# Luckick/EAGCN

Measured on AMD Instinct MI355X. Metric: molecules/sec fwd+bwd, 2-layer 5-view EAGCN, Tox21 batch, higher is better.
Workload: dtype f32 (bf16x3 split, fp32 accumulate): every fp32 operand leaves its producer as three bf16 planes, six v_mfma_f32_32x32x16_bf16 piece products per 16 k rebuild the fp32 product (csrc/gemm_bx3.hip); aggregation, BatchNorm, head, first layer fp32

## Files before the change

eagcn_amd/_lib.py:

```python
import ctypes as C
import os

_HERE = os.path.dirname(os.path.abspath(__file__))
LIB_PATH = os.path.join(_HERE, 'lib', 'libeagcn_hip.so')

MAX_VIEWS = 8
MAX_SEGS = 8
META_WORDS = 16
META_NLOG = 8
META_T, META_NMAX, META_NTILES, META_BAD_ADJ, META_BAD_REL, META_NEDGE, META_OVERFLOW, META_EDGE_OVERFLOW = range(8)
META_NBLK = 9
STRUCT_CONCATE, STRUCT_WEIGHTED = 0, 1

_fp = C.c_void_p


class Batch(C.Structure):
    _fields_ = [('B', C.c_int32), ('N', C.c_int32), ('K', C.c_int32), ('ldc', C.c_int32),
                ('T', C.c_int32), ('n_max', C.c_int32), ('n_tiles', C.c_int32),
                ('channels', C.c_int32 * MAX_VIEWS),
                ('code', _fp), ('deg_bn', _fp), ('nat', _fp), ('row0', _fp), ('tile0', _fp),
                ('meta', _fp), ('row_mol', _fp), ('row_loc', _fp), ('row_m', _fp), ('row_deg', _fp),
                ('tile_mol', _fp), ('row_info', _fp), ('tile_info', _fp),
                ('rel_vec', _fp * MAX_VIEWS), ('rel_c', C.c_int32 * MAX_VIEWS),
# ... 33 lines not shown
    _fields_ = [('K', C.c_int32), ('mode', C.c_int32), ('att_c', C.c_int32 * MAX_VIEWS), ('att_w', _fp * MAX_VIEWS),
                ('ave_a', _fp), ('self_r', _fp), ('datt_w', _fp * MAX_VIEWS), ('dave_a', _fp), ('dself_r', _fp)]


class Layout(C.Structure):
    _fields_ = [('nseg', C.c_int32), ('width', C.c_int32 * MAX_SEGS), ('pad', C.c_int32 * MAX_SEGS)]


class LayerParams(C.Structure):
    _fields_ = [('K', C.c_int32), ('structure', C.c_int32), ('training', C.c_int32),
                ('width', C.c_int32 * MAX_VIEWS), ('inp', Layout),
                ('dropout', C.c_float), ('bn_eps', C.c_float), ('bn_momentum', C.c_float),
                ('seed', C.c_uint64), ('seed_dev', _fp),
                ('att_w', _fp * MAX_VIEWS), ('self_r', _fp * MAX_VIEWS), ('W', _fp * MAX_VIEWS),
                ('bias', _fp * MAX_VIEWS), ('gamma', _fp * MAX_VIEWS), ('beta', _fp * MAX_VIEWS),
                ('run_mean', _fp * MAX_VIEWS), ('run_var', _fp * MAX_VIEWS), ('ave_w', _fp)]


class LayerBufs(C.Structure):
    _fields_ = [('x', _fp), ('P', _fp), ('Y', _fp), ('rscale', _fp), ('bn', _fp), ('xout', _fp),
                ('pad_row', _fp), ('scratch', _fp), ('scratch_bytes', C.c_size_t),
                ('aux_stream', _fp), ('packed', _fp), ('packed_bytes', C.c_size_t),
                ('stats_hook', _fp), ('stats_user', _fp), ('x_planes', _fp), ('xout_planes', _fp)]


class LayerGrads(C.Structure):
    _fields_ = [('dW', _fp * MAX_VIEWS), ('dbias', _fp * MAX_VIEWS), ('dgamma', _fp * MAX_VIEWS),
                ('dbeta', _fp * MAX_VIEWS), ('datt_w', _fp * MAX_VIEWS), ('dself_r', _fp * MAX_VIEWS),
                ('dave_w', _fp)]


class HeadParams(C.Structure):
    _fields_ = [('f_in', C.c_int32), ('n_den1', C.c_int32), ('n_den2', C.c_int32), ('nclass', C.c_int32),
                ('dropout', C.c_float), ('bn_eps', C.c_float), ('bn_momentum', C.c_float),
                ('den1_w', _fp), ('den2_w', _fp), ('den3_w', _fp),
                ('gbn_w', _fp), ('gbn_b', _fp), ('gbn_rm', _fp), ('gbn_rv', _fp),
                ('bn1_w', _fp), ('bn1_b', _fp), ('bn1_rm', _fp), ('bn1_rv', _fp),
                ('bn2_w', _fp), ('bn2_b', _fp), ('bn2_rm', _fp), ('bn2_rv', _fp)]


class HeadGrads(C.Structure):
    _fields_ = [(n, _fp) for n in ('d_den1_w', 'd_den2_w', 'd_den3_w', 'd_gbn_w', 'd_gbn_b', 'd_bn1_w', 'd_bn1_b',
                                   'd_bn2_w', 'd_bn2_b')]


class Model(C.Structure):
    _fields_ = [('n_layers', C.c_int32), ('molfp_mode', C.c_int32), ('training', C.c_int32),
                ('head_seed', C.c_uint64), ('head_seed_dev', _fp), ('input_packed', C.c_int32), ('aux_stream', _fp),
                ('layer', LayerParams * 4), ('head', HeadParams), ('stats_hook', _fp), ('stats_user', _fp),
                ('stats_world', C.c_int32), ('fuse_readout', C.c_int32), ('fwd_signal', _fp), ('wait_flag', _fp), ('start_signal', _fp)]


class StepLoss(C.Structure):
    _fields_ = [('kind', C.c_int32), ('labels', _fp), ('class_weight', _fp), ('loss', _fp), ('scale', _fp), ('dout', _fp)]


ALLREDUCE_FN = C.CFUNCTYPE(C.c_int, C.c_void_p, C.c_int, C.c_void_p, C.c_void_p)


SIGNATURES = {
    'eagcn_abi_version': (C.c_int, []),
    'eagcn_struct_size': (C.c_size_t, [C.c_int]),
    'eagcn_last_error': (C.c_char_p, []),
    'eagcn_pad16': (C.c_int, [C.c_int]),
    'eagcn_layer_out_ld': (C.c_int, [C.POINTER(LayerParams)]),
    'eagcn_layer_fp': (C.c_int, [C.POINTER(LayerParams)]),
    'eagcn_layer_packed_bytes': (C.c_size_t, [C.POINTER(Batch), C.POINTER(LayerParams)]),
    'eagcn_layer_fwd_scratch_bytes': (C.c_size_t, [C.POINTER(Batch), C.POINTER(LayerParams)]),
    'eagcn_layer_bwd_scratch_bytes': (C.c_size_t, [C.POINTER(Batch), C.POINTER(LayerParams)]),
    'eagcn_index_build': (C.c_int, [_fp, C.POINTER(_fp), C.POINTER(Batch), _fp, _fp]),
    'eagcn_index_from_bonds': (C.c_int, [_fp, _fp, _fp, _fp, C.c_int64, C.POINTER(Batch), _fp, _fp]),
    'eagcn_index_rows': (C.c_int, [C.POINTER(Batch), _fp]),
    'eagcn_set_gemm_mode': (C.c_int, [C.c_int]),
    'eagcn_stream_wait_counter': (C.c_int, [_fp, C.c_uint32, _fp]),
    'eagcn_stream_signal_flag': (C.c_int, [_fp, _fp]),
    'eagcn_stream_wait_flag': (C.c_int, [_fp, C.c_double, _fp]),
    'eagcn_stream_wait_timeouts': (C.c_int, []),
    'eagcn_stream_wait_reset': (None, []),
    'eagcn_adam_step': (C.c_int, [_fp, _fp, _fp, _fp, C.c_int64, _fp, _fp, _fp, _fp]),
    'eagcn_agg_wants_bond_lists': (C.c_int, [C.c_int, C.c_int]),
    'eagcn_agg_wants_bond_lists_for': (C.c_int, [C.c_int, C.c_int, C.c_int]),
    'eagcn_bx3_used_splits': (C.c_int, [C.c_int, C.c_int, C.c_int, C.c_int]),
    'eagcn_set_bx3_wide': (C.c_int, [C.c_int]),
    'eagcn_bx3_pair_used_splits': (C.c_int, [C.c_int] * 7),
    'eagcn_bx3_plane_elems': (C.c_size_t, [C.c_int, C.c_int]),
    'eagcn_bx3_split': (C.c_int, [_fp, C.c_int, C.c_int, _fp, C.c_size_t, C.c_int, C.c_int, _fp]),
    'eagcn_gemm_bx3': (C.c_int, [C.c_int, C.c_int, C.c_int, C.c_int, _fp, C.c_size_t, C.c_int, C.c_int, _fp, C.c_size_t, C.c_int, C.c_int,
                                 _fp, C.c_int, C.c_int, C.c_size_t, C.c_int, _fp]),
    'eagcn_gemm_bx3_pair': (C.c_int, [C.c_int, C.c_int, C.c_int, _fp, C.c_size_t, C.c_int, C.c_int, _fp, C.c_size_t, C.c_int, C.c_int, _fp, C.c_int,
                                      C.c_int, C.c_int, C.c_int, _fp, C.c_size_t, C.c_int, C.c_int, _fp, C.c_size_t, C.c_int, C.c_int, _fp, C.c_int,
                                      C.c_int, C.c_size_t, C.c_int, _fp]),
    'eagcn_pack_rows': (C.c_int, [C.POINTER(Batch), _fp, C.c_int, C.POINTER(Layout), _fp, _fp]),
    'eagcn_unpack_rows': (C.c_int, [C.POINTER(Batch), _fp, C.POINTER(Layout), _fp, _fp, C.c_int, _fp]),
    'eagcn_pad_rows': (C.c_int, [_fp, _fp, C.c_int, C.c_int, C.c_int, _fp, _fp]),
    'eagcn_gat_scratch_bytes': (C.c_size_t, [C.POINTER(Batch), C.c_int]),
    'eagcn_gat_forward': (C.c_int, [C.POINTER(Batch), C.POINTER(GatParams), _fp, _fp, _fp, _fp, _fp]),
    'eagcn_gat_backward': (C.c_int, [C.POINTER(Batch), C.POINTER(GatParams), _fp, _fp, _fp, _fp, _fp, _fp, _fp, _fp, _fp,
                                     C.c_size_t, _fp]),
    'eagcn_pool_scratch_bytes': (C.c_size_t, []),
    'eagcn_pool_attention_forward': (C.c_int, [C.POINTER(Batch), C.POINTER(PoolAtt), _fp, C.c_int, _fp, _fp, _fp]),
    'eagcn_pool_attention_backward': (C.c_int, [C.POINTER(Batch), C.POINTER(PoolAtt), _fp, C.c_int, _fp, _fp, _fp, C.c_size_t,
                                                _fp]),
    'eagcn_pool_mix_forward': (C.c_int, [C.POINTER(Batch), C.POINTER(Layout), _fp, C.c_int, _fp, _fp, _fp, _fp, C.c_int, _fp]),
    'eagcn_pool_mix_backward': (C.c_int, [C.POINTER(Batch), C.POINTER(Layout), _fp, C.c_int, _fp, _fp, _fp, _fp, C.c_int, _fp,
                                          _fp, _fp, _fp]),
    'eagcn_pool_reduce_forward': (C.c_int, [C.POINTER(Batch), _fp, C.c_int, C.c_int, C.c_int, _fp, _fp, _fp, _fp]),
    'eagcn_pool_reduce_backward': (C.c_int, [C.POINTER(Batch), _fp, C.c_int, C.c_int, C.c_int, _fp, _fp, _fp, _fp, _fp]),
    'eagcn_layer_forward': (C.c_int, [C.POINTER(Batch), C.POINTER(LayerParams), C.POINTER(LayerBufs), _fp]),
    'eagcn_layer_backward': (C.c_int, [C.POINTER(Batch), C.POINTER(LayerParams), C.POINTER(LayerBufs),
                                       _fp, _fp, _fp, C.POINTER(LayerGrads), _fp]),
    'eagcn_attention_dense': (C.c_int, [C.POINTER(Batch), C.POINTER(LayerParams), _fp, _fp]),
    'eagcn_readout_forward': (C.c_int, [C.POINTER(Batch), _fp, C.POINTER(Layout), _fp, _fp, C.c_int, _fp,
                                        C.c_int, _fp]),
    'eagcn_readout_backward': (C.c_int, [C.POINTER(Batch), _fp, C.POINTER(Layout), _fp, C.c_int, C.c_int,
                                         _fp, _fp, _fp]),
    'eagcn_gemm_f32': (C.c_int, [C.c_int, C.c_int, C.c_int, C.c_int, C.c_int, _fp, C.c_int, _fp, C.c_int,
                                 _fp, C.c_int, _fp]),
    'eagcn_gemm_f32_dev': (C.c_int, [C.c_int, C.c_int, C.c_int, C.c_int, C.c_int, _fp, C.c_int, _fp, C.c_int,
                                     _fp, C.c_int, _fp, C.c_int, _fp]),
    'eagcn_gemm_sk_workspace_bytes': (C.c_size_t, []),
    'eagcn_gemm_f32_sk': (C.c_int, [C.c_int, C.c_int, C.c_int, C.c_int, C.c_int, _fp, C.c_int, _fp, C.c_int,
                                    _fp, C.c_int, _fp, C.c_size_t, _fp]),
    'eagcn_gemm_pair_sk': (C.c_int, [C.c_int, C.c_int, C.c_int, _fp, C.c_int, _fp, C.c_int, _fp, C.c_int,
                                     C.c_int, C.c_int, C.c_int, _fp, C.c_int, _fp, C.c_int, _fp, C.c_int,
                                     _fp, C.c_size_t, _fp]),
    'eagcn_gemm_pair_sk_slabs': (C.c_int, [C.c_int, C.c_int, C.c_int, _fp, C.c_int, _fp, C.c_int, _fp, C.c_int,
                                           C.c_int, C.c_int, C.c_int, _fp, C.c_int, _fp, C.c_int, _fp, C.c_int,
                                           C.c_size_t, _fp, C.c_size_t, _fp]),
    'eagcn_gemm_sk_plan': (C.c_int, [C.c_int] * 7 + [C.POINTER(C.c_int), C.POINTER(C.c_int)]),
    'eagcn_gemm_sk_timeouts': (C.c_int, []),
    'eagcn_gemm_sk_failed': (C.c_int, []),
    'eagcn_gemm_sk_reset_failed': (None, []),
    'eagcn_gemm_sk_inject_failure': (None, []),
    'eagcn_model_saved_bytes': (C.c_size_t, [C.POINTER(Batch), C.POINTER(Model)]),
    'eagcn_model_scratch_bytes': (C.c_size_t, [C.POINTER(Batch), C.POINTER(Model)]),
    'eagcn_model_atom_rep': (C.c_int, [C.POINTER(Batch), C.POINTER(Model), C.POINTER(C.c_size_t),
                                       C.POINTER(C.c_size_t), C.POINTER(C.c_int)]),
    'eagcn_model_atom_rep_materialize': (C.c_int, [C.POINTER(Batch), C.POINTER(Model), _fp, C.c_size_t, _fp]),
    'eagcn_model_pack_input': (C.c_int, [C.POINTER(Batch), C.POINTER(Model), _fp, _fp, C.c_size_t, _fp]),
    'eagcn_model_forward': (C.c_int, [C.POINTER(Batch), C.POINTER(Model), _fp, _fp, _fp, C.c_size_t, _fp,
                                      C.c_size_t, _fp, _fp, _fp]),
    'eagcn_model_backward': (C.c_int, [C.POINTER(Batch), C.POINTER(Model), _fp, _fp, C.c_size_t, _fp, C.c_size_t,
                                       _fp, _fp, C.POINTER(LayerGrads), C.POINTER(HeadGrads), _fp]),
    'eagcn_model_backward_range': (C.c_int, [C.POINTER(Batch), C.POINTER(Model), _fp, _fp, C.c_size_t, _fp, C.c_size_t,
                                             _fp, _fp, C.POINTER(LayerGrads), C.POINTER(HeadGrads), C.c_int, C.c_int, C.c_int, _fp]),
    'eagcn_model_input_scratch_bytes': (C.c_size_t, [C.POINTER(Batch), C.POINTER(Model)]),
    'eagcn_model_backward_input': (C.c_int, [C.POINTER(Batch), C.POINTER(Model), _fp, _fp, C.c_size_t, _fp, C.c_size_t,
                                             _fp, _fp, C.POINTER(LayerGrads), C.POINTER(HeadGrads), _fp, _fp]),
    'eagcn_attr_alpha': (C.c_float, [C.c_int, C.c_int]),
    'eagcn_attr_weight': (C.c_float, [C.c_int]),
    'eagcn_attr_acc_elems': (C.c_size_t, [C.POINTER(Batch), C.POINTER(Model)]),
    'eagcn_attr_pack_input': (C.c_int, [C.POINTER(Batch), C.POINTER(Model), _fp, _fp, C.c_float, _fp, C.c_size_t, _fp]),
    'eagcn_attr_step': (C.c_int, [C.POINTER(Batch), C.POINTER(Model), _fp, _fp, C.c_size_t, _fp, C.c_size_t, _fp, _fp, C.c_float,
                                  C.c_int, _fp, _fp]),
    'eagcn_attr_finalize': (C.c_int, [C.POINTER(Batch), C.POINTER(Model), _fp, _fp, _fp, _fp, _fp, _fp]),
    'eagcn_model_forward_step': (C.c_int, [C.POINTER(Batch), C.POINTER(Model), _fp, _fp, _fp, C.c_size_t, _fp, C.c_size_t, _fp, _fp,
                                           C.POINTER(StepLoss), _fp, C.POINTER(HeadGrads), _fp]),
    'eagcn_head_saved_bytes': (C.c_size_t, [C.POINTER(HeadParams), C.c_int]),
    'eagcn_head_scratch_bytes': (C.c_size_t, [C.POINTER(HeadParams), C.c_int]),
    'eagcn_head_forward': (C.c_int, [C.POINTER(HeadParams), C.c_int, C.c_int, C.c_uint64, _fp, _fp, _fp, C.c_size_t, _fp, C.c_size_t,
                                     _fp, _fp, _fp]),
    'eagcn_head_backward': (C.c_int, [C.POINTER(HeadParams), C.c_int, C.c_int, C.c_uint64, _fp, _fp, _fp, C.c_size_t, _fp, C.c_size_t,
                                      _fp, _fp, C.POINTER(HeadGrads), _fp, _fp]),
    'eagcn_bce_loss': (C.c_int, [_fp, _fp, _fp, C.c_int, C.c_int, _fp, _fp, _fp]),
    'eagcn_mse_loss': (C.c_int, [_fp, _fp, C.c_int, _fp, _fp, _fp]),
    'eagcn_eval_append': (C.c_int, [_fp, _fp, C.c_int, C.c_int, C.c_int, _fp, _fp, _fp, C.c_int64, _fp]),
# ... 65 lines not shown
```

eagcn_amd/csrc/head.hip:

```cpp
#include <stdlib.h>

#include <algorithm>

#include "common.h"
#include "kernels.h"

namespace eagcn {

__global__ void wait_counter_kernel(const uint32_t* __restrict__ word, uint32_t value, int* __restrict__ err,
                                    unsigned long long budget_ticks) {
    if (threadIdx.x == 0) {
        const unsigned long long t0 = wall_clock64();
        while ((int32_t)(__hip_atomic_load(word, __ATOMIC_ACQUIRE, __HIP_MEMORY_SCOPE_AGENT) - value) < 0) {
            __builtin_amdgcn_s_sleep(64);
            if (wall_clock64() - t0 > budget_ticks) {
                if (err) __hip_atomic_store(err, 1, __ATOMIC_RELAXED, __HIP_MEMORY_SCOPE_SYSTEM);
                break;
            }
        }
    }
}



// ... 36 lines not shown
    return EAGCN_OK;
}

struct Carver2 {
    char* base;
    size_t off = 0;
    explicit Carver2(void* p) : base((char*)p) {}
    template <typename T>
    T* take(size_t n) {
        T* p = base ? (T*)(base + off) : nullptr;
        off = align256(off + std::max<size_t>(n, 1) * sizeof(T));
        return p;
    }
};

struct LayerSaved { float *P, *Y, *rscale, *bn, *xout, *pad_row; void* packed; size_t packed_bytes; int fp, ldo, ld_in;
                    uint16_t* xout_planes; };
struct ModelSaved {
    float* x0;
    LayerSaved L[4];
    float *g, *h1, *h2, *bn_g, *bn_1, *bn_2;
    uint16_t* pad_cnt;
    float* padc;
    uint32_t* pad_tab;
    size_t xout_last_off, pad_last_off;
};
static bool pad_sampled(const eagcn_model* m) {
    const eagcn_layer_params* last = &m->layer[m->n_layers - 1];
    return last->structure == EAGCN_STRUCT_WEIGHTED && m->training && last->dropout > 0.0f;
}

static size_t carve_saved(void* base, const eagcn_batch* b, const eagcn_model* m, ModelSaved* out) {
    Carver2 c(base);
    ModelSaved s;
    const size_t T = (size_t)b->T;
    s.x0 = c.take<float>(T * layout_ld(&m->layer[0].in));
    for (int l = 0; l < m->n_layers; ++l) {
        const eagcn_layer_params* p = &m->layer[l];
        LayerSaved& L = s.L[l];
        L.fp = eagcn_layer_fp(p);
        L.ldo = eagcn_layer_out_ld(p);
        L.ld_in = layout_ld(&p->in);
        L.P = c.take<float>(T * L.fp);
        L.Y = c.take<float>(T * L.fp);
        L.rscale = c.take<float>((size_t)p->K * T);
        L.bn = c.take<float>((size_t)4 * L.fp);
        if (l == m->n_layers - 1) s.xout_last_off = c.off;
        L.xout = c.take<float>(T * L.ldo);
        if (l == m->n_layers - 1) s.pad_last_off = c.off;
        L.pad_row = c.take<float>(L.ldo);
        L.packed_bytes = eagcn_layer_packed_bytes(b, p);
        L.packed = c.take<char>(L.packed_bytes);
        const int np = (l + 1 < m->n_layers && L.ldo >= 128 && (L.ldo & 15) == 0) ? gemm_planes() : 0;
        L.xout_planes = np ? c.take<uint16_t>((size_t)np * bx_plane_elems(T, L.ldo)) : nullptr;
    }
    const eagcn_head_params* h = &m->head;
    const size_t B = (size_t)b->B;
    s.g = c.take<float>(B * h->f_in);
    s.h1 = c.take<float>(B * h->n_den1);
    s.h2 = c.take<float>(B * h->n_den2);
    s.bn_g = c.take<float>((size_t)4 * h->f_in);
    s.bn_1 = c.take<float>((size_t)4 * h->n_den1);
    s.bn_2 = c.take<float>((size_t)4 * h->n_den2);
    {
        const eagcn_layer_params* last = &m->layer[m->n_layers - 1];
        const size_t ldo = (size_t)eagcn_layer_out_ld(last);
        const bool need = last->structure == EAGCN_STRUCT_WEIGHTED;
        s.pad_cnt = c.take<uint16_t>(need ? B * last->K * ldo : 1);
        s.padc = c.take<float>(need ? B * ldo : 1);
        const size_t nt = (size_t)(b->N + 1) * (b->N + 1);
        s.pad_tab = c.take<uint32_t>(need ? nt : 1);
    }
    if (out) *out = s;
    return c.off;
}

struct ModelScratch {
    float *da2, *da1, *dgn, *dg, *dxa, *dxb, *dpad;
    float* hdw; int hdw_ks;
    double* hst; int n_hst;
    double* hws;
    double* hsb;
    void* layer; size_t layer_bytes;
};
static size_t carve_scratch(void* base, const eagcn_batch* b, const eagcn_model* m, ModelScratch* out) {
    Carver2 c(base);
    ModelScratch s;
    const eagcn_head_params* h = &m->head;
    const size_t B = (size_t)b->B, T = (size_t)b->T;
    s.n_hst = 2 * (h->f_in + h->n_den1 + h->n_den2) + 6;
    s.hst = c.take<double>((size_t)(HEAD_COPIES + 1) * s.n_hst + HEAD_WS);
    s.hsb = s.hst + (size_t)HEAD_COPIES * s.n_hst;
    s.hws = s.hsb + s.n_hst;
    s.da2 = c.take<float>(B * h->n_den2);
    s.da1 = c.take<float>(B * h->n_den1);
    s.dgn = c.take<float>(B * h->f_in);
    s.dg = c.take<float>(B * h->f_in);
    s.hdw_ks = head_dw_chunks(b->B);
    s.hdw = c.take<float>(s.hdw_ks > 1 ? (size_t)s.hdw_ks * ((size_t)h->f_in * h->n_den1 + (size_t)h->n_den1 * h->n_den2 +
                                                             (size_t)h->n_den2 * h->nclass) : 1);
    int ldmax = 0;
    size_t lbytes = 0;
    for (int l = 0; l < m->n_layers; ++l) {
        ldmax = std::max(ldmax, eagcn_layer_out_ld(&m->layer[l]));
        lbytes = std::max(lbytes, eagcn_layer_fwd_scratch_bytes(b, &m->layer[l]));
        lbytes = std::max(lbytes, eagcn_layer_bwd_scratch_bytes(b, &m->layer[l]));
    }
    s.dxa = c.take<float>(T * ldmax);
    s.dxb = c.take<float>(T * ldmax);
    s.dpad = c.take<float>((size_t)EAGCN_MAX_VIEWS * ldmax);
    s.layer_bytes = lbytes;
    s.layer = c.take<char>(lbytes);
    if (out) *out = s;
    return c.off;
}

static int check_model(const eagcn_batch* b, const eagcn_model* m, const char* who) {
    EAGCN_CHECK_ARG(b && m, "%s: null argument", who);
    EAGCN_CHECK_ARG(m->n_layers >= 1 && m->n_layers <= 4, "%s: n_layers=%d", who, m->n_layers);
    const eagcn_head_params* h = &m->head;
    EAGCN_CHECK_ARG(h->f_in >= 1 && h->n_den1 >= 1 && h->n_den2 >= 1 && h->nclass >= 1, "%s: bad head sizes", who);
    EAGCN_CHECK_ARG(h->den1_w && h->den2_w && h->den3_w && h->gbn_w && h->gbn_b && h->gbn_rm && h->gbn_rv &&
                        h->bn1_w && h->bn1_b && h->bn1_rm && h->bn1_rv && h->bn2_w && h->bn2_b && h->bn2_rm &&
                        h->bn2_rv, "%s: null head parameter", who);
    const eagcn_layer_params* last = &m->layer[m->n_layers - 1];
    const int f_last = last->structure == EAGCN_STRUCT_CONCATE ? [&] { int s = 0; for (int k = 0; k < last->K; ++k) s += last->width[k]; return s; }()
                                                                 : last->width[0];
    EAGCN_CHECK_ARG(f_last == h->f_in, "%s: head expects %d features, last layer yields %d", who, h->f_in, f_last);
    EAGCN_CHECK_ARG(!m->training || b->B > 1, "%s: BatchNorm in training mode needs more than one molecule", who);
    return EAGCN_OK;
}

static eagcn_layout out_layout(const eagcn_layer_params* p) {
    eagcn_layout l;
    memset(&l, 0, sizeof(l));
    if (p->structure == EAGCN_STRUCT_CONCATE) {
        l.nseg = p->K;
        for (int k = 0; k < p->K; ++k) { l.width[k] = p->width[k]; l.pad[k] = pad16(p->width[k]); }
    } else {
        l.nseg = 1;
        l.width[0] = p->width[0];
        l.pad[0] = pad16(p->width[0]);
    }
    return l;
}

static bool fused_readout(const eagcn_model* m) {
    static const bool env = [] { const char* v = getenv("EAGCN_NO_FUSED_READOUT"); return !(v && v[0] == '1'); }();
    return env && m->fuse_readout && m->layer[m->n_layers - 1].structure == EAGCN_STRUCT_CONCATE;
}

static bool hidden_planes_only(const eagcn_batch* b, const eagcn_model* m, const ModelSaved& sv, int l) {
    return l + 1 < m->n_layers && sv.L[l].xout_planes && layer_reads_planes_only(b, &m->layer[l + 1], m->aux_stream != nullptr);
}

static void fill_drop(float p, int training, int* do_drop, uint32_t* thr, float* inv_keep) {
    *do_drop = (training && p > 0.0f) ? 1 : 0;
    *thr = (uint32_t)std::min(4294967295.0, (double)p * 4294967296.0);
    *inv_keep = 1.0f / (1.0f - p);
}

}

using namespace eagcn;

#define RC(call) do { int rc_ = (call); if (rc_) return rc_; } while (0)

extern "C" size_t eagcn_model_saved_bytes(const eagcn_batch* b, const eagcn_model* m) {
    return carve_saved(nullptr, b, m, nullptr);
}
extern "C" size_t eagcn_model_scratch_bytes(const eagcn_batch* b, const eagcn_model* m) {
    return carve_scratch(nullptr, b, m, nullptr);
}
extern "C" int eagcn_model_atom_rep(const eagcn_batch* b, const eagcn_model* m, size_t* xout_offset,
                                    size_t* pad_row_offset, int* ld) {
    EAGCN_CHECK_ARG(b && m && xout_offset && pad_row_offset && ld, "eagcn_model_atom_rep: null argument");
    ModelSaved s;
    carve_saved(nullptr, b, m, &s);
    *xout_offset = s.xout_last_off;
    *pad_row_offset = s.pad_last_off;
    *ld = eagcn_layer_out_ld(&m->layer[m->n_layers - 1]);
    return EAGCN_OK;
}

extern "C" int eagcn_model_atom_rep_materialize(const eagcn_batch* b, const eagcn_model* m, void* saved, size_t saved_bytes,
                                                 void* stream) {
    EAGCN_CHECK_ARG(b && m && saved, "eagcn_model_atom_rep_materialize: null argument");
    if (!fused_readout(m)) return EAGCN_OK;
    ModelSaved sv;
// ... 10 lines not shown
                                      size_t saved_bytes, void* stream) {
    EAGCN_CHECK_ARG(b && m && afm && saved, "eagcn_model_pack_input: null argument");
    ModelSaved sv;
    EAGCN_CHECK_ARG(carve_saved(saved, b, m, &sv) <= saved_bytes, "eagcn_model_pack_input: saved block too small");
    return eagcn_pack_rows(b, afm, layout_width(&m->layer[0].in), &m->layer[0].in, sv.x0, stream);
}

struct HeadPlan {
    HeadFwd f1, f2, f3;
    HeadBwd b3, b2, b1;
    HeadGbn bg;
    double *st_g, *st_1, *st_2, *sb_g, *sb_1, *sb_2;
    bool sync;
};
static HeadPlan head_plan(const eagcn_batch* b, const eagcn_model* m, const ModelSaved& sv, const ModelScratch& sc, float* out,
                          float* graph_rep, const float* dout, const float* dgraph_rep, const eagcn_head_grads* hg) {
    HeadPlan P;
    const eagcn_head_params* h = &m->head;
    const int B = b->B, F = h->f_in, n1 = h->n_den1, n2 = h->n_den2, nc = h->nclass;
    P.st_g = sc.hst; P.st_1 = sc.hst + 2 * F + 2; P.st_2 = sc.hst + 2 * (F + n1) + 4;
    P.sb_g = sc.hsb; P.sb_1 = sc.hsb + 2 * F + 2; P.sb_2 = sc.hsb + 2 * (F + n1) + 4;
    P.sync = m->stats_hook && m->training;
    const int copies = P.sync ? 1 : HEAD_COPIES;
    HeadDrop nodrop{0, 0u, 1.0f, 0, nullptr}, drop1 = nodrop;
    {
        int on; uint32_t thr; float inv_keep;
        fill_drop(h->dropout, m->training, &on, &thr, &inv_keep);
        drop1 = HeadDrop{on, thr, inv_keep, m->head_seed, m->head_seed_dev};
    }
    P.f1 = HeadFwd{B, F, n1, sv.g, P.st_g, h->gbn_w, h->gbn_b, h->gbn_rm, h->gbn_rv, sv.bn_g, h->den1_w, sv.h1, nullptr, P.st_1,
                   m->training, 0, h->bn_eps, h->bn_momentum, nodrop};
    P.f2 = HeadFwd{B, n1, n2, sv.h1, P.st_1, h->bn1_w, h->bn1_b, h->bn1_rm, h->bn1_rv, sv.bn_1, h->den2_w, sv.h2, graph_rep, P.st_2,
                   m->training, 1, h->bn_eps, h->bn_momentum, drop1};
    P.f3 = HeadFwd{B, n2, nc, sv.h2, P.st_2, h->bn2_w, h->bn2_b, h->bn2_rm, h->bn2_rv, sv.bn_2, h->den3_w, out, nullptr, nullptr,
                   m->training, 1, h->bn_eps, h->bn_momentum, nodrop};
    if (P.sync) { P.f1.cnt_in = P.st_g + 2 * F; P.f2.cnt_in = P.st_1 + 2 * n1; P.f3.cnt_in = P.st_2 + 2 * n2; }
    P.f3.nw = 8;
    P.f1.signal = m->fwd_signal;
    P.f1.st_copies = P.f2.st_copies = P.f3.st_copies = copies;
    P.f1.st_stride = P.f2.st_stride = P.f3.st_stride = sc.n_hst;
    if (!hg) return P;
    const double *cn_g = sc.hst + 2 * F, *cn_1 = sc.hst + 2 * F + 2 + 2 * n1, *cn_2 = sc.hst + 2 * (F + n1) + 4 + 2 * n2;
    const float gscale = P.sync && m->stats_world > 1 ? 1.0f / (float)m->stats_world : 1.0f;
    P.b3 = HeadBwd{B, n2, nc, sv.h2, sv.bn_2, 1, nodrop, h->den3_w, dout, nullptr, nullptr, nullptr, nullptr, nullptr, nullptr,
                   sc.da2, P.sb_2, hg->d_den3_w, m->training};
    P.b2 = HeadBwd{B, n1, n2, sv.h1, sv.bn_1, 1, drop1, h->den2_w, sc.da2, sv.h2, sv.bn_2, P.sb_2, dgraph_rep, hg->d_bn2_w, hg->d_bn2_b,
                   sc.da1, P.sb_1, hg->d_den2_w, m->training};
    P.b1 = HeadBwd{B, F, n1, sv.g, sv.bn_g, 0, nodrop, h->den1_w, sc.da1, sv.h1, sv.bn_1, P.sb_1, nullptr, hg->d_bn1_w, hg->d_bn1_b,
                   sc.dgn, P.sb_g, hg->d_den1_w, m->training};
    if (P.sync) { P.b2.cnt_y = cn_2; P.b2.gscale = gscale; P.b1.cnt_y = cn_1; P.b1.gscale = gscale; }
    P.b3.nw = 8;
    const int ks = sc.hdw_ks;
    float* part3 = sc.hdw;
    float* part2 = part3 + (size_t)ks * n2 * nc;
    float* part1 = part2 + (size_t)ks * n1 * n2;
    if (ks > 1) {
        P.b3.ks = ks; P.b3.dW_part = part3;
        P.b2.ks = ks; P.b2.dW_part = part2;
        P.b1.ks = ks; P.b1.dW_part = part1;
    }
    P.bg = HeadGbn{B, F, sc.dgn, sv.g, sv.bn_g, P.sb_g, sc.dg, hg->d_gbn_w, hg->d_gbn_b, m->training};
    if (P.sync) { P.bg.cnt = cn_g; P.bg.gscale = gscale; }
    if (ks > 1) {
        P.bg.sum[0] = HeadDwSum{hg->d_den3_w, part3, n2 * nc, ks};
        P.bg.sum[1] = HeadDwSum{hg->d_den2_w, part2, n1 * n2, ks};
        P.bg.sum[2] = HeadDwSum{hg->d_den1_w, part1, F * n1, ks};
        P.bg.nsum = 3;
    }
    return P;
}

static int model_forward_trunk(const eagcn_batch* b, const eagcn_model* m, const float* afm, const int64_t* size, void* saved,
                               size_t saved_bytes, void* scratch, size_t scratch_bytes, ModelSaved& sv, ModelScratch& sc,
                               void* stream, const char* who) {
    hipStream_t s = (hipStream_t)stream;
    RC(check_model(b, m, who));
    EAGCN_CHECK_GEMM3(who);
    EAGCN_CHECK_ARG((afm || m->input_packed) && saved && scratch, "%s: null buffer", who);
    EAGCN_CHECK_ARG(m->molfp_mode == 0 || size, "%s: 'ave' read-out needs size", who);
    EAGCN_CHECK_ARG(carve_saved(saved, b, m, &sv) <= saved_bytes, "%s: saved block too small", who);
    EAGCN_CHECK_ARG(carve_scratch(scratch, b, m, &sc) <= scratch_bytes, "%s: scratch too small", who);
    const eagcn_head_params* h = &m->head;
    HandOff ho{m->start_signal, m->wait_flag, wait_err_word(), 200000000ull};
    if (!m->input_packed && (m->wait_flag || m->start_signal)) {
        handoff_kernel<<<1, 64, 0, s>>>(ho);
        EAGCN_LAUNCH_CHECK();
        ho.start = nullptr; ho.flag = nullptr;
    }
    ZeroJob zj;
    RC(gemm3_zero_job(sc.layer, sc.layer_bytes, sc.hst, (HEAD_COPIES + 1) * sc.n_hst + HEAD_WS, &zj));
    if (!m->input_packed)
        RC(eagcn_pack_rows(b, afm, layout_width(&m->layer[0].in), &m->layer[0].in, sv.x0, stream));
    const float* x = sv.x0;
    {
        const eagcn_layer_params* ps[4];
        void* pk[4];
        size_t pkb[4];
        for (int l = 0; l < m->n_layers; ++l) { ps[l] = &m->layer[l]; pk[l] = sv.L[l].packed; pkb[l] = sv.L[l].packed_bytes; }
        RC(pack_params_all(b, ps, pk, pkb, m->n_layers, stream, &zj, &ho));
    }
    for (int l = 0; l < m->n_layers; ++l) {
        LayerSaved& L = sv.L[l];
        eagcn_layer_bufs w;
        memset(&w, 0, sizeof(w));
        w.x = x; w.P = L.P; w.Y = L.Y; w.rscale = L.rscale; w.bn = L.bn; w.xout = L.xout; w.pad_row = L.pad_row;
        w.scratch = sc.layer; w.scratch_bytes = sc.layer_bytes; w.packed = L.packed; w.packed_bytes = L.packed_bytes;
        w.stats_hook = m->stats_hook; w.stats_user = m->stats_user;
        w.x_planes = l > 0 ? sv.L[l - 1].xout_planes : nullptr; w.xout_planes = L.xout_planes;
        const bool po = hidden_planes_only(b, m, sv, l);
        RC(layer_forward_impl(b, &m->layer[l], &w, stream, true, l == m->n_layers - 1 && fused_readout(m), po));
        x = po ? nullptr : L.xout;
    }
    const eagcn_layer_params* last = &m->layer[m->n_layers - 1];
    const LayerSaved& LL = sv.L[m->n_layers - 1];
    const eagcn_layout lay = out_layout(last);
    const int B = b->B, F = h->f_in, n1 = h->n_den1, n2 = h->n_den2;
    double *st_g = sc.hst, *st_1 = sc.hst + 2 * F + 2, *st_2 = sc.hst + 2 * (F + n1) + 4;
    const int copies = (m->stats_hook && m->training) ? 1 : HEAD_COPIES;
    if (fused_readout(m)) {
        ReadoutBn rb;
        rb.Y = LL.Y; rb.ldy = LL.fp; rb.bn = LL.bn; rb.fp = LL.fp;
        fill_drop(last->dropout, last->training, &rb.do_drop, &rb.thr, &rb.inv_keep);
        rb.seed = last->seed; rb.seed_dev = last->seed_dev;
        rb.size = size; rb.mode = m->molfp_mode; rb.g = sv.g; rb.F = F; rb.st = st_g;
        rb.cnt0 = st_g + 2 * F; rb.cnt1 = st_1 + 2 * n1; rb.cnt2 = st_2 + 2 * n2;
        rb.st_copies = copies; rb.st_stride = sc.n_hst;
        RC(readout_bn_forward(b, &lay, rb, stream));
    } else if (pad_sampled(m))
        RC(readout_forward_sampled(b, LL.xout, &lay, last, LL.bn + (size_t)LL.fp , size,
                                   m->molfp_mode, sv.g, F, sv.pad_cnt, sv.padc, sv.pad_tab, stream));
    else
        RC(eagcn_readout_forward(b, LL.xout, &lay, last->structure == EAGCN_STRUCT_WEIGHTED ? LL.pad_row : nullptr,
                                 size, m->molfp_mode, sv.g, F, stream));
    if (!fused_readout(m)) RC(head_colstats(sv.g, B, F, st_g, s, st_g + 2 * F, st_1 + 2 * n1, st_2 + 2 * n2));
    return EAGCN_OK;
}

static int stats_hook_call(const eagcn_model* m, bool sync, double* buf, int n, void* stream) {
    if (!sync) return EAGCN_OK;
    if (m->stats_hook(buf, n, stream, m->stats_user)) {
        set_error("eagcn_model: the sync-BatchNorm all-reduce hook failed");
        return EAGCN_ERR_HIP;
    }
    return EAGCN_OK;
}

static int head_forward_launches(const eagcn_model* m, const HeadPlan& P, void* stream) {
    hipStream_t s = (hipStream_t)stream;
    const eagcn_head_params* h = &m->head;
    RC(stats_hook_call(m, P.sync, P.st_g, 2 * h->f_in + 1, stream));
    RC(head_fwd(P.f1, s));
    RC(stats_hook_call(m, P.sync, P.st_1, 2 * h->n_den1 + 1, stream));
    RC(head_fwd(P.f2, s));
    RC(stats_hook_call(m, P.sync, P.st_2, 2 * h->n_den2 + 1, stream));
    RC(head_fwd(P.f3, s));
    return EAGCN_OK;
}
static int head_backward_launches(const eagcn_model* m, const HeadPlan& P, void* stream) {
    hipStream_t s = (hipStream_t)stream;
    const eagcn_head_params* h = &m->head;
    RC(head_bwd(P.b3, s));
    RC(stats_hook_call(m, P.sync, P.sb_2, 2 * h->n_den2, stream));
    RC(head_bwd(P.b2, s));
    RC(stats_hook_call(m, P.sync, P.sb_1, 2 * h->n_den1, stream));
    RC(head_bwd(P.b1, s));
    RC(stats_hook_call(m, P.sync, P.sb_g, 2 * h->f_in, stream));
    RC(head_gbn_bwd(P.bg, s));
    return EAGCN_OK;
}
static int readout_pad_backward(const eagcn_batch* b, const eagcn_model* m, const int64_t* size, const ModelSaved& sv,
                                const ModelScratch& sc, void* stream) {
    const eagcn_layer_params* last = &m->layer[m->n_layers - 1];
    const eagcn_layout lay = out_layout(last);
    const int F = m->head.f_in;
    if (pad_sampled(m)) return readout_backward_pad_views(b, sc.dg, &lay, size, m->molfp_mode, F, last->K, sv.pad_cnt, last->dropout, sc.dpad, stream);
    if (last->structure == EAGCN_STRUCT_WEIGHTED) return readout_backward_pad(b, sc.dg, &lay, size, m->molfp_mode, F, sc.dpad, stream);
    return EAGCN_OK;
}

extern "C" int eagcn_model_forward(const eagcn_batch* b, const eagcn_model* m, const float* afm,
                                   const int64_t* size, void* saved, size_t saved_bytes, void* scratch,
                                   size_t scratch_bytes, float* out, float* graph_rep, void* stream) {
    EAGCN_CHECK_ARG(out && graph_rep, "eagcn_model_forward: null buffer");
    ModelSaved sv;
    ModelScratch sc;
    RC(model_forward_trunk(b, m, afm, size, saved, saved_bytes, scratch, scratch_bytes, sv, sc, stream, "eagcn_model_forward"));
    const HeadPlan P = head_plan(b, m, sv, sc, out, graph_rep, nullptr, nullptr, nullptr);
    return head_forward_launches(m, P, stream);
}

namespace eagcn {
static int check_head(const eagcn_head_params* h, int B, int training, const char* who) {
    EAGCN_CHECK_ARG(h, "%s: null argument", who);
// ... 113 lines not shown
                                        const eagcn_head_grads* hg, void* stream) {
    hipStream_t s = (hipStream_t)stream;
    EAGCN_CHECK_ARG(out && graph_rep && loss && hg, "eagcn_model_forward_step: null argument");
    EAGCN_CHECK_ARG(m && m->training, "eagcn_model_forward_step: a training-mode model is required");
    EAGCN_CHECK_ARG((loss->kind == 0 || loss->kind == 1) && loss->labels && loss->loss && loss->dout && (loss->kind == 1 || loss->class_weight),
                    "eagcn_model_forward_step: bad loss descriptor");
    EAGCN_CHECK_ARG(hg->d_den1_w && hg->d_den2_w && hg->d_den3_w && hg->d_gbn_w && hg->d_gbn_b && hg->d_bn1_w &&
                        hg->d_bn1_b && hg->d_bn2_w && hg->d_bn2_b, "eagcn_model_forward_step: null head gradient");
    ModelSaved sv;
    ModelScratch sc;
    RC(model_forward_trunk(b, m, afm, size, saved, saved_bytes, scratch, scratch_bytes, sv, sc, stream, "eagcn_model_forward_step"));
    const HeadPlan P = head_plan(b, m, sv, sc, out, graph_rep, loss->dout, dgraph_rep, hg);
    const eagcn_head_params* h = &m->head;
    if (!P.sync && head_mid_ok(h->n_den2, h->nclass)) {
        HeadPlan Q = P;
        unsigned* words = reinterpret_cast<unsigned*>(sc.hws);
        if (loss->kind == 0) { Q.f2.lab = loss->labels; Q.f2.nlab = b->B * h->nclass; Q.f2.lab_cnt = words + 1; }
        RC(head_fwd(Q.f1, s));
        RC(head_fwd(Q.f2, s));
        HeadMid M;
        M.f3 = Q.f3; M.b3 = Q.b3;
        M.L = HeadLoss{loss->kind, loss->labels, loss->class_weight, loss->loss, loss->scale, loss->dout};
        M.ws = sc.hws;
        RC(head_mid(M, s));
        RC(head_bwd_pair(Q.b2, Q.b3, HeadLossFin{loss->loss, sc.hws, loss->scale, loss->kind, b->B * h->nclass}, s));
        RC(head_bwd(Q.b1, s));
        RC(head_gbn_bwd(Q.bg, s));
    } else {
        RC(head_forward_launches(m, P, stream));
        if (loss->kind == 0) RC(eagcn_bce_loss(out, loss->labels, loss->class_weight, b->B, h->nclass, loss->loss, loss->dout, stream));
        else RC(eagcn_mse_loss(out, loss->labels, b->B * h->nclass, loss->loss, loss->dout, stream));
        if (loss->scale) {
            const int n = b->B * h->nclass;
            scale_loss_kernel<<<cdiv(n, 256), 256, 0, s>>>(loss->loss, loss->dout, n, loss->scale);
            EAGCN_LAUNCH_CHECK();
        }
        RC(head_backward_launches(m, P, stream));
    }
    return readout_pad_backward(b, m, size, sv, sc, stream);
}

extern "C" int eagcn_model_backward(const eagcn_batch* b, const eagcn_model* m, const int64_t* size, void* saved,
                                    size_t saved_bytes, void* scratch, size_t scratch_bytes, const float* dout,
                                    const float* dgraph_rep, const eagcn_layer_grads* lg,
                                    const eagcn_head_grads* hg, void* stream) {
    EAGCN_CHECK_ARG(m, "eagcn_model_backward: null model");
    return eagcn_model_backward_range(b, m, size, saved, saved_bytes, scratch, scratch_bytes, dout, dgraph_rep, lg, hg, 1,
                                      m->n_layers - 1, 0, stream);
}

static int model_backward_impl(const eagcn_batch* b, const eagcn_model* m, const int64_t* size, void* saved, size_t saved_bytes,
                               void* scratch, size_t scratch_bytes, const float* dout, const float* dgraph_rep,
                               const eagcn_layer_grads* lg, const eagcn_head_grads* hg, int with_head, int layer_hi, int layer_lo,
                               float* dx0, bool input_only, void* stream) {
    hipStream_t s = (hipStream_t)stream;
    EAGCN_CHECK_ARG(saved && scratch && dout && (lg || input_only) && hg, "eagcn_model_backward: null buffer");
    EAGCN_CHECK_ARG(hg->d_den1_w && hg->d_den2_w && hg->d_den3_w && hg->d_gbn_w && hg->d_gbn_b && hg->d_bn1_w &&
                        hg->d_bn1_b && hg->d_bn2_w && hg->d_bn2_b, "eagcn_model_backward: null head gradient");
    EAGCN_CHECK_ARG(layer_hi < m->n_layers && layer_lo >= 0 && layer_lo <= layer_hi + 1,
                    "eagcn_model_backward_range: layers %d..%d of %d", layer_hi, layer_lo, m->n_layers);
    EAGCN_CHECK_ARG(!with_head || layer_hi == m->n_layers - 1 || layer_hi < layer_lo,
                    "eagcn_model_backward_range: the head's backward is followed by the top layer");
    ModelSaved sv;
    ModelScratch sc;
    EAGCN_CHECK_ARG(carve_saved(saved, b, m, &sv) <= saved_bytes, "eagcn_model_backward: saved block too small");
    EAGCN_CHECK_ARG(carve_scratch(scratch, b, m, &sc) <= scratch_bytes, "eagcn_model_backward: scratch too small");
    const int F = m->head.f_in;
    const ZeroJob zb{nullptr, 0, sc.hsb, sc.n_hst};
    hipStream_t side = m->aux_stream ? (hipStream_t)m->aux_stream : s;
    const bool forked = side != s;
    const eagcn_layer_params* last = &m->layer[m->n_layers - 1];
    const eagcn_layout lay = out_layout(last);
    const bool weighted = last->structure == EAGCN_STRUCT_WEIGHTED;
    const bool sampled = pad_sampled(m);
    if (with_head) {
        const HeadPlan P = head_plan(b, m, sv, sc, nullptr, nullptr, dout, dgraph_rep, hg);
        RC(head_backward_launches(m, P, stream));
        if (!(input_only && !m->training)) RC(readout_pad_backward(b, m, size, sv, sc, stream));
    }
    ReadoutGrad rgd;
    memset(&rgd, 0, sizeof(rgd));
    rgd.dg = sc.dg; rgd.F = F; rgd.size = size; rgd.mode = m->molfp_mode; rgd.map = make_colmap(&lay);
    const int top_l = m->n_layers - 1;
    EdgeDrain pend_in, pend_out;
    pend_in.eacc = nullptr;
    pend_out.eacc = nullptr;
    for (int l = layer_hi; l >= layer_lo; --l) {
        const int t = top_l - l;
        float* cur = (t & 1) ? sc.dxb : sc.dxa;
        float* other = (t & 1) ? sc.dxa : sc.dxb;
        LayerSaved& L = sv.L[l];
        eagcn_layer_bufs w;
        memset(&w, 0, sizeof(w));
        w.x = l == 0 ? sv.x0 : (hidden_planes_only(b, m, sv, l - 1) ? nullptr : sv.L[l - 1].xout);
        w.P = L.P; w.Y = L.Y; w.rscale = L.rscale; w.bn = L.bn; w.xout = L.xout; w.pad_row = L.pad_row;
        w.scratch = sc.layer; w.scratch_bytes = sc.layer_bytes; w.packed = L.packed; w.packed_bytes = L.packed_bytes;
        w.aux_stream = m->aux_stream;
        w.stats_hook = m->stats_hook; w.stats_user = m->stats_user;
        w.x_planes = l > 0 ? sv.L[l - 1].xout_planes : nullptr;
        const bool top = l == top_l;
        const float* dpad = (weighted && top) ? sc.dpad : nullptr;
        RC(layer_backward_impl(b, &m->layer[l], &w, top ? nullptr : cur, top ? &rgd : nullptr, dpad,
                               l > 0 ? other : dx0, input_only ? nullptr : &lg[l], stream, top && sampled, top ? &zb : nullptr,
                               pend_in.eacc ? &pend_in : nullptr, (l > layer_lo && !input_only) ? &pend_out : nullptr, input_only));
        pend_in = pend_out;
        if (l == layer_lo) pend_in.eacc = nullptr;
    }
    if (forked) RC(stream_after(s, side));
    return EAGCN_OK;
}

extern "C" int eagcn_model_backward_range(const eagcn_batch* b, const eagcn_model* m, const int64_t* size, void* saved,
                                          size_t saved_bytes, void* scratch, size_t scratch_bytes, const float* dout,
                                          const float* dgraph_rep, const eagcn_layer_grads* lg,
                                          const eagcn_head_grads* hg, int with_head, int layer_hi, int layer_lo, void* stream) {
    RC(check_model(b, m, "eagcn_model_backward"));
    EAGCN_CHECK_GEMM3("eagcn_model_backward");
    return model_backward_impl(b, m, size, saved, saved_bytes, scratch, scratch_bytes, dout, dgraph_rep, lg, hg, with_head, layer_hi,
                               layer_lo, nullptr, false, stream);
}

struct InputScratch { float* dx0; eagcn_head_grads hg; };
static size_t carve_input_scratch(void* base, const eagcn_batch* b, const eagcn_model* m, InputScratch* out) {
    Carver2 c(base);
    c.off = carve_scratch(nullptr, b, m, nullptr);
    InputScratch t;
    const eagcn_head_params* h = &m->head;
    const size_t F = h->f_in, n1 = h->n_den1, n2 = h->n_den2, nc = h->nclass;
    t.dx0 = c.take<float>((size_t)std::max(b->T, 1) * layout_ld(&m->layer[0].in));
    t.hg.d_den1_w = c.take<float>(F * n1);
    t.hg.d_den2_w = c.take<float>(n1 * n2);
    t.hg.d_den3_w = c.take<float>(n2 * nc);
    t.hg.d_gbn_w = c.take<float>(F);
    t.hg.d_gbn_b = c.take<float>(F);
    t.hg.d_bn1_w = c.take<float>(n1);
    t.hg.d_bn1_b = c.take<float>(n1);
    t.hg.d_bn2_w = c.take<float>(n2);
    t.hg.d_bn2_b = c.take<float>(n2);
    if (out) *out = t;
    return c.off;
}

static int check_engine_model(const eagcn_batch* b, const eagcn_model* m, const char* who) {
    RC(check_model(b, m, who));
    EAGCN_CHECK_ARG(m->molfp_mode == 0 || m->molfp_mode == 1, "%s: read-out mode %d has no engine path", who, m->molfp_mode);
    for (int l = 0; l < m->n_layers; ++l)
        EAGCN_CHECK_ARG(m->layer[l].structure == EAGCN_STRUCT_CONCATE || m->layer[l].structure == EAGCN_STRUCT_WEIGHTED,
                        "%s: layer %d has structure %d, which the engine does not run", who, l, m->layer[l].structure);
    return EAGCN_OK;
}

int eagcn::model_backward_input_packed(const eagcn_batch* b, const eagcn_model* m, const int64_t* size, void* saved, size_t saved_bytes,
                                       void* scratch, size_t scratch_bytes, const float* dout, const float* dgraph_rep,
                                       const eagcn_layer_grads* lg, const eagcn_head_grads* hg, float** dx0, void* stream,
                                       const char* who) {
    EAGCN_CHECK_ARG(b && m, "%s: null argument", who);
    EAGCN_CHECK_ARG((lg == nullptr) == (hg == nullptr), "%s: lg and hg are both given (full backward) or both NULL (input-only)", who);
    RC(check_engine_model(b, m, who));
    EAGCN_CHECK_GEMM3(who);
    EAGCN_CHECK_ARG(saved && scratch && dout, "%s: null buffer", who);
    InputScratch is;
    EAGCN_CHECK_ARG(carve_input_scratch(scratch, b, m, &is) <= scratch_bytes, "%s: scratch too small (eagcn_model_input_scratch_bytes)", who);
    *dx0 = is.dx0;
    const bool input_only = lg == nullptr;
    return model_backward_impl(b, m, size, saved, saved_bytes, scratch, scratch_bytes, dout, dgraph_rep, lg, input_only ? &is.hg : hg, 1,
                               m->n_layers - 1, 0, is.dx0, input_only, stream);
}

int eagcn::model_input_slot(const eagcn_batch* b, const eagcn_model* m, void* saved, size_t saved_bytes, float** x0, const char* who) {
    ModelSaved sv;
    EAGCN_CHECK_ARG(carve_saved(saved, b, m, &sv) <= saved_bytes, "%s: saved block too small", who);
    *x0 = sv.x0;
    return EAGCN_OK;
}

extern "C" size_t eagcn_model_input_scratch_bytes(const eagcn_batch* b, const eagcn_model* m) {
    return (b && m) ? carve_input_scratch(nullptr, b, m, nullptr) : 0;
}

extern "C" int eagcn_model_backward_input(const eagcn_batch* b, const eagcn_model* m, const int64_t* size, void* saved,
                                          size_t saved_bytes, void* scratch, size_t scratch_bytes, const float* dout,
                                          const float* dgraph_rep, const eagcn_layer_grads* lg, const eagcn_head_grads* hg,
                                          float* dafm, void* stream) {
    EAGCN_CHECK_ARG(dafm, "eagcn_model_backward_input: null dafm");
    float* dx0 = nullptr;
    RC(model_backward_input_packed(b, m, size, saved, saved_bytes, scratch, scratch_bytes, dout, dgraph_rep, lg, hg, &dx0, stream,
                                   "eagcn_model_backward_input"));
    return launch_attr_dense(b, &m->layer[0].in, dx0, nullptr, nullptr, dafm, nullptr, (hipStream_t)stream);
}
// ... 25 lines not shown
```

eagcn_amd/csrc/kernels.h:

```cpp
#pragma once
#include "bx3.h"
#include "common.h"

namespace eagcn {

struct AggArgs {
    eagcn_batch bt;
    ViewCols vc;
    const float* src; int lds;
    float* dst; int ldd;
    const float* sig;
    const float* rsig;
    float* rscale;
    double* stats;
    int nchunk;
    int cpw = 1;
    int xcd = 0;
    bool w_rowm = false;
    BxOut planes = {nullptr, 0, 0, 0};
    const float* bn_tab = nullptr; const float* bn_cc = nullptr; int bn_fp = 0;
    const float* w_aw = nullptr;
    int w_drop = 0; uint32_t w_thr = 0; float w_inv_keep = 1.0f; uint64_t w_seed = 0; const uint64_t* w_seed_dev = nullptr;
};
int agg_grid_x(const eagcn_batch* b);
// ... 92 lines not shown
}
size_t gemm3_workspace_bytes();
bool gemm3_xk_enabled();
int gemm3_grid();
int gemm3_clear_flags(void* workspace, size_t bytes, hipStream_t s, double* zero = nullptr, int nzero = 0);
int gemm3_failed();
#define EAGCN_CHECK_GEMM3(who)                                                                                         \
    do {                                                                                                               \
        if (::eagcn::gemm3_failed()) {                                                                                 \
            ::eagcn::set_error("%s: a stream-K hand-off of an earlier GEMM launch timed out (a contributor wave was not " \
                               "co-resident with its owner): that launch's results are NaN-poisoned; call "           \
                               "eagcn_gemm_sk_reset_failed() after fixing the cause (EAGCN_GEMM3_WGS, concurrent work)", who); \
            return EAGCN_ERR_HIP;                                                                                      \
        }                                                                                                              \
    } while (0)
int gemm_mode();
inline int gemm_planes() { const int m = gemm_mode(); return m == 3 ? 3 : m == 4 ? 1 : 0; }
struct ZeroJob { unsigned* u; int nu; double* d; int nd; };
struct HandOff { uint32_t* start; uint32_t* flag; int* err; unsigned long long budget; };
__device__ __forceinline__ void handoff_body(const HandOff& h) {
    if (h.start) __hip_atomic_fetch_add(h.start, 1u, __ATOMIC_RELEASE, __HIP_MEMORY_SCOPE_AGENT);
    if (h.flag) {
        const unsigned long long t0 = wall_clock64();
        while (__hip_atomic_load(h.flag, __ATOMIC_ACQUIRE, __HIP_MEMORY_SCOPE_AGENT) == 0u) {
            __builtin_amdgcn_s_sleep(8);
            if (wall_clock64() - t0 > h.budget) {
                if (h.err) __hip_atomic_store(h.err, 1, __ATOMIC_RELAXED, __HIP_MEMORY_SCOPE_SYSTEM);
                break;
            }
        }
        __hip_atomic_store(h.flag, 0u, __ATOMIC_RELAXED, __HIP_MEMORY_SCOPE_AGENT);
    }
}
int gemm3_zero_job(void* workspace, size_t bytes, double* zero, int nzero, ZeroJob* out);
int zero_fill(void* p, size_t bytes, hipStream_t s);
bool gemm3_ok(const GemmDesc& g);
int launch_gemm3(const GemmDesc& g, const DwScatter* sc, void* workspace, size_t bytes, hipStream_t s);
int launch_gemm3_pair(const GemmDesc& dx, const GemmDesc& dw, const DwScatter* sc, void* workspace, size_t bytes, hipStream_t s,
                      size_t xk_slab = 0);

constexpr int HEAD_COPIES = 8;
struct HeadDrop { int on; uint32_t thr; float inv_keep; uint64_t seed; const uint64_t* seed_dev; };
struct HeadFwd {
    int B, K, N;
    const float* x; const double* st_in; const float *gamma, *beta; float *run_mean, *run_var; float* bn;
    const float* W; float* y; float* y2; double* st_out;
    int training, relu; float eps, momentum; HeadDrop drop;
    const double* cnt_in = nullptr;
    int st_copies = 1, st_stride = 0;
    const float* lab = nullptr; int nlab = 0; unsigned* lab_cnt = nullptr;
    int nw = 0;
    uint32_t* signal = nullptr;
};
struct HeadBwd {
    int B, K, N;
    const float* x; const float* bnp; int relu_p; HeadDrop drop; const float* W;
    const float* dy; const float* y; const float* bny; const double* sb_y; const float* extra;
    float *dgamma_y, *dbeta_y; float* dyp; double* sb_p; float* dW; int training;
    const double* cnt_y = nullptr;
    float gscale = 1.0f;
    int ks = 1; float* dW_part = nullptr;
    int nw = 0;
};
inline int head_dw_chunks(int B) { return B > 256 ? (B + 255) / 256 < 16 ? (B + 255) / 256 : 16 : 1; }
struct HeadDwSum { float* dst; const float* part; int n, ks; };
struct HeadGbn { int B, F; const float *dgn, *g, *bn; const double* sb; float *dg, *dgamma, *dbeta; int training;
                 const double* cnt = nullptr; float gscale = 1.0f;
                 HeadDwSum sum[3] = {}; int nsum = 0; };
struct HeadLoss { int kind;
                  const float* labels; const float* weight; float* loss; const float* scale; float* dout; };
struct HeadMid { HeadFwd f3; HeadBwd b3; HeadLoss L;
                 double* ws; };
constexpr int HEAD_WS = 4;
struct HeadLossFin { float* loss; const double* ws; const float* scale; int kind, n; };
bool head_mid_ok(int n_den2, int nclass);
int head_mid(const HeadMid& a, hipStream_t s);
int head_bwd_pair(const HeadBwd& a, const HeadBwd& e, const HeadLossFin& lf, hipStream_t s);
int head_colstats(const float* g, int B, int F, double* st, hipStream_t s, double* cnt0 = nullptr, double* cnt1 = nullptr,
                  double* cnt2 = nullptr);
int head_fwd(const HeadFwd& a, hipStream_t s);
int head_bwd(const HeadBwd& a, hipStream_t s);
int head_gbn_bwd(const HeadGbn& a, hipStream_t s);

struct EdgeDrain {
    double* eacc; int K;
    float* datt_w[EAGCN_MAX_VIEWS]; float* dself_r[EAGCN_MAX_VIEWS]; int channels[EAGCN_MAX_VIEWS];
    const float* rsig;
};
int layer_backward_impl(const eagcn_batch* b, const eagcn_layer_params* p, const eagcn_layer_bufs* w,
                        const float* dxout, const ReadoutGrad* rg, const float* dpad_row, float* dx,
                        const eagcn_layer_grads* g, void* stream, bool dpad_views = false,
                        const ZeroJob* zero_after = nullptr, const EdgeDrain* drain_in = nullptr, EdgeDrain* drain_out = nullptr,
                        bool input_only = false);
int model_backward_input_packed(const eagcn_batch* b, const eagcn_model* m, const int64_t* size, void* saved, size_t saved_bytes,
                                void* scratch, size_t scratch_bytes, const float* dout, const float* dgraph_rep,
                                const eagcn_layer_grads* lg, const eagcn_head_grads* hg, float** dx0, void* stream, const char* who);
int launch_attr_dense(const eagcn_batch* b, const eagcn_layout* in, const float* acc, const float* x, const float* base, float* attr,
                      float* score, hipStream_t s);
int model_input_slot(const eagcn_batch* b, const eagcn_model* m, void* saved, size_t saved_bytes, float** x0, const char* who);
int layer_forward_impl(const eagcn_batch* b, const eagcn_layer_params* p, const eagcn_layer_bufs* w, void* stream,
                       bool prepacked, bool skip_apply = false, bool planes_only = false);
bool layer_reads_planes_only(const eagcn_batch* b, const eagcn_layer_params* p, bool aux_stream);
int layer_apply_impl(const eagcn_batch* b, const eagcn_layer_params* p, const eagcn_layer_bufs* w, void* stream);
int pack_params_all(const eagcn_batch* b, const eagcn_layer_params* const* ps, void* const* packed,
                    const size_t* packed_bytes, int n, void* stream, const ZeroJob* zj = nullptr, const HandOff* ho = nullptr);
struct ReadoutBn {
    const float* Y; int ldy;
    const float* bn; int fp;
    int do_drop; uint32_t thr; float inv_keep; uint64_t seed; const uint64_t* seed_dev;
    const int64_t* size; int mode;
    float* g; int F;
    double* st;
    int st_copies = 1, st_stride = 0;
    bool pair = false;
    double *cnt0, *cnt1, *cnt2;
};
int readout_bn_forward(const eagcn_batch* b, const eagcn_layout* lay, const ReadoutBn& a, void* stream);
int readout_forward_sampled(const eagcn_batch* b, const float* x, const eagcn_layout* lay, const eagcn_layer_params* p,
                            const float* bn_sh, const int64_t* size, int mode, float* g, int F, uint16_t* cnt, float* padc,
                            uint32_t* tab, void* stream);
int readout_backward_pad_views(const eagcn_batch* b, const float* dg, const eagcn_layout* lay, const int64_t* size, int mode,
                               int F, int K, const uint16_t* cnt, float dropout, float* dpad, void* stream);
int readout_backward_pad(const eagcn_batch* b, const float* dg, const eagcn_layout* lay, const int64_t* size,
                         int mode, int F, float* dpad_row, void* stream);

}
```

eagcn_amd/csrc/layer.hip:

```cpp
#include <algorithm>

#include <stdlib.h>

#include "common.h"
#include "kernels.h"

namespace eagcn {

struct ParamPtrs {
    const float* att_w[EAGCN_MAX_VIEWS];
    const float* self_r[EAGCN_MAX_VIEWS];
    const float* W[EAGCN_MAX_VIEWS];
    const float* bias[EAGCN_MAX_VIEWS];
    const float* gamma[EAGCN_MAX_VIEWS];
    const float* beta[EAGCN_MAX_VIEWS];
    float* run_mean[EAGCN_MAX_VIEWS];
    float* run_var[EAGCN_MAX_VIEWS];
    const float* ave_w;
    int channels[EAGCN_MAX_VIEWS];
    const float* rel_vec[EAGCN_MAX_VIEWS];
    int rel_c[EAGCN_MAX_VIEWS];
};
__device__ __forceinline__ float att_logit(const ParamPtrs& pp, int k, int c) {
    if (!pp.rel_vec[k]) return pp.att_w[k][c - 1];
    const float* v = pp.rel_vec[k] + (size_t)(c - 1) * pp.rel_c[k];
    float s = 0.0f;
    for (int ch = 0; ch < pp.rel_c[k]; ++ch) s = fmaf(pp.att_w[k][ch], v[ch], s);
    return s;
}
struct GradPtrs {
    float* dW[EAGCN_MAX_VIEWS];
    float* dbias[EAGCN_MAX_VIEWS];
    float* dgamma[EAGCN_MAX_VIEWS];
    float* dbeta[EAGCN_MAX_VIEWS];
    float* datt_w[EAGCN_MAX_VIEWS];
    float* dself_r[EAGCN_MAX_VIEWS];
    float* dave_w;
};

enum { CP_GAMMA = 0, CP_BETA, CP_BIAS, CP_RMEAN, CP_RVAR, CP_AVEW, CP_ROWS = 8 };

__device__ __forceinline__ int col_view(const ViewCols& vc, int cp) {
    int k = 0;
#pragma unroll
    for (int v = 1; v < EAGCN_MAX_VIEWS; ++v) k += (v < vc.K && cp >= vc.off[v]) ? 1 : 0;
    return k;
}
__device__ __forceinline__ int packed_to_exact(const ColMapD& m, int cp) {
    int eo = 0, po = 0;
    for (int s = 0; s < m.nseg; ++s) {
        if (cp < po + m.p[s]) return (cp - po < m.w[s]) ? eo + (cp - po) : -1;
        eo += m.w[s];
        po += m.p[s];
    }
    return -1;
}

__device__ __forceinline__ void pack_params_body(const ParamPtrs& pp, const ViewCols& vc, const ColMapD& in, int ld_in,
                                                 int fp, float* __restrict__ Wcat, float* __restrict__ WcatT,
                                                 float* __restrict__ colp, float* __restrict__ sig, float* __restrict__ rsig,
                                                 const BxOut wp = BxOut{nullptr, 0, 0, 0}, const BxOut wtp = BxOut{nullptr, 0, 0, 0}) {
    __shared__ float tile[32][33];
    const int tx = threadIdx.x & 31, ty = threadIdx.x >> 5;
    const int ntx = (fp + 31) >> 5, nty = (ld_in + 31) >> 5;
    for (int t = blockIdx.x; t < ntx * nty; t += gridDim.x) {
        const int ip0 = (t / ntx) << 5, cp0 = (t % ntx) << 5;
        {
            const int cp = cp0 + tx;
            const int k = cp < fp ? col_view(vc, cp) : 0;
            const int f = cp - vc.off[k];
#pragma unroll
            for (int j = 0; j < 4; ++j) {
                const int ip = ip0 + ty + 8 * j;
                float v = 0.0f;
                if (ip < ld_in && cp < fp) {
                    const int fi = packed_to_exact(in, ip);
                    if (fi >= 0 && f < vc.width[k]) v = pp.W[k][(size_t)fi * vc.width[k] + f];
                    Wcat[(size_t)ip * fp + cp] = v;
                }
                tile[ty + 8 * j][tx] = v;
            }
        }
        __syncthreads();
#pragma unroll
        for (int j = 0; j < 4; ++j) {
            const int cp = cp0 + ty + 8 * j, ip = ip0 + tx;
            if (cp < fp && ip < ld_in) WcatT[(size_t)cp * ld_in + ip] = tile[tx][ty + 8 * j];
        }
        if (wp.p) {
            const int r = threadIdx.x >> 3, c4 = (threadIdx.x & 7) << 2;
            if (ip0 + r < ld_in && cp0 + c4 < fp)
                bx_store4(wp, ip0 + r, cp0 + c4, make_float4(tile[r][c4], tile[r][c4 + 1], tile[r][c4 + 2], tile[r][c4 + 3]));
            if (cp0 + r < fp && ip0 + c4 < ld_in)
                bx_store4(wtp, cp0 + r, ip0 + c4, make_float4(tile[c4][r], tile[c4 + 1][r], tile[c4 + 2][r], tile[c4 + 3][r]));
        }
        __syncthreads();
    }
    for (int cp = blockIdx.x * blockDim.x + threadIdx.x; cp < fp; cp += gridDim.x * blockDim.x) {
        const int k = col_view(vc, cp), f = cp - vc.off[k];
        const bool ok = f < vc.width[k];
        colp[CP_GAMMA * fp + cp] = ok ? pp.gamma[k][f] : 0.0f;
        colp[CP_BETA * fp + cp] = ok ? pp.beta[k][f] : 0.0f;
        colp[CP_BIAS * fp + cp] = ok ? pp.bias[k][f] : 0.0f;
        colp[CP_RMEAN * fp + cp] = ok ? pp.run_mean[k][f] : 0.0f;
        colp[CP_RVAR * fp + cp] = ok ? pp.run_var[k][f] : 1.0f;
        colp[CP_AVEW * fp + cp] = pp.ave_w ? pp.ave_w[k] : 1.0f;
    }
    for (int e = blockIdx.x * blockDim.x + threadIdx.x; e < vc.K * 256; e += gridDim.x * blockDim.x) {
        const int k = e >> 8, c = e & 255;
        sig[e] = (c >= 1 && c <= pp.channels[k]) ? sigmoidf_(att_logit(pp, k, c)) : 0.0f;
    }
    if (blockIdx.x == 0 && threadIdx.x < vc.K) rsig[threadIdx.x] = sigmoidf_(pp.self_r[threadIdx.x][0]);
}
__global__ __launch_bounds__(256) void pack_params_kernel(ParamPtrs pp, ViewCols vc, ColMapD in, int ld_in, int fp,
                                                           float* __restrict__ Wcat, float* __restrict__ WcatT,
                                                           float* __restrict__ colp, float* __restrict__ sig,
                                                           float* __restrict__ rsig, BxOut wp, BxOut wtp) {
    pack_params_body(pp, vc, in, ld_in, fp, Wcat, WcatT, colp, sig, rsig, wp, wtp);
}
struct PackJob {
    ParamPtrs pp; ViewCols vc; ColMapD in; int ld_in, fp;
    float *Wcat, *WcatT, *colp, *sig, *rsig;
    BxOut wp, wtp;
};
struct PackJobs { PackJob j0, j1, j2, j3; };
__global__ __launch_bounds__(256) void pack_params_multi_kernel(PackJobs jobs, ZeroJob zj, HandOff ho) {
    if (blockIdx.y == 0) {
        for (int i = blockIdx.x * blockDim.x + threadIdx.x; i < max(zj.nu, zj.nd); i += gridDim.x * blockDim.x) {
            if (i < zj.nu) zj.u[i] = 0u;
            if (i < zj.nd) zj.d[i] = 0.0;
        }
    }
    if (blockIdx.y == 0) pack_params_body(jobs.j0.pp, jobs.j0.vc, jobs.j0.in, jobs.j0.ld_in, jobs.j0.fp, jobs.j0.Wcat, jobs.j0.WcatT, jobs.j0.colp, jobs.j0.sig, jobs.j0.rsig, jobs.j0.wp, jobs.j0.wtp);
    else if (blockIdx.y == 1) pack_params_body(jobs.j1.pp, jobs.j1.vc, jobs.j1.in, jobs.j1.ld_in, jobs.j1.fp, jobs.j1.Wcat, jobs.j1.WcatT, jobs.j1.colp, jobs.j1.sig, jobs.j1.rsig, jobs.j1.wp, jobs.j1.wtp);
    else if (blockIdx.y == 2) pack_params_body(jobs.j2.pp, jobs.j2.vc, jobs.j2.in, jobs.j2.ld_in, jobs.j2.fp, jobs.j2.Wcat, jobs.j2.WcatT, jobs.j2.colp, jobs.j2.sig, jobs.j2.rsig, jobs.j2.wp, jobs.j2.wtp);
    else pack_params_body(jobs.j3.pp, jobs.j3.vc, jobs.j3.in, jobs.j3.ld_in, jobs.j3.fp, jobs.j3.Wcat, jobs.j3.WcatT, jobs.j3.colp, jobs.j3.sig, jobs.j3.rsig, jobs.j3.wp, jobs.j3.wtp);
    if (blockIdx.x == 0 && blockIdx.y == 0 && threadIdx.x == 0) handoff_body(ho);
}

template <int L>
__device__ __forceinline__ void slab_sum(const double* __restrict__ slab, int nslab, int fp, int cp, int sl,
                                           double& s1, double& s2) {
    s1 = 0.0;
    s2 = 0.0;
    for (int s0 = sl; s0 < nslab; s0 += L * 8) {
        double2 v[8];
#pragma unroll
        for (int u = 0; u < 8; ++u) {
            const int s = s0 + L * u;
            v[u] = s < nslab ? *reinterpret_cast<const double2*>(slab + ((size_t)s * fp + cp) * 2) : make_double2(0.0, 0.0);
        }
#pragma unroll
        for (int u = 0; u < 8; ++u) { s1 += v[u].x; s2 += v[u].y; }
    }
#pragma unroll
    for (int o = L / 2; o > 0; o >>= 1) {
        s1 += __shfl_xor(s1, o);
        s2 += __shfl_xor(s2, o);
    }
}

constexpr int BWD_ROWS = 7;
template <int L>
__global__ __launch_bounds__(256) void bn_stats_sum_kernel(const double* __restrict__ slab, int nslab, int fp, double M,
                                                            double* __restrict__ out, const int32_t* __restrict__ meta,
                                                            int mode, int tiles_per_wg, int nvirt, int batch_B) {
    if (meta[EAGCN_META_NLOG] > 0) M = (double)batch_B * (double)meta[EAGCN_META_NLOG];
    if (mode == 1 && tiles_per_wg > 0) nslab = min(nslab, (meta[EAGCN_META_NTILES] + tiles_per_wg - 1) / tiles_per_wg);
    if (mode == 1 && tiles_per_wg < 0) nslab = min(nslab, meta[EAGCN_META_NBLK]);
    if (mode == 2) nslab = max(1, min(nslab, (meta[EAGCN_META_T] + nvirt + BWD_ROWS - 1) / BWD_ROWS));
    const int cpr = blockIdx.x * (256 / L) + threadIdx.x / L, sl = threadIdx.x % L;
    const int cp = min(cpr, fp - 1);
    double s1, s2;
    slab_sum<L>(slab, nslab, fp, cp, sl, s1, s2);
    if (cpr < fp && sl == 0) { out[2 * cp] = s1; out[2 * cp + 1] = s2; }
    if (blockIdx.x == 0 && threadIdx.x == 0) out[2 * fp] = M;
}

template <int L>
__global__ __launch_bounds__(256) void bn_finalize_kernel(const double* __restrict__ slab, int nslab, int fp,
                                                           double M, int training, float eps, float momentum,
                                                           const float* __restrict__ colp, ParamPtrs pp,
                                                           ViewCols vc, float* __restrict__ bn,
                                                           const int32_t* __restrict__ meta, int tiles_per_wg, int batch_B,
                                                           const double* __restrict__ M_dev) {
    if (meta[EAGCN_META_NLOG] > 0) M = (double)batch_B * (double)meta[EAGCN_META_NLOG];
    if (M_dev) M = *M_dev;
    if (tiles_per_wg > 0) nslab = min(nslab, (meta[EAGCN_META_NTILES] + tiles_per_wg - 1) / tiles_per_wg);
    if (tiles_per_wg < 0) nslab = min(nslab, meta[EAGCN_META_NBLK]);
    const int cpr = blockIdx.x * (256 / L) + threadIdx.x / L, sl = threadIdx.x % L;
    const int cp = min(cpr, fp - 1);
    double s1 = 0.0, s2 = 0.0;
    if (training) slab_sum<L>(slab, nslab, fp, cp, sl, s1, s2);
    if (cpr >= fp || sl != 0) return;
    const int k = col_view(vc, cp), f = cp - vc.off[k];
    const float gamma = colp[CP_GAMMA * fp + cp], beta = colp[CP_BETA * fp + cp];
    const float bias = colp[CP_BIAS * fp + cp];
    float mu, inv;
    if (training) {
        const double mean = s1 / M;
        double var = s2 / M - mean * mean;
        var = var > 0.0 ? var : 0.0;
        mu = (float)mean;
        inv = (float)(1.0 / sqrt(var + (double)eps));
        if (f < vc.width[k]) {
            const double unbiased = var * (M / (M - 1.0));
            pp.run_mean[k][f] = (float)((1.0 - momentum) * (double)colp[CP_RMEAN * fp + cp] + momentum * (mean + (double)bias));
            pp.run_var[k][f] = (float)((1.0 - momentum) * (double)colp[CP_RVAR * fp + cp] + momentum * unbiased);
        }
    } else {
        mu = colp[CP_RMEAN * fp + cp] - bias;
        inv = 1.0f / sqrtf(colp[CP_RVAR * fp + cp] + eps);
    }
    const float sc = gamma * inv;
    bn[BN_SC * fp + cp] = sc;
    bn[BN_SH * fp + cp] = beta - mu * sc;
    bn[BN_MU * fp + cp] = mu;
    bn[BN_INV * fp + cp] = inv;
}

struct ApplyArgs {
    eagcn_batch bt;
    ViewCols vc;
    int structure, fp;
    const float* Y; int ldy;
    const float* bn;
    const float* colp;
    float* out; int ldo;
    float* pad_row;
    int do_drop; uint32_t thr; float inv_keep; uint64_t seed; const uint64_t* seed_dev;
    BxOut planes;
    int tile_map;
};

__global__ __launch_bounds__(256) void bn_apply_kernel(ApplyArgs a) {
    const int fp = a.fp;
    const uint64_t seed = a.seed_dev ? *a.seed_dev : a.seed;
    if (blockIdx.x == 0) {
        for (int c = threadIdx.x; c < a.ldo; c += blockDim.x) {
            float v = 0.0f;
            if (a.structure == EAGCN_STRUCT_WEIGHTED)
                for (int k = 0; k < a.vc.K; ++k) {
                    const int cp = a.vc.off[k] + c;
                    v += a.colp[CP_AVEW * fp + cp] * fmaxf(a.bn[BN_SH * fp + cp], 0.0f);
                }
            a.pad_row[c] = v;
        }
    }
    const int T = dev_rows(a.bt);
    if (a.structure == EAGCN_STRUCT_CONCATE) {
        const uint32_t g4 = a.tile_map ? ((uint32_t)(fp + 31) >> 5) : fp / 4;
        const uint32_t total = a.tile_map ? (((uint32_t)T + 7) >> 3) * g4 * 64u : (uint32_t)T * g4;
        for (uint32_t e = blockIdx.x * blockDim.x + threadIdx.x; e < total; e += gridDim.x * blockDim.x) {
            int r, c;
            if (a.tile_map) {
                const uint32_t it = e >> 6, rg = it / g4;
                r = (int)(rg * 8u + ((e >> 3) & 7u)); c = (int)((it - rg * g4) * 32u + (e & 7u) * 4u);
                if (r >= T || c >= fp) continue;
            } else {
                r = (int)(e / g4); c = (int)(e - (uint32_t)r * g4) * 4;
            }
            const float4 y = *reinterpret_cast<const float4*>(a.Y + (size_t)r * a.ldy + c);
            const float4 sc = *reinterpret_cast<const float4*>(a.bn + BN_SC * fp + c);
            const float4 sh = *reinterpret_cast<const float4*>(a.bn + BN_SH * fp + c);
            const float m = a.bt.row_m[r];
            float4 o;
            o.x = fmaxf(y.x * sc.x + sh.x, 0.0f) * m;
            o.y = fmaxf(y.y * sc.y + sh.y, 0.0f) * m;
            o.z = fmaxf(y.z * sc.z + sh.z, 0.0f) * m;
            o.w = fmaxf(y.w * sc.w + sh.w, 0.0f) * m;
            if (a.do_drop) {
                float ds[4];
                drop_scale4(seed, (uint64_t)r * fp + c, a.thr, a.inv_keep, ds);
                o.x *= ds[0]; o.y *= ds[1]; o.z *= ds[2]; o.w *= ds[3];
            }
            if (a.out) *reinterpret_cast<float4*>(a.out + (size_t)r * a.ldo + c) = o;
            if (a.planes.p) bx_store4(a.planes, r, c, o);
        }
    } else {
        const uint32_t g4 = a.tile_map ? ((uint32_t)(a.ldo + 31) >> 5) : a.ldo / 4;
        const uint32_t total = a.tile_map ? (((uint32_t)T + 7) >> 3) * g4 * 64u : (uint32_t)T * g4;
        for (uint32_t e = blockIdx.x * blockDim.x + threadIdx.x; e < total; e += gridDim.x * blockDim.x) {
            int r, f;
            if (a.tile_map) {
                const uint32_t it = e >> 6, rg = it / g4;
                r = (int)(rg * 8u + ((e >> 3) & 7u)); f = (int)((it - rg * g4) * 32u + (e & 7u) * 4u);
                if (r >= T || f >= a.ldo) continue;
            } else {
                r = (int)(e / g4); f = (int)(e - (uint32_t)r * g4) * 4;
            }
            float4 y[EAGCN_MAX_VIEWS];
#pragma unroll
            for (int k = 0; k < EAGCN_MAX_VIEWS; ++k)
                if (k < a.vc.K) y[k] = *reinterpret_cast<const float4*>(a.Y + (size_t)r * a.ldy + a.vc.off[k] + f);
            float4 acc = {0.0f, 0.0f, 0.0f, 0.0f};
#pragma unroll
            for (int k = 0; k < EAGCN_MAX_VIEWS; ++k)
                if (k < a.vc.K) {
                    const int cp = a.vc.off[k] + f;
                    const float4 sc = *reinterpret_cast<const float4*>(a.bn + BN_SC * fp + cp);
                    const float4 sh = *reinterpret_cast<const float4*>(a.bn + BN_SH * fp + cp);
                    const float4 w = *reinterpret_cast<const float4*>(a.colp + CP_AVEW * fp + cp);
                    float4 p;
                    p.x = fmaxf(y[k].x * sc.x + sh.x, 0.0f);
                    p.y = fmaxf(y[k].y * sc.y + sh.y, 0.0f);
                    p.z = fmaxf(y[k].z * sc.z + sh.z, 0.0f);
                    p.w = fmaxf(y[k].w * sc.w + sh.w, 0.0f);
                    if (a.do_drop) {
                        float ds[4];
                        drop_scale4(seed, (uint64_t)r * fp + cp, a.thr, a.inv_keep, ds);
                        p.x *= ds[0]; p.y *= ds[1]; p.z *= ds[2]; p.w *= ds[3];
                    }
                    acc.x += w.x * p.x; acc.y += w.y * p.y; acc.z += w.z * p.z; acc.w += w.w * p.w;
                }
            if (a.out) *reinterpret_cast<float4*>(a.out + (size_t)r * a.ldo + f) = acc;
            if (a.planes.p) bx_store4(a.planes, r, f, acc);
        }
    }
}

struct BwdArgs {
    const int32_t* meta; int Tcap;
    const int32_t* row_mol;
    const float* row_m;
    ViewCols vc;
    int structure, fp, nvirt;
    const float* dxout; int ldo;
    ReadoutGrad rg;
    const float* dpad;
    int dpad_views;
    const float* Y; int ldy;
    const float* bn;
    const float* colp;
    float* dH;
    double* slab;
    double* slab_da;
    int do_drop; uint32_t thr; float inv_keep; uint64_t seed; const uint64_t* seed_dev;
    double* zero; int nzero;
    EdgeDrain drain;
    const float* cc;
    int store_dh;
};

template <bool WEIGHTED, bool DG, bool DROP, bool APPLY>
__global__ __launch_bounds__(256) void bn_bwd_reduce_kernel(BwdArgs a) {
    __shared__ double da_s[EAGCN_MAX_VIEWS];
    const uint64_t seed = DROP ? (a.seed_dev ? *a.seed_dev : a.seed) : 0ull;
    const int fp = a.fp, T = min(a.meta[EAGCN_META_T], a.Tcap);
    const int rows = T + (APPLY ? 0 : a.nvirt);
    const int nwg = max(1, min((int)gridDim.x, (rows + BWD_ROWS - 1) / BWD_ROWS));
    if (!APPLY && a.drain.eacc && blockIdx.x == 0 && blockIdx.y == 0) {
        const int K = a.drain.K;
        for (int e = threadIdx.x; e < K * EDGE_SLAB; e += blockDim.x) {
            const int k = e / EDGE_SLAB, c = e - k * EDGE_SLAB;
            if (c > 256) continue;
            double v[EDGE_COPIES];
#pragma unroll
            for (int z = 0; z < EDGE_COPIES; ++z) v[z] = a.drain.eacc[((size_t)z * K + k) * EDGE_SLAB + c];
            double t = 0.0;
#pragma unroll
            for (int z = 0; z < EDGE_COPIES; ++z) { t += v[z]; a.drain.eacc[((size_t)z * K + k) * EDGE_SLAB + c] = 0.0; }
            float* dw = nullptr;
            float* dr = nullptr;
            int ch = 0;
#pragma unroll
            for (int q = 0; q < EAGCN_MAX_VIEWS; ++q)
                if (q == k) { dw = a.drain.datt_w[q]; dr = a.drain.dself_r[q]; ch = a.drain.channels[q]; }
            if (c == 256) {
                const double r = (double)a.drain.rsig[k];
                dr[0] = (float)(t * r * (1.0 - r));
            } else if (c >= 1 && c <= ch) {
                dw[c - 1] = (float)t;
            }
        }
    }
    if ((int)blockIdx.x >= nwg || (APPLY && T == 0)) return;
    if constexpr (!APPLY) {
        if (threadIdx.x < EAGCN_MAX_VIEWS) da_s[threadIdx.x] = 0.0;
        __syncthreads();
    }
    constexpr bool weighted = WEIGHTED;
    double da[EAGCN_MAX_VIEWS];
#pragma unroll
    for (int k = 0; k < EAGCN_MAX_VIEWS; ++k) da[k] = 0.0;
    const int c_lo = blockIdx.y * (int)blockDim.x * 4;
    for (int cp = c_lo + threadIdx.x * 4; cp < min(fp, c_lo + (int)blockDim.x * 4); cp += blockDim.x * 4) {
        const int k = col_view(a.vc, cp), f = cp - a.vc.off[k];
        const float4 sc = *reinterpret_cast<const float4*>(a.bn + BN_SC * fp + cp);
        const float4 sh = *reinterpret_cast<const float4*>(a.bn + BN_SH * fp + cp);
        const float4 mu = *reinterpret_cast<const float4*>(a.bn + BN_MU * fp + cp);
        const float4 iv = *reinterpret_cast<const float4*>(a.bn + BN_INV * fp + cp);
        const float4 aw = *reinterpret_cast<const float4*>(a.colp + CP_AVEW * fp + cp);
        float4 c1 = make_float4(0.f, 0.f, 0.f, 0.f), c2 = c1;
        if constexpr (APPLY) {
            c1 = *reinterpret_cast<const float4*>(a.cc + cp);
            c2 = *reinterpret_cast<const float4*>(a.cc + fp + cp);
        }
        const int cu = weighted ? f : cp;
        auto exact = [&](int c) {
            int eo = 0, po = 0, res = -1;
            bool done = false;
#pragma unroll
            for (int sg = 0; sg < EAGCN_MAX_SEGS; ++sg) {
                if (sg < a.rg.map.nseg && !done) {
                    if (c < po + a.rg.map.p[sg]) { res = (c - po < a.rg.map.w[sg]) ? eo + (c - po) : -1; done = true; }
                    eo += a.rg.map.w[sg];
                    po += a.rg.map.p[sg];
                }
            }
            return res;
        };
        int ce0 = -1, ce1 = -1, ce2 = -1, ce3 = -1;
        bool ce4 = false;
        if constexpr (DG) {
            ce0 = exact(cu); ce1 = exact(cu + 1); ce2 = exact(cu + 2); ce3 = exact(cu + 3);
            ce4 = ce0 >= 0 && ce3 == ce0 + 3 && (ce0 & 3) == 0 && (a.rg.F & 3) == 0 &&
                  (reinterpret_cast<uintptr_t>(a.rg.dg) & 15) == 0;
        }
        double s1[4] = {0.0, 0.0, 0.0, 0.0}, s2[4] = {0.0, 0.0, 0.0, 0.0}, dak = 0.0;
        for (int rb = blockIdx.x; rb < rows; rb += BWD_ROWS * nwg) {
            float4 yv[BWD_ROWS], upv[BWD_ROWS];
#pragma unroll
            for (int u = 0; u < BWD_ROWS; ++u) {
                const int r = rb + u * nwg;
                yv[u] = make_float4(0.f, 0.f, 0.f, 0.f);
                upv[u] = make_float4(0.f, 0.f, 0.f, 0.f);
                if (r < T) {
                    yv[u] = *reinterpret_cast<const float4*>(a.Y + (size_t)r * a.ldy + cp);
                    if constexpr (DG) {
                        const int mol = a.row_mol[r];
                        const float* g = a.rg.dg + (size_t)mol * a.rg.F;
                        float4 v;
                        if (ce4) {
                            v = *reinterpret_cast<const float4*>(g + ce0);
                        } else {
                            v.x = ce0 >= 0 ? g[ce0] : 0.0f;
                            v.y = ce1 >= 0 ? g[ce1] : 0.0f;
                            v.z = ce2 >= 0 ? g[ce2] : 0.0f;
                            v.w = ce3 >= 0 ? g[ce3] : 0.0f;
                        }
                        if (a.rg.mode == 1) {
                            const float is = 1.0f / (float)a.rg.size[mol];
                            v.x *= is; v.y *= is; v.z *= is; v.w *= is;
                        }
                        upv[u] = v;
                    } else {
                        upv[u] = *reinterpret_cast<const float4*>(a.dxout + (size_t)r * a.ldo + cu);
                    }
                    if (!weighted) {
                        const float m = a.row_m[r];
                        upv[u].x *= m; upv[u].y *= m; upv[u].z *= m; upv[u].w *= m;
                    }
                } else if (r < rows) {
                    upv[u] = *reinterpret_cast<const float4*>(a.dpad + (size_t)(a.dpad_views ? k : (r - T)) * a.ldo + cu);
                }
            }
#pragma unroll
            for (int u = 0; u < BWD_ROWS; ++u) {
                const int r = rb + u * nwg;
                if (r >= rows) continue;
                const float yy[4] = {yv[u].x, yv[u].y, yv[u].z, yv[u].w};
                const float uu[4] = {upv[u].x, upv[u].y, upv[u].z, upv[u].w};
                const float scv[4] = {sc.x, sc.y, sc.z, sc.w}, shv[4] = {sh.x, sh.y, sh.z, sh.w};
                const float muv[4] = {mu.x, mu.y, mu.z, mu.w}, ivv[4] = {iv.x, iv.y, iv.z, iv.w};
                const float awv[4] = {aw.x, aw.y, aw.z, aw.w};
                const float c1v[4] = {c1.x, c1.y, c1.z, c1.w}, c2v[4] = {c2.x, c2.y, c2.z, c2.w};
                float dh[4], dsv[4] = {1.0f, 1.0f, 1.0f, 1.0f};
                if (DROP && r < T) drop_scale4(seed, (uint64_t)r * fp + cp, a.thr, a.inv_keep, dsv);
#pragma unroll
                for (int j = 0; j < 4; ++j) {
                    float up = uu[j];
                    const float ds = dsv[j];
                    const float h = yy[j] * scv[j] + shv[j];
                    if (weighted) { if constexpr (!APPLY) dak += (double)(up * ds * fmaxf(h, 0.0f)); up *= awv[j]; }
                    dh[j] = h > 0.0f ? up * ds : 0.0f;
                    const float xh = (yy[j] - muv[j]) * ivv[j];
                    if constexpr (APPLY) {
                        dh[j] = scv[j] * (dh[j] - c1v[j] - xh * c2v[j]);
                    } else {
                        s1[j] += (double)dh[j];
                        s2[j] += (double)(dh[j] * xh);
                    }
                }
                if ((APPLY || a.store_dh) && r < T)
                    *reinterpret_cast<float4*>(a.dH + (size_t)r * fp + cp) = make_float4(dh[0], dh[1], dh[2], dh[3]);
            }
        }
        if constexpr (!APPLY) {
            double* sl = a.slab + ((size_t)blockIdx.x * fp + cp) * 2;
            *reinterpret_cast<double4*>(sl) = make_double4(s1[0], s2[0], s1[1], s2[1]);
            *reinterpret_cast<double4*>(sl + 4) = make_double4(s1[2], s2[2], s1[3], s2[3]);
            if (weighted) {
#pragma unroll
                for (int v = 0; v < EAGCN_MAX_VIEWS; ++v) da[v] += (v == k) ? dak : 0.0;
            }
        }
    }
    if (weighted && !APPLY) {
#pragma unroll
        for (int v = 0; v < EAGCN_MAX_VIEWS; ++v) {
            const double t = wave_sum(da[v]);
            if ((threadIdx.x & 63) == 0 && t != 0.0) atomicAdd(&da_s[v], t);
        }
        __syncthreads();
        if (threadIdx.x < EAGCN_MAX_VIEWS)
            a.slab_da[((size_t)blockIdx.y * gridDim.x + blockIdx.x) * EAGCN_MAX_VIEWS + threadIdx.x] = da_s[threadIdx.x];
    }
}

template <int L>
__global__ __launch_bounds__(256) void bn_bwd_finalize_kernel(const double* __restrict__ slab,
                                                               const double* __restrict__ slab_da, int nslab,
                                                               int fp, double M, int training,
                                                               const float* __restrict__ bn, ViewCols vc,
                                                               GradPtrs gp, float* __restrict__ cc, const int32_t* __restrict__ meta, int nvirt,
                                                               int batch_B, int da_chunks, int da_stride,
                                                               const double* __restrict__ gsum, double* __restrict__ zero, int nzero) {
    if (blockIdx.x == 0 && zero)
        for (int i = threadIdx.x; i < nzero; i += blockDim.x) zero[i] = 0.0;
    if (meta[EAGCN_META_NLOG] > 0) M = (double)batch_B * (double)meta[EAGCN_META_NLOG];
    nslab = max(1, min(nslab, (meta[EAGCN_META_T] + nvirt + BWD_ROWS - 1) / BWD_ROWS));
    const int cpr = blockIdx.x * (256 / L) + threadIdx.x / L, sl = threadIdx.x % L;
    const int cp = min(cpr, fp - 1);
    if (blockIdx.x == 0 && gp.dave_w) {
        const int v = threadIdx.x >> 5, l = threadIdx.x & 31;
        double t = 0.0;
        if (v < vc.K)
            for (int y = 0; y < da_chunks; ++y)
                for (int s = l; s < nslab; s += 32) t += slab_da[((size_t)y * da_stride + s) * EAGCN_MAX_VIEWS + v];
#pragma unroll
        for (int o = 16; o > 0; o >>= 1) t += __shfl_xor(t, o);
        if (v < vc.K && l == 0) gp.dave_w[v] = (float)t;
    }
    double s1, s2;
    slab_sum<L>(slab, nslab, fp, cp, sl, s1, s2);
    if (cpr >= fp || sl != 0) return;
    {
        double g1 = s1, g2 = s2;
        if (gsum) { g1 = gsum[2 * cp]; g2 = gsum[2 * cp + 1]; M = gsum[2 * fp]; }
        cc[cp] = training ? (float)(g1 / M) : 0.0f;
        cc[fp + cp] = training ? (float)(g2 / M) : 0.0f;
    }
    const int k = col_view(vc, cp), f = cp - vc.off[k];
    if (f < vc.width[k]) {
        gp.dgamma[k][f] = (float)s2;
        gp.dbeta[k][f] = (float)s1;
        gp.dbias[k][f] = training ? 0.0f : (float)((double)bn[BN_SC * fp + cp] * s1);
    }
}

__global__ __launch_bounds__(256) void bn_bwd_apply_kernel(eagcn_batch bt, int fp, const float* __restrict__ Y, int ldy,
                                                            const float* __restrict__ bn,
                                                            const float* __restrict__ cc, float* __restrict__ dH) {
    const uint32_t g4 = fp / 4;
    const uint32_t total = (uint32_t)dev_rows(bt) * g4;
    for (uint32_t e = blockIdx.x * blockDim.x + threadIdx.x; e < total; e += gridDim.x * blockDim.x) {
        const int r = (int)(e / g4), c = (int)(e - (uint32_t)r * g4) * 4;
        const float4 y = *reinterpret_cast<const float4*>(Y + (size_t)r * ldy + c);
        float4 d = *reinterpret_cast<float4*>(dH + (size_t)r * fp + c);
        const float4 sc = *reinterpret_cast<const float4*>(bn + BN_SC * fp + c);
        const float4 mu = *reinterpret_cast<const float4*>(bn + BN_MU * fp + c);
        const float4 iv = *reinterpret_cast<const float4*>(bn + BN_INV * fp + c);
        const float4 c1 = *reinterpret_cast<const float4*>(cc + c);
        const float4 c2 = *reinterpret_cast<const float4*>(cc + fp + c);
        d.x = sc.x * (d.x - c1.x - (y.x - mu.x) * iv.x * c2.x);
        d.y = sc.y * (d.y - c1.y - (y.y - mu.y) * iv.y * c2.y);
        d.z = sc.z * (d.z - c1.z - (y.z - mu.z) * iv.z * c2.z);
        d.w = sc.w * (d.w - c1.w - (y.w - mu.w) * iv.w * c2.w);
        *reinterpret_cast<float4*>(dH + (size_t)r * fp + c) = d;
    }
}

__global__ __launch_bounds__(256) void unpack_grads_kernel(GradPtrs gp, ParamPtrs pp, ViewCols vc, ColMapD in,
                                                            int ld_in, int fp, const float* __restrict__ dWcat,
                                                            int nsplit, size_t slab, double* __restrict__ datt,
                                                            int nedge, const float* __restrict__ rsig, int wblocks,
                                                            const int32_t* __restrict__ meta, int xk_G, int edge_drain, int bx_per, int bx_wide) {
    nedge = nedge < 0 ? -nedge : min(nedge, (meta[EAGCN_META_T] + 15) / 16);
    const int bxm = bx_wide ? BX3W_BM : BX3_BM, bxn = bx_wide ? BX3W_BN : BX3_BN;
    nsplit = nsplit < 0 ? bx3_used_splits_wave(-nsplit, meta[EAGCN_META_T], ((ld_in + bxm - 1) / bxm) * ((fp + bxn - 1) / bxn),
                                          bx_per > 0 ? ((meta[EAGCN_META_T] + bxm - 1) / bxm) * ((ld_in + bxn - 1) / bxn) : 0, max(1, (fp + 31) >> 5), bx_per)
                        : max(1, min(nsplit, meta[EAGCN_META_T] >> 7));
    if ((int)blockIdx.x < wblocks) {
        const int tid = blockIdx.x * blockDim.x + threadIdx.x;
        if (xk_G > 0) {
            const int e = tid;
            if (e >= ld_in * fp) return;
            const int ip = e / fp, cp = e % fp;
            const int k = col_view(vc, cp), f = cp - vc.off[k];
            const int fi = packed_to_exact(in, ip);
            if (fi < 0 || f >= vc.width[k]) return;
            const int T = meta[EAGCN_META_T];
            G3Plan pl;
            g3_plan((T + 63) / 64, (ld_in + 63) / 64, max(1, (fp + 15) / 16), ((ld_in + 63) / 64) * ((fp + 63) / 64),
                    max(1, (T + 15) / 16), xk_G, pl);
            float v[G3_XSEG];
#pragma unroll
            for (int x = 0; x < G3_XSEG; ++x) v[x] = pl.c[x + 1] > pl.c[x] ? dWcat[(size_t)x * slab + e] : 0.0f;
            float t = 0.0f;
#pragma unroll
            for (int x = 0; x < G3_XSEG; ++x) t += v[x];
            gp.dW[k][(size_t)fi * vc.width[k] + f] = T > 0 ? t : 0.0f;
            return;
        }
        const int sub = tid & 3;
        const int e = (tid >> 2) * 4;
        if (e >= ld_in * fp) return;
        const int ip = e / fp, cp = e % fp;
        const int k = col_view(vc, cp), f = cp - vc.off[k];
        const int fi = packed_to_exact(in, ip);
        if (fi < 0 || f >= vc.width[k]) return;
        float4 s0 = make_float4(0.f, 0.f, 0.f, 0.f), s1 = s0;
        int z = sub;
#pragma unroll 4
        for (; z + 4 < nsplit; z += 8) {
            const float4 a0 = *reinterpret_cast<const float4*>(dWcat + (size_t)z * slab + e);
            const float4 a1 = *reinterpret_cast<const float4*>(dWcat + (size_t)(z + 4) * slab + e);
            s0.x += a0.x; s0.y += a0.y; s0.z += a0.z; s0.w += a0.w;
            s1.x += a1.x; s1.y += a1.y; s1.z += a1.z; s1.w += a1.w;
        }
        if (z < nsplit) {
            const float4 a0 = *reinterpret_cast<const float4*>(dWcat + (size_t)z * slab + e);
            s0.x += a0.x; s0.y += a0.y; s0.z += a0.z; s0.w += a0.w;
        }
        float t[4] = {s0.x + s1.x, s0.y + s1.y, s0.z + s1.z, s0.w + s1.w};
#pragma unroll
        for (int j = 0; j < 4; ++j) { t[j] += __shfl_xor(t[j], 1); t[j] += __shfl_xor(t[j], 2); }
        const float tv = sub == 0 ? t[0] : sub == 1 ? t[1] : sub == 2 ? t[2] : t[3];
        if (f + sub < vc.width[k]) gp.dW[k][(size_t)fi * vc.width[k] + f + sub] = tv;
        return;
    }
    const int er = ((int)blockIdx.x - wblocks) * 16 + (threadIdx.x >> 4), sl = threadIdx.x & 15;
    const int tot = vc.K * EDGE_SLAB;
    const int e = min(er, tot - 1);
    const int k = e / EDGE_SLAB, c = e % EDGE_SLAB;
    const bool general = pp.rel_vec[k] != nullptr && c != 256;
    double t = 0.0;
    if (!general) {
        for (int z0 = sl; z0 < nedge; z0 += 16 * 8) {
            double v[8];
#pragma unroll
            for (int u = 0; u < 8; ++u) {
                const int z = z0 + 16 * u;
                v[u] = z < nedge ? datt[(size_t)z * tot + e] : 0.0;
            }
#pragma unroll
            for (int u = 0; u < 8; ++u) t += v[u];
            if (edge_drain && er < tot) {
#pragma unroll
                for (int u = 0; u < 8; ++u) {
                    const int z = z0 + 16 * u;
                    if (z < nedge) datt[(size_t)z * tot + e] = 0.0;
                }
            }
        }
    } else if (c >= 1 && c <= pp.rel_c[k]) {
        const float* vec = pp.rel_vec[k];
        const int C = pp.rel_c[k], D = pp.channels[k];
        for (int z = sl; z < nedge; z += 16)
            for (int code = 1; code <= D; ++code)
                t += datt[(size_t)z * tot + k * EDGE_SLAB + code] * (double)vec[(size_t)(code - 1) * C + (c - 1)];
    }
#pragma unroll
    for (int o = 8; o > 0; o >>= 1) t += __shfl_xor(t, o);
    if (er >= tot || sl != 0) return;
    if (c == 256) {
        const double r = (double)rsig[k];
        gp.dself_r[k][0] = (float)(t * r * (1.0 - r));
    } else if (c >= 1 && c <= (pp.rel_vec[k] ? pp.rel_c[k] : pp.channels[k])) {
        gp.datt_w[k][c - 1] = (float)t;
    }
}

__global__ __launch_bounds__(256) void attention_dense_kernel(eagcn_batch bt, ParamPtrs pp, float* __restrict__ out) {
    const size_t total = (size_t)bt.K * bt.B * bt.N * bt.N;
    for (size_t e = (size_t)blockIdx.x * blockDim.x + threadIdx.x; e < total;
         e += (size_t)gridDim.x * blockDim.x) {
        const int j = (int)(e % bt.N);
        const size_t kbi = e / bt.N;
        const int k = (int)(kbi / ((size_t)bt.B * bt.N));
        const size_t bi = kbi - (size_t)k * bt.B * bt.N;
        const uint32_t c = bt.deg_bn[bi] > 0 ? bt.code[kbi * bt.ldc + j] : 0u;
        out[e] = (c >= 1 && (int)c <= pp.channels[k]) ? sigmoidf_(att_logit(pp, k, (int)c)) : 0.0f;
    }
}

struct Carver {
    char* base;
    size_t off = 0;
    explicit Carver(void* p) : base((char*)p) {}
    template <typename T>
    T* take(size_t n) {
        T* p = base ? (T*)(base + off) : nullptr;
        off = align256(off + n * sizeof(T));
        return p;
    }
};

struct LayerDims {
    ViewCols vc;
    int fp, ld_in, fin, ldo, gx, gxb, nsplit;
    int gslab;
    size_t wslab;
    size_t wpslab, wtpslab;
    int np;
    int bx_splits;
};
static LayerDims layer_dims(const eagcn_batch* b, const eagcn_layer_params* p) {
    LayerDims d;
    d.vc = view_cols(p);
    d.fp = d.vc.off[p->K];
    d.ld_in = layout_ld(&p->in);
    d.fin = layout_width(&p->in);
    d.ldo = p->structure == EAGCN_STRUCT_CONCATE ? d.fp : pad16(p->width[0]);
    d.gx = agg_grid_x(b);
    d.gslab = std::max(d.gx, lagg_use(b, 0, false, &d.vc) ? lagg_slabs(b) : 0);
    {
        const long by_rows = cdiv(b->T + 1, BWD_ROWS);
        const long by_bytes = std::max<long>(64, (32L << 20) / ((long)d.fp * 16));
        d.gxb = (int)std::max<long>(1, std::min<long>(std::min<long>(by_rows, 2048), by_bytes));
    }
    const int tiles = cdiv(d.ld_in, 64) * cdiv(d.fp, 64);
    d.nsplit = std::max(1, std::min(std::max(1, 1024 / tiles), cdiv(std::max(b->T, 1), 128)));
    d.wslab = (size_t)d.ld_in * d.fp;
    d.wpslab = bx_plane_elems(d.ld_in, d.fp);
    d.wtpslab = bx_plane_elems(d.fp, d.ld_in);
    d.np = (d.ld_in >= 128 && (d.ld_in & 15) == 0 && (d.fp & 15) == 0) ? gemm_planes() : 0;
    d.bx_splits = std::max(1, std::min(std::min(1023, std::max(64, cdiv(std::max(b->T, 1), 4096))), std::max(cdiv(std::max(b->T, 1), 4096), cdiv(std::max(b->T, 1), 256))));
    return d;
}

static bool gemm3_layer(int ld_in) {
    static const bool on = [] { const char* v = getenv("EAGCN_NO_GEMM3"); return !(v && v[0] == '1'); }();
    return on && ld_in >= 128 && gemm_mode() != 2;
}

struct Packed { float *Wcat, *WcatT, *colp, *sig, *rsig; uint16_t *Wp, *WTp; };
struct FwdScratch { void* gws; double* eacc; float *Wcat, *WcatT, *colp, *sig, *rsig; uint16_t *Wp, *WTp; double* stats; double* gsum;
                    uint16_t* xp; };
static size_t carve_packed(void* base, const LayerDims& d, Packed* s) {
    Carver c(base);
    Packed t;
    t.Wcat = c.take<float>(d.wslab);
    t.WcatT = c.take<float>(d.wslab);
    t.colp = c.take<float>((size_t)CP_ROWS * d.fp);
    t.sig = c.take<float>(EAGCN_MAX_VIEWS * 256);
    t.rsig = c.take<float>(EAGCN_MAX_VIEWS);
    t.Wp = c.take<uint16_t>(d.np ? (size_t)d.np * d.wpslab : 1);
    t.WTp = c.take<uint16_t>(d.np ? (size_t)d.np * d.wtpslab : 1);
    if (s) *s = t;
    return c.off;
}
struct BwdScratch {
    void* gws;
    double* eacc;
    float *Wcat, *WcatT, *colp, *sig, *rsig, *dY, *dP, *cc, *dWcat;
    uint16_t *Wp, *WTp;
    double *slab, *slab_da, *datt, *gsum;
    uint16_t *dPp, *xp;
};
static size_t carve_fwd(void* base, const eagcn_batch* b, const LayerDims& d, FwdScratch* s) {
    Carver c(base);
    FwdScratch t;
    t.gws = c.take<char>(gemm3_workspace_bytes());
    t.eacc = (double*)c.take<char>(edge_acc_bytes());
    t.Wcat = c.take<float>(d.wslab);
    t.WcatT = c.take<float>(d.wslab);
    t.colp = c.take<float>((size_t)CP_ROWS * d.fp);
    t.sig = c.take<float>(EAGCN_MAX_VIEWS * 256);
    t.rsig = c.take<float>(EAGCN_MAX_VIEWS);
    t.Wp = c.take<uint16_t>(d.np ? (size_t)d.np * d.wpslab : 1);
    t.WTp = c.take<uint16_t>(d.np ? (size_t)d.np * d.wtpslab : 1);
    t.stats = c.take<double>((size_t)d.gslab * d.fp * 2);
    t.gsum = c.take<double>((size_t)2 * d.fp + 8);
    t.xp = c.take<uint16_t>(d.np ? (size_t)d.np * bx_plane_elems(b->T, d.ld_in) : 1);
    if (s) *s = t;
    return c.off;
}
static size_t carve_bwd(void* base, const eagcn_batch* b, const LayerDims& d, BwdScratch* s) {
    Carver c(base);
    BwdScratch t;
    t.gws = c.take<char>(gemm3_workspace_bytes());
    t.eacc = (double*)c.take<char>(edge_acc_bytes());
    t.Wcat = c.take<float>(d.wslab);
    t.WcatT = c.take<float>(d.wslab);
    t.colp = c.take<float>((size_t)CP_ROWS * d.fp);
    t.sig = c.take<float>(EAGCN_MAX_VIEWS * 256);
    t.rsig = c.take<float>(EAGCN_MAX_VIEWS);
    t.Wp = c.take<uint16_t>(d.np ? (size_t)d.np * d.wpslab : 1);
    t.WTp = c.take<uint16_t>(d.np ? (size_t)d.np * d.wtpslab : 1);
    t.dY = c.take<float>((size_t)std::max(b->T, 1) * d.fp);
    t.dP = c.take<float>((size_t)std::max(b->T, 1) * d.fp);
    t.cc = c.take<float>((size_t)2 * d.fp);
    t.dWcat = c.take<float>(d.wslab * std::max(std::max(d.nsplit, G3_XSEG), d.np ? d.bx_splits : 1));
    t.slab = c.take<double>((size_t)d.gxb * d.fp * 2);
    t.slab_da = c.take<double>((size_t)d.gxb * cdiv(d.fp, 1024) * EAGCN_MAX_VIEWS);
    t.datt = c.take<double>((size_t)edge_grid_x(b) * EAGCN_MAX_VIEWS * EDGE_SLAB);
    t.gsum = c.take<double>((size_t)2 * d.fp + 8);
    t.dPp = c.take<uint16_t>(d.np ? (size_t)d.np * bx_plane_elems(b->T, d.fp) : 1);
    t.xp = c.take<uint16_t>(d.np ? (size_t)d.np * bx_plane_elems(b->T, d.ld_in) : 1);
    if (s) *s = t;
    return c.off;
}

static int check_layer(const eagcn_batch* b, const eagcn_layer_params* p, const char* who) {
    EAGCN_CHECK_ARG(b && p, "%s: null argument", who);
    EAGCN_CHECK_ARG(p->K >= 1 && p->K <= EAGCN_MAX_VIEWS && p->K == b->K,
                    "%s: layer has %d views, batch index has %d", who, p->K, b->K);
    EAGCN_CHECK_ARG(p->structure == EAGCN_STRUCT_CONCATE || p->structure == EAGCN_STRUCT_WEIGHTED,
                    "%s: unknown structure %d", who, p->structure);
    EAGCN_CHECK_ARG(p->in.nseg >= 1 && p->in.nseg <= EAGCN_MAX_SEGS, "%s: bad input layout", who);
    for (int s = 0; s < p->in.nseg; ++s)
        EAGCN_CHECK_ARG(p->in.width[s] >= 1 && p->in.pad[s] >= p->in.width[s] && (p->in.pad[s] % 4) == 0,
                        "%s: input segment %d: width %d pad %d (pad must be a multiple of 4 >= width)", who, s,
                        p->in.width[s], p->in.pad[s]);
    for (int k = 0; k < p->K; ++k) {
        EAGCN_CHECK_ARG(p->width[k] >= 1, "%s: view %d has width %d", who, k, p->width[k]);
        EAGCN_CHECK_ARG(p->att_w[k] && p->self_r[k] && p->W[k] && p->bias[k] && p->gamma[k] && p->beta[k] &&
                            p->run_mean[k] && p->run_var[k], "%s: view %d has a null parameter", who, k);
        if (p->structure == EAGCN_STRUCT_WEIGHTED)
            EAGCN_CHECK_ARG(p->width[k] == p->width[0], "%s: Weighted_sum needs equal view widths", who);
    }
    if (p->structure == EAGCN_STRUCT_WEIGHTED) EAGCN_CHECK_ARG(p->ave_w, "%s: Weighted_sum needs ave_w", who);
    EAGCN_CHECK_ARG(p->dropout >= 0.0f && p->dropout < 1.0f, "%s: dropout %f out of [0,1)", who, p->dropout);
    EAGCN_CHECK_ARG((uint64_t)std::max(b->T, 0) * (uint64_t)view_cols(p).off[p->K] / 4 < (1ull << 32),
                    "%s: %d rows x %d packed columns exceed the 32-bit element index of the BatchNorm passes", who, b->T,
                    view_cols(p).off[p->K]);
    return EAGCN_OK;
}

static ParamPtrs param_ptrs(const eagcn_batch* b, const eagcn_layer_params* p) {
    ParamPtrs pp;
    memset(&pp, 0, sizeof(pp));
    for (int k = 0; k < p->K; ++k) {
        pp.att_w[k] = p->att_w[k]; pp.self_r[k] = p->self_r[k]; pp.W[k] = p->W[k]; pp.bias[k] = p->bias[k];
        pp.gamma[k] = p->gamma[k]; pp.beta[k] = p->beta[k]; pp.run_mean[k] = p->run_mean[k];
        pp.run_var[k] = p->run_var[k]; pp.channels[k] = b->channels[k];
        pp.rel_vec[k] = b->rel_vec[k]; pp.rel_c[k] = b->rel_c[k];
    }
    pp.ave_w = p->structure == EAGCN_STRUCT_WEIGHTED ? p->ave_w : nullptr;
    return pp;
}

static inline int ew_grid(size_t n) { return (int)std::max<size_t>(1, std::min<size_t>((n + 255) / 256, 2048)); }

}

static int apply_launch_(const eagcn_batch* b, const eagcn_layer_params* p, const eagcn_layer_bufs* w, const eagcn::LayerDims& d,
                         const float* colp, hipStream_t s, bool planes_only = false);
#define apply_launch apply_launch_

using namespace eagcn;

extern "C" int eagcn_pad16(int w) { return pad16(w); }
extern "C" int eagcn_layer_fp(const eagcn_layer_params* p) { return view_cols(p).off[p->K]; }
extern "C" int eagcn_layer_out_ld(const eagcn_layer_params* p) {
    return p->structure == EAGCN_STRUCT_CONCATE ? eagcn_layer_fp(p) : pad16(p->width[0]);
}
extern "C" size_t eagcn_layer_packed_bytes(const eagcn_batch* b, const eagcn_layer_params* p) {
    LayerDims d = layer_dims(b, p);
    return carve_packed(nullptr, d, nullptr);
}
extern "C" size_t eagcn_layer_fwd_scratch_bytes(const eagcn_batch* b, const eagcn_layer_params* p) {
    LayerDims d = layer_dims(b, p);
    return carve_fwd(nullptr, b, d, nullptr);
}
extern "C" size_t eagcn_layer_bwd_scratch_bytes(const eagcn_batch* b, const eagcn_layer_params* p) {
    LayerDims d = layer_dims(b, p);
    return carve_bwd(nullptr, b, d, nullptr);
}

extern "C" int eagcn_layer_forward(const eagcn_batch* b, const eagcn_layer_params* p, const eagcn_layer_bufs* w,
                                   void* stream) {
    EAGCN_CHECK_GEMM3("eagcn_layer_forward");
    if (w && w->scratch && w->scratch_bytes >= gemm3_workspace_bytes()) {
        int rc = gemm3_clear_flags(w->scratch, w->scratch_bytes, (hipStream_t)stream);
        if (rc) return rc;
    }
    return layer_forward_impl(b, p, w, stream, false);
}

int eagcn::pack_params_all(const eagcn_batch* b, const eagcn_layer_params* const* ps, void* const* packed,
                           const size_t* packed_bytes, int n, void* stream, const ZeroJob* zj, const HandOff* ho) {
    hipStream_t s = (hipStream_t)stream;
    EAGCN_CHECK_ARG(n >= 1 && n <= 4, "pack_params_all: 1..4 layers");
    PackJob jobs[4];
    size_t wmax = 0;
    for (int l = 0; l < 4; ++l) {
        const int ll = l < n ? l : n - 1;
        int rc = check_layer(b, ps[ll], "eagcn_model_forward");
        if (rc) return rc;
        const LayerDims d = layer_dims(b, ps[ll]);
        Packed pk;
        const size_t pneed = carve_packed(packed[ll], d, &pk);
        if (pneed > packed_bytes[ll]) {
            set_error("pack_params_all: packed buffer of layer %d too small (%zu < %zu)", ll, packed_bytes[ll], pneed);
            return EAGCN_ERR_SCRATCH;
        }
        jobs[l].pp = param_ptrs(b, ps[ll]); jobs[l].vc = d.vc; jobs[l].in = make_colmap(&ps[ll]->in);
        jobs[l].ld_in = d.ld_in; jobs[l].fp = d.fp;
        jobs[l].Wcat = pk.Wcat; jobs[l].WcatT = pk.WcatT; jobs[l].colp = pk.colp; jobs[l].sig = pk.sig; jobs[l].rsig = pk.rsig;
        jobs[l].wp = BxOut{d.np ? pk.Wp : nullptr, d.wpslab, d.np, d.ld_in};
        jobs[l].wtp = BxOut{d.np ? pk.WTp : nullptr, d.wtpslab, d.np, d.fp};
        if (l < n) wmax = std::max(wmax, d.wslab);
    }
    PackJobs pj{jobs[0], jobs[1], jobs[2], jobs[3]};
    ProfScope ps_(PROF_PACK, s);
    const ZeroJob none{nullptr, 0, nullptr, 0};
    const HandOff noho{nullptr, nullptr, nullptr, 0};
    pack_params_multi_kernel<<<dim3(ew_grid(wmax), n), 256, 0, s>>>(pj, zj ? *zj : none, ho ? *ho : noho);
    EAGCN_LAUNCH_CHECK();
    return EAGCN_OK;
}

int eagcn::layer_forward_impl(const eagcn_batch* b, const eagcn_layer_params* p, const eagcn_layer_bufs* w,
                              void* stream, bool prepacked, bool skip_apply, bool planes_only) {
    hipStream_t s = (hipStream_t)stream;
    int rc = check_layer(b, p, "eagcn_layer_forward");
    if (rc) return rc;
    EAGCN_CHECK_ARG(w && w->bn && w->xout && w->pad_row && w->scratch, "eagcn_layer_forward: null buffer");
    EAGCN_CHECK_ARG(b->T == 0 || ((w->x || w->x_planes) && w->P && w->Y && w->rscale), "eagcn_layer_forward: null activation buffer");
    EAGCN_CHECK_ARG(!planes_only || (w->xout_planes && gemm_planes()), "eagcn_layer_forward: planes-only output without plane images");
    const LayerDims d = layer_dims(b, p);
    FwdScratch sc;
    const size_t need = carve_fwd(w->scratch, b, d, &sc);
    if (need > w->scratch_bytes) {
        set_error("eagcn_layer_forward: scratch too small (%zu < %zu)", w->scratch_bytes, need);
        return EAGCN_ERR_SCRATCH;
    }
    const ParamPtrs pp = param_ptrs(b, p);
    const ColMapD in = make_colmap(&p->in);
    if (w->packed) {
        Packed pk;
        const size_t pneed = carve_packed(w->packed, d, &pk);
        if (pneed > w->packed_bytes) {
            set_error("eagcn_layer_forward: packed buffer too small (%zu < %zu)", w->packed_bytes, pneed);
            return EAGCN_ERR_SCRATCH;
        }
        sc.Wcat = pk.Wcat; sc.WcatT = pk.WcatT; sc.colp = pk.colp; sc.sig = pk.sig; sc.rsig = pk.rsig;
        sc.Wp = pk.Wp; sc.WTp = pk.WTp;
    }
    EAGCN_CHECK_ARG(!prepacked || w->packed, "eagcn_layer_forward: prepacked parameters need the packed block");
    if (!prepacked) {
        ProfScope ps(PROF_PACK, s);
        pack_params_kernel<<<ew_grid(d.wslab), 256, 0, s>>>(pp, d.vc, in, d.ld_in, d.fp, sc.Wcat, sc.WcatT, sc.colp, sc.sig, sc.rsig,
                                                            BxOut{d.np ? sc.Wp : nullptr, d.wpslab, d.np, d.ld_in},
                                                            BxOut{d.np ? sc.WTp : nullptr, d.wtpslab, d.np, d.fp});
    }
    EAGCN_LAUNCH_CHECK();
    double fsum = 0.0;
    for (int k = 0; k < p->K; ++k) fsum += p->width[k];
    const double gemm_work = 2.0 * (double)b->T * (double)d.fin * fsum;
    int nslab = 0, tiles_per_wg = agg_ksplit(b) ? 1 : 4;
    if (b->T > 0) {
        GemmDesc g3{0, 1, b->T, d.fp, d.ld_in, w->x, d.ld_in, sc.WcatT, d.ld_in, w->P, d.fp, 1, 0, gemm_work};
        g3.M_dev = b->meta + EAGCN_META_T;
        BxProb bp;
        memset(&bp, 0, sizeof(bp));
        if (d.np) {
            const size_t xstride = bx_plane_elems(b->T, d.ld_in);
            const uint16_t* xp = w->x_planes;
            if (!xp) {
                EAGCN_CHECK_ARG(w->x, "eagcn_layer_forward: neither an fp32 input nor its plane images");
                rc = launch_bx3_split(w->x, b->T, b->meta + EAGCN_META_T, d.ld_in, sc.xp, xstride, b->T, d.np, s);
                if (rc) return rc;
                xp = sc.xp;
            }
            bp.A = BxPlanes{xp, xstride, d.ld_in, b->T}; bp.B = BxPlanes{sc.WTp, d.wtpslab, d.ld_in, d.fp}; bp.C = w->P; bp.ldc = d.fp;
            bp.M = b->T; bp.N = d.fp; bp.K = d.ld_in; bp.M_dev = b->meta + EAGCN_META_T; bp.tn = 0; bp.splits = 1;
        }
        if (d.np && bx3_ok(bp)) {
            rc = launch_bx3(bp, nullptr, d.np, s, gemm_work, PROF_GEMM, bx3_pick_wide(bp, nullptr, b->t_hint));
        } else if (!w->x) {
            set_error("eagcn_layer_forward: the input exists as plane images only and the plane product does not apply");
            return EAGCN_ERR_ARG;
        } else if (gemm3_layer(d.ld_in) && gemm3_ok(g3)) {
            rc = launch_gemm3(g3, nullptr, sc.gws, gemm3_workspace_bytes(), s);
        } else {
            GemmDesc g{0, 0, b->T, d.fp, d.ld_in, w->x, d.ld_in, sc.Wcat, d.fp, w->P, d.fp, 1, 0, gemm_work};
            g.M_dev = b->meta + EAGCN_META_T;
            rc = launch_gemm(g, s);
        }
        if (rc) return rc;
        {
            AggArgs a;
            a.bt = *b; a.vc = d.vc; a.src = w->P; a.lds = d.fp; a.dst = w->Y; a.ldd = d.fp;
            a.sig = sc.sig; a.rsig = sc.rsig; a.rscale = w->rscale; a.stats = sc.stats; a.nchunk = 1;
            if (lagg_use(b, 0, false, &d.vc)) {
                rc = launch_lagg_fwd(a, s);
                nslab = lagg_slabs(b);
                tiles_per_wg = -1;
            } else {
                rc = launch_agg(a, false, s);
                nslab = d.gx;
            }
            if (rc) return rc;
        }
    }
    const double M = (double)b->B * (double)b->N;
    {
    ProfScope psbn(PROF_BN, s);
    if (w->stats_hook && p->training) {
        if (nslab > 64) bn_stats_sum_kernel<64><<<cdiv(d.fp, 4), 256, 0, s>>>(sc.stats, nslab, d.fp, M, sc.gsum, b->meta, 1, tiles_per_wg, 0, b->B);
        else bn_stats_sum_kernel<16><<<cdiv(d.fp, 16), 256, 0, s>>>(sc.stats, nslab, d.fp, M, sc.gsum, b->meta, 1, tiles_per_wg, 0, b->B);
        EAGCN_LAUNCH_CHECK();
        if (w->stats_hook(sc.gsum, 2 * d.fp + 1, stream, w->stats_user)) {
            set_error("eagcn_layer_forward: the sync-BatchNorm all-reduce hook failed");
            return EAGCN_ERR_HIP;
        }
        bn_finalize_kernel<16><<<cdiv(d.fp, 16), 256, 0, s>>>(sc.gsum, 1, d.fp, M, p->training, p->bn_eps, p->bn_momentum, sc.colp,
                                                                pp, d.vc, w->bn, b->meta, 0, b->B, sc.gsum + 2 * d.fp);
    } else if (nslab > 64)
        bn_finalize_kernel<64><<<cdiv(d.fp, 4), 256, 0, s>>>(sc.stats, nslab, d.fp, M, p->training, p->bn_eps,
                                                               p->bn_momentum, sc.colp, pp, d.vc, w->bn, b->meta, tiles_per_wg, b->B, nullptr);
    else
        bn_finalize_kernel<16><<<cdiv(d.fp, 16), 256, 0, s>>>(sc.stats, nslab, d.fp, M, p->training, p->bn_eps,
                                                                p->bn_momentum, sc.colp, pp, d.vc, w->bn, b->meta, tiles_per_wg, b->B, nullptr);
    EAGCN_LAUNCH_CHECK();
    }
    if (skip_apply) return EAGCN_OK;
    return apply_launch(b, p, w, d, sc.colp, s, planes_only);
}

bool eagcn::layer_reads_planes_only(const eagcn_batch* b, const eagcn_layer_params* p, bool aux_stream) {
    static const bool on = [] { const char* v = getenv("EAGCN_PLANES_ONLY"); return !(v && v[0] == '0'); }();
    if (!on || aux_stream || !b || !p || b->T <= 0) return false;
    const LayerDims d = layer_dims(b, p);
    if (!d.np) return false;
    const uint16_t* pl = reinterpret_cast<const uint16_t*>(static_cast<uintptr_t>(4096));
    float* fo = reinterpret_cast<float*>(static_cast<uintptr_t>(4096));
    const size_t xstride = bx_plane_elems(b->T, d.ld_in), pstride = bx_plane_elems(b->T, d.fp);
    BxProb bp, bx, bw;
    memset(&bp, 0, sizeof(bp)); memset(&bx, 0, sizeof(bx)); memset(&bw, 0, sizeof(bw));
    bp.A = BxPlanes{pl, xstride, d.ld_in, b->T}; bp.B = BxPlanes{pl, d.wtpslab, d.ld_in, d.fp}; bp.C = fo; bp.ldc = d.fp;
    bp.M = b->T; bp.N = d.fp; bp.K = d.ld_in; bp.M_dev = b->meta + EAGCN_META_T; bp.tn = 0; bp.splits = 1;
    bx.A = BxPlanes{pl, pstride, d.fp, b->T}; bx.B = BxPlanes{pl, d.wpslab, d.fp, d.ld_in}; bx.C = fo; bx.ldc = d.ld_in;
    bx.M = b->T; bx.N = d.ld_in; bx.K = d.fp; bx.M_dev = b->meta + EAGCN_META_T; bx.tn = 0; bx.splits = 1;
    bw.A = BxPlanes{pl, xstride, d.ld_in, b->T}; bw.B = BxPlanes{pl, pstride, d.fp, b->T};
    bw.C = fo; bw.ldc = d.fp; bw.M = d.ld_in; bw.N = d.fp; bw.K = b->T; bw.K_dev = b->meta + EAGCN_META_T; bw.tn = 1;
    bw.splits = d.bx_splits; bw.slab = d.wslab;
    return bx3_ok(bp) && bx3_ok(bw) && bx3_ok(bx);
}

int eagcn::layer_apply_impl(const eagcn_batch* b, const eagcn_layer_params* p, const eagcn_layer_bufs* w, void* stream) {
    EAGCN_CHECK_ARG(b && p && w && w->bn && w->xout && w->pad_row && w->packed, "layer_apply: null buffer");
    const LayerDims d = layer_dims(b, p);
    Packed pk;
    EAGCN_CHECK_ARG(carve_packed(w->packed, d, &pk) <= w->packed_bytes, "layer_apply: packed buffer too small");
    return apply_launch(b, p, w, d, pk.colp, (hipStream_t)stream);
}

static int apply_launch_(const eagcn_batch* b, const eagcn_layer_params* p, const eagcn_layer_bufs* w, const LayerDims& d,
                         const float* colp, hipStream_t s, bool planes_only) {
    ProfScope psbn(PROF_BN, s);
    ApplyArgs aa;
    aa.bt = *b; aa.vc = d.vc; aa.structure = p->structure; aa.fp = d.fp; aa.Y = w->Y; aa.ldy = d.fp;
    aa.bn = w->bn; aa.colp = colp; aa.out = w->xout; aa.ldo = d.ldo; aa.pad_row = w->pad_row;
    aa.do_drop = (p->training && p->dropout > 0.0f) ? 1 : 0;
    aa.thr = (uint32_t)std::min(4294967295.0, (double)p->dropout * 4294967296.0);
    aa.inv_keep = 1.0f / (1.0f - p->dropout);
    aa.seed = p->seed;
    aa.seed_dev = p->seed_dev;
    aa.planes = BxOut{gemm_planes() ? w->xout_planes : nullptr, bx_plane_elems(b->T, d.ldo), gemm_planes(), b->T};
    if (planes_only && aa.planes.p) aa.out = nullptr;
    static const int map_env = [] { const char* v = getenv("EAGCN_BN_APPLY_MAP"); return v ? atoi(v) : -1; }();
    aa.tile_map = map_env >= 0 ? map_env : (aa.planes.p ? 1 : 0);
    const size_t nthr = aa.tile_map ? (size_t)cdiv(std::max(b->T, 1), 8) * cdiv(d.ldo, 32) * 64 : (size_t)std::max(b->T, 1) * d.ldo / 4;
    bn_apply_kernel<<<ew_grid(nthr), 256, 0, s>>>(aa);
    EAGCN_LAUNCH_CHECK();
    return EAGCN_OK;
}

static bool lagg_fuses_bn() {
    static const bool on = [] { const char* v = getenv("EAGCN_LAGG_FUSE_BN"); return !(v && v[0] == '0'); }();
    return on;
}
static bool bn_bwd_two_pass(bool weighted) {
    static const int force = [] { const char* v = getenv("EAGCN_BWD_STORE_DH"); return v ? (v[0] == '1' ? 1 : 0) : -1; }();
    return force < 0 ? weighted : force == 0;
}
static void launch_bn_bwd_pass(bool apply, bool wt, bool dg, bool dr, dim3 grid, const BwdArgs& ba, hipStream_t s) {
#define EAGCN_BWD(W, G, D) do { if (apply) bn_bwd_reduce_kernel<W, G, D, true><<<grid, 256, 0, s>>>(ba); \
                                else bn_bwd_reduce_kernel<W, G, D, false><<<grid, 256, 0, s>>>(ba); } while (0)
    if (wt) { if (dg) { if (dr) EAGCN_BWD(true, true, true); else EAGCN_BWD(true, true, false); }
              else    { if (dr) EAGCN_BWD(true, false, true); else EAGCN_BWD(true, false, false); } }
    else    { if (dg) { if (dr) EAGCN_BWD(false, true, true); else EAGCN_BWD(false, true, false); }
              else    { if (dr) EAGCN_BWD(false, false, true); else EAGCN_BWD(false, false, false); } }
#undef EAGCN_BWD
}

extern "C" int eagcn_layer_backward(const eagcn_batch* b, const eagcn_layer_params* p, const eagcn_layer_bufs* w,
                                    const float* dxout, const float* dpad_row, float* dx,
                                    const eagcn_layer_grads* g, void* stream) {
    EAGCN_CHECK_GEMM3("eagcn_layer_backward");
    if (w && w->scratch && w->scratch_bytes >= gemm3_workspace_bytes()) {
        int rc = gemm3_clear_flags(w->scratch, w->scratch_bytes, (hipStream_t)stream);
        if (rc) return rc;
    }
    return layer_backward_impl(b, p, w, dxout, nullptr, dpad_row, dx, g, stream);
}

int eagcn::layer_backward_impl(const eagcn_batch* b, const eagcn_layer_params* p, const eagcn_layer_bufs* w,
                               const float* dxout, const ReadoutGrad* rg, const float* dpad_row, float* dx,
                               const eagcn_layer_grads* g, void* stream, bool dpad_views, const ZeroJob* zero_after,
                               const EdgeDrain* drain_in, EdgeDrain* drain_out, bool input_only) {
    if (drain_out) drain_out->eacc = nullptr;
    hipStream_t s = (hipStream_t)stream;
    int rc = check_layer(b, p, "eagcn_layer_backward");
    if (rc) return rc;
    EAGCN_CHECK_ARG(w && (g || input_only) && w->bn && w->scratch, "eagcn_layer_backward: null buffer");
    EAGCN_CHECK_ARG(!input_only || (dx && !drain_in), "eagcn_layer_backward: the input-only form needs dx and takes no edge reduction");
    EAGCN_CHECK_ARG(b->T == 0 || ((dxout || rg) && (input_only || w->x || w->x_planes) && w->P && w->Y && w->rscale),
                    "eagcn_layer_backward: null activation buffer");
    if (!input_only)
        for (int k = 0; k < p->K; ++k)
            EAGCN_CHECK_ARG(g->dW[k] && g->dbias[k] && g->dgamma[k] && g->dbeta[k] && g->datt_w[k] && g->dself_r[k],
                            "eagcn_layer_backward: view %d has a null gradient buffer", k);
    const LayerDims d = layer_dims(b, p);
    BwdScratch sc;
    const size_t need = carve_bwd(w->scratch, b, d, &sc);
    if (need > w->scratch_bytes) {
        set_error("eagcn_layer_backward: scratch too small (%zu < %zu)", w->scratch_bytes, need);
        return EAGCN_ERR_SCRATCH;
    }
    const ParamPtrs pp = param_ptrs(b, p);
    GradPtrs gp;
    memset(&gp, 0, sizeof(gp));
    if (input_only) {
        EAGCN_CHECK_ARG(d.wslab >= (size_t)3 * d.fp + EAGCN_MAX_VIEWS, "eagcn_layer_backward: no room for the discarded BatchNorm gradients");
        for (int k = 0; k < p->K; ++k) {
            gp.dgamma[k] = sc.dWcat + d.vc.off[k];
            gp.dbeta[k] = sc.dWcat + d.fp + d.vc.off[k];
            gp.dbias[k] = sc.dWcat + 2 * d.fp + d.vc.off[k];
        }
        gp.dave_w = p->structure == EAGCN_STRUCT_WEIGHTED ? sc.dWcat + 3 * d.fp : nullptr;
    } else {
        for (int k = 0; k < p->K; ++k) {
            gp.dW[k] = g->dW[k]; gp.dbias[k] = g->dbias[k]; gp.dgamma[k] = g->dgamma[k]; gp.dbeta[k] = g->dbeta[k];
            gp.datt_w[k] = g->datt_w[k]; gp.dself_r[k] = g->dself_r[k];
        }
        gp.dave_w = p->structure == EAGCN_STRUCT_WEIGHTED ? g->dave_w : nullptr;
    }
    const ColMapD in = make_colmap(&p->in);
    if (w->packed) {
        Packed pk;
        const size_t pneed = carve_packed(w->packed, d, &pk);
        if (pneed > w->packed_bytes) {
            set_error("eagcn_layer_backward: packed buffer too small (%zu < %zu)", w->packed_bytes, pneed);
            return EAGCN_ERR_SCRATCH;
        }
        sc.Wcat = pk.Wcat; sc.WcatT = pk.WcatT; sc.colp = pk.colp; sc.sig = pk.sig; sc.rsig = pk.rsig;
        sc.Wp = pk.Wp; sc.WTp = pk.WTp;
    } else {
        ProfScope ps(PROF_PACK, s);
        pack_params_kernel<<<ew_grid(d.wslab), 256, 0, s>>>(pp, d.vc, in, d.ld_in, d.fp, sc.Wcat, sc.WcatT, sc.colp, sc.sig, sc.rsig,
                                                            BxOut{d.np ? sc.Wp : nullptr, d.wpslab, d.np, d.ld_in},
                                                            BxOut{d.np ? sc.WTp : nullptr, d.wtpslab, d.np, d.fp});
    }
    EAGCN_LAUNCH_CHECK();
    double fsum = 0.0;
    for (int k = 0; k < p->K; ++k) fsum += p->width[k];
    const double gemm_work = 2.0 * (double)b->T * (double)d.fin * fsum;

    BwdArgs ba;
    ba.meta = b->meta; ba.Tcap = b->T; ba.row_mol = b->row_mol; ba.row_m = b->row_m;
    ba.vc = d.vc; ba.structure = p->structure; ba.fp = d.fp;
    ba.nvirt = (dpad_row && p->structure == EAGCN_STRUCT_WEIGHTED) ? 1 : 0;
    ba.dxout = dxout; ba.ldo = d.ldo; ba.dpad = dpad_row; ba.dpad_views = dpad_views ? 1 : 0;
    if (rg) ba.rg = *rg; else memset(&ba.rg, 0, sizeof(ba.rg)); ba.Y = w->Y; ba.ldy = d.fp; ba.bn = w->bn;
    ba.colp = sc.colp; ba.dH = sc.dY; ba.slab = sc.slab; ba.slab_da = sc.slab_da;
    ba.do_drop = (p->training && p->dropout > 0.0f) ? 1 : 0;
    ba.thr = (uint32_t)std::min(4294967295.0, (double)p->dropout * 4294967296.0);
    ba.inv_keep = 1.0f / (1.0f - p->dropout);
    ba.seed = p->seed;
    ba.seed_dev = p->seed_dev;
    ba.zero = zero_after ? zero_after->d : nullptr;
    ba.nzero = zero_after ? zero_after->nd : 0;
    if (drain_in && drain_in->eacc) ba.drain = *drain_in; else memset(&ba.drain, 0, sizeof(ba.drain));
    const int rows = b->T + ba.nvirt;
    const int gxb = std::max(1, std::min(rows, d.gxb));
    bool fused_bn_apply = false, fused_w_apply = false, w_rows = false, fused_c_apply = false;
    bool lagg_bwd = false;
    {
        static const bool edge_atomic0 = [] { const char* v = getenv("EAGCN_EDGE_SLABS"); return !(v && v[0] == '1'); }();
        bool general0 = false;
        for (int k = 0; k < p->K; ++k) general0 = general0 || pp.rel_vec[k] != nullptr;
        const bool wt0 = p->structure == EAGCN_STRUCT_WEIGHTED;
        const bool absorbs = lagg_fuses_bn() && (!bn_bwd_two_pass(wt0) || (wt0 && lagg_wfuse()));
        lagg_bwd = b->T > 0 && edge_atomic0 && !general0 && lagg_use(b, 1, absorbs);
        if (input_only) lagg_bwd = b->T > 0 && lagg_use(b, 1, true);
    }
    const double M = (double)b->B * (double)b->N;
    const bool eval_in = input_only && !p->training;
    if (eval_in) {
        const bool wt = p->structure == EAGCN_STRUCT_WEIGHTED, dg = ba.rg.dg != nullptr;
        if (b->T > 0 && lagg_bwd) {
            if (dg) {
                rc = launch_readout_bwd_rows(b, ba.rg, d.ldo, sc.dY, s);
                if (rc) return rc;
                w_rows = true;
            }
            if (wt) fused_w_apply = true; else fused_c_apply = true;
        } else if (b->T > 0) {
            rc = zero_fill(sc.cc, (size_t)2 * d.fp * sizeof(float), s);
            if (rc) return rc;
            ba.cc = sc.cc;
            launch_bn_bwd_pass(true, wt, dg, false, dim3(std::max(1, std::min(b->T, d.gxb)), cdiv(d.fp, 1024)), ba, s);
            EAGCN_LAUNCH_CHECK();
        }
        if (zero_after && zero_after->nd) { rc = zero_fill(zero_after->d, (size_t)zero_after->nd * sizeof(double), s); if (rc) return rc; }
    } else {
        ProfScope ps(PROF_BN, s);
        const int ny = cdiv(d.fp, 1024);
        {
            const bool wt = p->structure == EAGCN_STRUCT_WEIGHTED, dr = ba.do_drop != 0;
            bool dg = ba.rg.dg != nullptr;
            const dim3 grid(gxb, ny);
            ba.cc = sc.cc;
            ba.store_dh = bn_bwd_two_pass(wt) ? 0 : 1;
            static const bool rows_first = [] { const char* v = getenv("EAGCN_W_ROWS_FIRST"); return !(v && v[0] == '0'); }();
            if (wt && dg && b->T > 0 && bn_bwd_two_pass(wt) && lagg_bwd && lagg_fuses_bn() && lagg_wfuse() && rows_first) {
                rc = launch_readout_bwd_rows(b, ba.rg, d.ldo, sc.dY, s);
                if (rc) return rc;
                w_rows = true;
                ba.dxout = sc.dY;
                dg = false;
            }
            launch_bn_bwd_pass(false, wt, dg, dr, grid, ba, s);
        }
        EAGCN_LAUNCH_CHECK();
        const double* gsum = nullptr;
        if (w->stats_hook && p->training) {
            if (gxb > 64) bn_stats_sum_kernel<64><<<cdiv(d.fp, 4), 256, 0, s>>>(sc.slab, gxb, d.fp, M, sc.gsum, b->meta, 2, 0, ba.nvirt, b->B);
            else bn_stats_sum_kernel<16><<<cdiv(d.fp, 16), 256, 0, s>>>(sc.slab, gxb, d.fp, M, sc.gsum, b->meta, 2, 0, ba.nvirt, b->B);
            EAGCN_LAUNCH_CHECK();
            if (w->stats_hook(sc.gsum, 2 * d.fp + 1, stream, w->stats_user)) {
                set_error("eagcn_layer_backward: the sync-BatchNorm all-reduce hook failed");
                return EAGCN_ERR_HIP;
            }
            gsum = sc.gsum;
        }
        if (gxb > 64)
            bn_bwd_finalize_kernel<64><<<cdiv(d.fp, 4), 256, 0, s>>>(sc.slab, sc.slab_da, gxb, d.fp, M, p->training, w->bn,
                                                                       d.vc, gp, sc.cc, b->meta, ba.nvirt, b->B, ny, gxb, gsum, ba.zero, ba.nzero);
        else
            bn_bwd_finalize_kernel<16><<<cdiv(d.fp, 16), 256, 0, s>>>(sc.slab, sc.slab_da, gxb, d.fp, M, p->training, w->bn,
                                                                        d.vc, gp, sc.cc, b->meta, ba.nvirt, b->B, ny, gxb, gsum, ba.zero, ba.nzero);
        EAGCN_LAUNCH_CHECK();
        if (b->T > 0) {
            const bool wt = p->structure == EAGCN_STRUCT_WEIGHTED, dg = ba.rg.dg != nullptr, dr = ba.do_drop != 0;
            if (bn_bwd_two_pass(wt) && wt && lagg_bwd && lagg_fuses_bn() && lagg_wfuse()) {
                fused_w_apply = true;
                if (dg && !w_rows) {
                    rc = launch_readout_bwd_rows(b, ba.rg, d.ldo, sc.dY, s);
                    if (rc) return rc;
                }
            } else if (bn_bwd_two_pass(wt)) launch_bn_bwd_pass(true, wt, dg, dr, dim3(std::max(1, std::min(b->T, d.gxb)), ny), ba, s);
            else if (lagg_bwd && lagg_fuses_bn()) fused_bn_apply = true;
            else bn_bwd_apply_kernel<<<ew_grid((size_t)b->T * d.fp / 4), 256, 0, s>>>(*b, d.fp, w->Y, d.fp, w->bn, sc.cc, sc.dY);
            EAGCN_LAUNCH_CHECK();
        }
    }
    int nsplit = 0, nedge = 0, xk_G = 0;
    bool bx_slabs = false;
    int bx_per = 0;
    int bx_wide = 0;
    hipStream_t side = w->aux_stream ? (hipStream_t)w->aux_stream : s;
    const bool forked = side != s;
    if (b->T > 0) {
        AggArgs a;
        a.bt = *b; a.vc = d.vc; a.src = sc.dY; a.lds = d.fp; a.dst = sc.dP; a.ldd = d.fp;
        a.sig = sc.sig; a.rsig = sc.rsig; a.rscale = w->rscale; a.stats = nullptr; a.nchunk = 1;
        const size_t xstride = bx_plane_elems(b->T, d.ld_in), pstride = bx_plane_elems(b->T, d.fp);
        BxProb bx, bw;
        memset(&bx, 0, sizeof(bx));
        memset(&bw, 0, sizeof(bw));
        bool use_bx = false;
        if (d.np && !w->aux_stream) {
            bx.A = BxPlanes{sc.dPp, pstride, d.fp, b->T}; bx.B = BxPlanes{sc.Wp, d.wpslab, d.fp, d.ld_in}; bx.C = dx; bx.ldc = d.ld_in;
            bx.M = b->T; bx.N = d.ld_in; bx.K = d.fp; bx.M_dev = b->meta + EAGCN_META_T; bx.tn = 0; bx.splits = 1;
            bw.A = BxPlanes{w->x_planes ? w->x_planes : sc.xp, xstride, d.ld_in, b->T}; bw.B = BxPlanes{sc.dPp, pstride, d.fp, b->T};
            bw.C = sc.dWcat; bw.ldc = d.fp; bw.M = d.ld_in; bw.N = d.fp; bw.K = b->T; bw.K_dev = b->meta + EAGCN_META_T; bw.tn = 1;
            bw.splits = d.bx_splits; bw.slab = d.wslab;
            use_bx = bx3_ok(bw) && (!dx || bx3_ok(bx));
        }
        if (use_bx) {
            a.planes = BxOut{sc.dPp, pstride, d.np, b->T};
            if (!w->x_planes && !input_only) {
                rc = launch_bx3_split(w->x, b->T, b->meta + EAGCN_META_T, d.ld_in, sc.xp, xstride, b->T, d.np, s);
                if (rc) return rc;
            }
        } else if (!w->x && !input_only) {
            set_error("eagcn_layer_backward: the input exists as plane images only and the plane products do not apply");
            return EAGCN_ERR_ARG;
        }
        EdgeArgs e;
        e.bt = *b; e.vc = d.vc; e.dY = sc.dY; e.Y = w->Y; e.P = w->P; e.ld = d.fp; e.sig = sc.sig;
        e.rsig = sc.rsig; e.rscale = w->rscale; e.datt = sc.datt; e.atomic = 0;
        static const bool edge_atomic = [] { const char* v = getenv("EAGCN_EDGE_SLABS"); return !(v && v[0] == '1'); }();
        bool general_rel = false;
        for (int k = 0; k < p->K; ++k) general_rel = general_rel || pp.rel_vec[k] != nullptr;
        if (edge_atomic && !general_rel) { e.datt = sc.eacc; e.atomic = 1; }
        static const bool colaunch = [] { const char* v = getenv("EAGCN_NO_COLAUNCH"); return !(v && v[0] == '1'); }();
        nedge = e.atomic ? -EDGE_COPIES : edge_grid_x(b);
        if (input_only) {
            if (lagg_bwd) {
                if (fused_bn_apply || fused_w_apply || fused_c_apply) { a.bn_tab = w->bn; a.bn_cc = eval_in ? nullptr : sc.cc; a.bn_fp = d.fp; }
                if (fused_w_apply || fused_c_apply) {
                    a.src = (ba.rg.dg || w_rows) ? sc.dY : dxout; a.lds = d.ldo;
                    a.w_aw = sc.colp + (size_t)CP_AVEW * d.fp;
                    a.w_rowm = fused_c_apply;
                    a.w_drop = ba.do_drop; a.w_thr = ba.thr; a.w_inv_keep = ba.inv_keep; a.w_seed = ba.seed; a.w_seed_dev = ba.seed_dev;
                }
                rc = launch_lagg_bwd(a, e, s, false);
            } else {
                rc = launch_agg(a, true, s);
            }
            if (rc) return rc;
            if (use_bx) {
                rc = launch_bx3(bx, nullptr, d.np, s, gemm_work, PROF_GEMM, bx3_pick_wide(bx, nullptr, b->t_hint));
            } else {
                GemmDesc gx{0, 1, b->T, d.ld_in, d.fp, sc.dP, d.fp, sc.Wcat, d.fp, dx, d.ld_in, 1, 0, gemm_work};
                gx.M_dev = b->meta + EAGCN_META_T;
                rc = launch_gemm(gx, s);
            }
            return rc;
        }
        if (lagg_bwd && e.atomic) {
            if (fused_bn_apply || fused_w_apply) { a.bn_tab = w->bn; a.bn_cc = sc.cc; a.bn_fp = d.fp; }
            if (fused_w_apply) {
                a.src = (ba.rg.dg || w_rows) ? sc.dY : dxout; a.lds = d.ldo;
                a.w_aw = sc.colp + (size_t)CP_AVEW * d.fp;
                a.w_drop = ba.do_drop; a.w_thr = ba.thr; a.w_inv_keep = ba.inv_keep; a.w_seed = ba.seed; a.w_seed_dev = ba.seed_dev;
            }
            rc = launch_lagg_bwd(a, e, s);
            if (rc) return rc;
        } else if (!forked && colaunch) {
            rc = launch_agg_edge(a, e, s);
            if (rc) return rc;
        } else {
            if (forked) { rc = stream_after(side, s); if (rc) return rc; }
            rc = launch_edge_grad(e, side);
            if (rc) return rc;
            rc = launch_agg(a, true, s);
            if (rc) return rc;
        }
        if (forked) { rc = stream_after(side, s); if (rc) return rc; }
        nsplit = d.nsplit;
        GemmDesc gw{1, 0, d.ld_in, d.fp, b->T, w->x, d.ld_in, sc.dP, d.fp, sc.dWcat, d.fp, nsplit, d.wslab, gemm_work};
        gw.K_dev = b->meta + EAGCN_META_T;
        GemmDesc gx{0, 1, b->T, d.ld_in, d.fp, sc.dP, d.fp, sc.Wcat, d.fp, dx, d.ld_in, 1, 0, gemm_work};
        gx.M_dev = b->meta + EAGCN_META_T;
        static const bool pair = [] { const char* v = getenv("EAGCN_NO_PAIR"); return !(v && v[0] == '1'); }();
        static const bool use3 = [] { const char* v = getenv("EAGCN_NO_GEMM3"); return !(v && v[0] == '1'); }();
        DwScatter dsc;
        for (int k = 0; k < EAGCN_MAX_VIEWS; ++k) dsc.dW[k] = gp.dW[k];
        dsc.vc = d.vc;
        dsc.in = in;
        if (use_bx) {
            bx_wide = dx ? bx3_pick_wide(bx, &bw, b->t_hint) : bx3_pick_wide(bw, nullptr, b->t_hint);
            rc = dx ? launch_bx3(bx, &bw, d.np, s, 2.0 * gemm_work, PROF_GEMM_PAIR, bx_wide) : launch_bx3(bw, nullptr, d.np, s, gemm_work, PROF_GEMM, bx_wide);
            if (rc) return rc;
            nsplit = d.bx_splits;
            bx_slabs = true;
            bx_per = (dx && bx3_pair_policy()) ? std::max(1, bx3_grid() >> 3) : 0;
        } else if (use3 && !forked && dx && gemm3_layer(d.ld_in) && gemm3_ok(gw) && gemm3_ok(gx) && gemm3_xk_enabled()) {
            rc = launch_gemm3_pair(gx, gw, nullptr, sc.gws, gemm3_workspace_bytes(), s, d.wslab);
            if (rc) return rc;
            nsplit = 1;
            xk_G = gemm3_grid();
        } else if (use3 && !forked && dx && gemm3_layer(d.ld_in) && gemm3_ok(gw) && gemm3_ok(gx)) {
            rc = launch_gemm3_pair(gx, gw, &dsc, sc.gws, gemm3_workspace_bytes(), s);
            if (rc) return rc;
            nsplit = 0;
        } else if (dx && !forked && colaunch && pair) {
            rc = launch_gemm_pair(gx, gw, s);
            if (rc) return rc;
        } else {
            rc = launch_gemm(gw, side);
            if (rc) return rc;
            if (dx) { rc = launch_gemm(gx, s); if (rc) return rc; }
        }
    }
    if (b->T == 0 && input_only) return EAGCN_OK;
    if (b->T == 0) {
        for (int k = 0; k < p->K; ++k)
            { int rcz = zero_fill(gp.dW[k], (size_t)d.fin * p->width[k] * sizeof(float), side); if (rcz) return rcz; }
    }
    {
        const int wblocks = nsplit > 0 ? cdiv((int)d.wslab, 256) : 0;
        double* edge_src = nedge == -EDGE_COPIES ? sc.eacc : sc.datt;
        const int edge_drain = edge_src == sc.eacc ? 1 : 0;
        static const bool defer_env = [] { const char* v = getenv("EAGCN_NO_EDGE_DEFER"); return !(v && v[0] == '1'); }();
        if (defer_env && drain_out && edge_drain && wblocks == 0 && !forked && b->T > 0) {
            drain_out->eacc = sc.eacc; drain_out->K = p->K; drain_out->rsig = sc.rsig;
            for (int k = 0; k < EAGCN_MAX_VIEWS; ++k) {
                drain_out->datt_w[k] = gp.datt_w[k]; drain_out->dself_r[k] = gp.dself_r[k]; drain_out->channels[k] = pp.channels[k];
            }
            return EAGCN_OK;
        }
        ProfScope psu(PROF_PACK, side);
        unpack_grads_kernel<<<wblocks + cdiv(p->K * EDGE_SLAB, 16), 256, 0, side>>>(gp, pp, d.vc, in, d.ld_in, d.fp, sc.dWcat,
                                                                                    bx_slabs ? -nsplit : nsplit, d.wslab, edge_src, nedge, sc.rsig,
                                                                                    wblocks, b->meta, xk_G, edge_drain, bx_per, bx_wide);
        EAGCN_LAUNCH_CHECK();
    }
    if (forked) { rc = stream_after(s, side); if (rc) return rc; }
    return EAGCN_OK;
}

extern "C" int eagcn_attention_dense(const eagcn_batch* b, const eagcn_layer_params* p, float* out, void* stream) {
    hipStream_t s = (hipStream_t)stream;
    EAGCN_CHECK_ARG(b && p && out, "eagcn_attention_dense: null argument");
    EAGCN_CHECK_ARG(p->K == b->K, "eagcn_attention_dense: view count mismatch");
    EAGCN_CHECK_ARG(b->code, "eagcn_attention_dense: batch has no code map");
    ParamPtrs pp;
    memset(&pp, 0, sizeof(pp));
    for (int k = 0; k < p->K; ++k) {
        EAGCN_CHECK_ARG(p->att_w[k], "eagcn_attention_dense: view %d has no attention weight", k);
        pp.att_w[k] = p->att_w[k];
        pp.channels[k] = b->channels[k];
        pp.rel_vec[k] = b->rel_vec[k]; pp.rel_c[k] = b->rel_c[k];
    }
    const size_t total = (size_t)b->K * b->B * b->N * b->N;
    attention_dense_kernel<<<ew_grid(total), 256, 0, s>>>(*b, pp, out);
    EAGCN_LAUNCH_CHECK();
    return EAGCN_OK;
}
```

include/eagcn_hip.h:

```cpp
#ifndef EAGCN_HIP_H
#define EAGCN_HIP_H

#include <stddef.h>
#include <stdint.h>

#ifdef __cplusplus
extern "C" {
#endif

#define EAGCN_MAX_VIEWS 8
#define EAGCN_MAX_SEGS 8
#define EAGCN_MAX_CHANNELS 255
#define EAGCN_STRUCT_CONCATE 0
#define EAGCN_STRUCT_WEIGHTED 1

#define EAGCN_OK 0
#define EAGCN_ERR_ARG (-1)
#define EAGCN_ERR_HIP (-2)
#define EAGCN_ERR_SCRATCH (-3)

#define EAGCN_META_T 0
#define EAGCN_META_NMAX 1
#define EAGCN_META_NTILES 2
#define EAGCN_META_BAD_ADJ 3
// ... 217 lines not shown

int eagcn_stream_signal_flag(uint32_t* flag, void* stream);
int eagcn_stream_wait_flag(uint32_t* flag, double budget_seconds, void* stream);
int eagcn_stream_wait_timeouts(void);
void eagcn_stream_wait_reset(void);

int eagcn_stream_wait_counter(const uint32_t* counter, uint32_t value, void* stream);

size_t eagcn_model_saved_bytes(const eagcn_batch* b, const eagcn_model* m);
size_t eagcn_model_scratch_bytes(const eagcn_batch* b, const eagcn_model* m);
int eagcn_model_atom_rep(const eagcn_batch* b, const eagcn_model* m, size_t* xout_offset,
                         size_t* pad_row_offset, int* ld);
int eagcn_model_atom_rep_materialize(const eagcn_batch* b, const eagcn_model* m, void* saved, size_t saved_bytes, void* stream);
int eagcn_model_pack_input(const eagcn_batch* b, const eagcn_model* m, const float* afm, void* saved,
                           size_t saved_bytes, void* stream);
int eagcn_model_forward(const eagcn_batch* b, const eagcn_model* m, const float* afm, const int64_t* size,
                        void* saved, size_t saved_bytes, void* scratch, size_t scratch_bytes, float* out,
                        float* graph_rep, void* stream);
int eagcn_model_backward(const eagcn_batch* b, const eagcn_model* m, const int64_t* size, void* saved,
                         size_t saved_bytes, void* scratch, size_t scratch_bytes, const float* dout,
                         const float* dgraph_rep, const eagcn_layer_grads* lg, const eagcn_head_grads* hg,
                         void* stream);

int eagcn_model_backward_range(const eagcn_batch* b, const eagcn_model* m, const int64_t* size, void* saved,
                               size_t saved_bytes, void* scratch, size_t scratch_bytes, const float* dout,
                               const float* dgraph_rep, const eagcn_layer_grads* lg, const eagcn_head_grads* hg,
                               int with_head, int layer_hi, int layer_lo, void* stream);

size_t eagcn_model_input_scratch_bytes(const eagcn_batch* b, const eagcn_model* m);
int eagcn_model_backward_input(const eagcn_batch* b, const eagcn_model* m, const int64_t* size, void* saved,
                               size_t saved_bytes, void* scratch, size_t scratch_bytes, const float* dout,
                               const float* dgraph_rep, const eagcn_layer_grads* lg, const eagcn_head_grads* hg,
                               float* dafm, void* stream);

float eagcn_attr_alpha(int step, int steps);
float eagcn_attr_weight(int steps);
size_t eagcn_attr_acc_elems(const eagcn_batch* b, const eagcn_model* m);
int eagcn_attr_pack_input(const eagcn_batch* b, const eagcn_model* m, const float* afm, const float* baseline, float alpha,
                          void* saved, size_t saved_bytes, void* stream);
int eagcn_attr_step(const eagcn_batch* b, const eagcn_model* m, const int64_t* size, void* saved, size_t saved_bytes,
                    void* scratch, size_t scratch_bytes, const float* dout, const float* dgraph_rep, float weight, int first,
                    float* acc, void* stream);
int eagcn_attr_finalize(const eagcn_batch* b, const eagcn_model* m, const float* afm, const float* baseline, const float* acc,
                        float* attr, float* score, void* stream);

typedef struct eagcn_step_loss {
    int32_t kind;
    const float* labels;
    const float* class_weight;
    float* loss;
    const float* scale;
    float* dout;
} eagcn_step_loss;
int eagcn_model_forward_step(const eagcn_batch* b, const eagcn_model* m, const float* afm, const int64_t* size,
                             void* saved, size_t saved_bytes, void* scratch, size_t scratch_bytes, float* out,
                             float* graph_rep, const eagcn_step_loss* loss, const float* dgraph_rep,
                             const eagcn_head_grads* hg, void* stream);

size_t eagcn_head_saved_bytes(const eagcn_head_params* h, int B);
size_t eagcn_head_scratch_bytes(const eagcn_head_params* h, int B);
int eagcn_head_forward(const eagcn_head_params* h, int B, int training, uint64_t seed, const uint64_t* seed_dev, const float* g,
                       void* saved, size_t saved_bytes, void* scratch, size_t scratch_bytes, float* out, float* graph_rep,
                       void* stream);
int eagcn_head_backward(const eagcn_head_params* h, int B, int training, uint64_t seed, const uint64_t* seed_dev, const float* g,
                        void* saved, size_t saved_bytes, void* scratch, size_t scratch_bytes, const float* dout,
                        const float* dgraph_rep, const eagcn_head_grads* hg, float* dg, void* stream);

int eagcn_bce_loss(const float* logits, const float* labels, const float* class_weight, int B, int T,
                   float* loss, float* dlogits, void* stream);
int eagcn_mse_loss(const float* pred, const float* target, int n, float* loss, float* dpred, void* stream);

int eagcn_adam_step(float* param, const float* grad, float* exp_avg, float* exp_avg_sq, int64_t n, const double* hyper_dev,
                    int64_t* step_dev, uint32_t* ticket_dev, void* stream);

int eagcn_eval_append(const float* logits, const float* labels, int B, int T, int classification, float* scores,
                      float* targets, uint8_t* valid, int64_t row_offset, void* stream);

int eagcn_set_gemm_mode(int mode);

size_t eagcn_bx3_plane_elems(int rows_cap, int ld);
int eagcn_bx3_split(const float* x, int rows, int ld, uint16_t* planes, size_t plane_stride, int rows_cap, int np, void* stream);
int eagcn_bx3_used_splits(int splits, int M, int N, int K);
int eagcn_set_bx3_wide(int mode);
int eagcn_bx3_pair_used_splits(int splits, int M, int N, int K, int M0, int N0, int K0);
int eagcn_gemm_bx3(int tn, int M, int N, int K, const uint16_t* A, size_t a_pstride, int lda, int a_rows, const uint16_t* B,
                   size_t b_pstride, int ldb, int b_rows, float* C, int ldc, int splits, size_t slab, int np, void* stream);
int eagcn_gemm_bx3_pair(int M0, int N0, int K0, const uint16_t* A0, size_t a0_pstride, int lda0, int a0_rows, const uint16_t* B0,
                        size_t b0_pstride, int ldb0, int b0_rows, float* C0, int ldc0, int M1, int N1, int K1, const uint16_t* A1,
                        size_t a1_pstride, int lda1, int a1_rows, const uint16_t* B1, size_t b1_pstride, int ldb1, int b1_rows,
                        float* C1, int ldc1, int splits, size_t slab, int np, void* stream);

int eagcn_gemm_f32(int ta, int tb, int M, int N, int K, const float* A, int lda, const float* B,
                   int ldb, float* C, int ldc, void* stream);
int eagcn_gemm_f32_dev(int ta, int tb, int M, int N, int K, const float* A, int lda, const float* B,
                       int ldb, float* C, int ldc, const int32_t* extent_dev, int which, void* stream);

size_t eagcn_gemm_sk_workspace_bytes(void);
int eagcn_gemm_f32_sk(int ta, int tb, int M, int N, int K, const float* A, int lda, const float* B, int ldb, float* C,
                      int ldc, void* workspace, size_t workspace_bytes, void* stream);
int eagcn_gemm_pair_sk(int M0, int N0, int K0, const float* A0, int lda0, const float* B0, int ldb0, float* C0, int ldc0,
                       int M1, int N1, int K1, const float* A1, int lda1, const float* B1, int ldb1, float* C1, int ldc1,
                       void* workspace, size_t workspace_bytes, void* stream);
int eagcn_gemm_pair_sk_slabs(int M0, int N0, int K0, const float* A0, int lda0, const float* B0, int ldb0, float* C0, int ldc0,
                             int M1, int N1, int K1, const float* A1, int lda1, const float* B1, int ldb1, float* C1, int ldc1,
                             size_t slab, void* workspace, size_t workspace_bytes, void* stream);
int eagcn_gemm_sk_plan(int M0, int N0, int K0, int M1, int N1, int K1, int wgs, int* a, int* c);
int eagcn_gemm_sk_timeouts(void);
int eagcn_gemm_sk_failed(void);
void eagcn_gemm_sk_reset_failed(void);
void eagcn_gemm_sk_inject_failure(void);

void eagcn_prof_enable(int on);
void eagcn_prof_reset(void);
int eagcn_prof_ntags(void);
const char* eagcn_prof_tag_name(int tag);
int eagcn_prof_read(int tag, double* total_ms, double* work, int64_t* launches);

#ifdef __cplusplus
}
#endif
#endif
```

Before: 711,000.

## Fold parameter packing and gradient unpack into neighbouring kernels as rider blocks

Packing of layers 1..3 parameters moves out of the multi-layer pack kernel and runs as extra rider blocks appended to layer 0's BN-apply launch. In backward, the per-layer gradient unpack kernel is deferred and run as extra blocks inside the next layer's BN backward pass. A dedicated dW scratch region sized across layers keeps the deferred data alive. Both folds are controlled by a chain_folds mask. The aim is fewer kernel launches and less serialization on the critical path, at the cost of larger kernel argument blocks and more complex scratch lifetimes.

```diff
diff --git a/eagcn_amd/_lib.py b/eagcn_amd/_lib.py
--- a/eagcn_amd/_lib.py
+++ b/eagcn_amd/_lib.py
@@ -139,6 +139,7 @@
     'eagcn_agg_wants_bond_lists_for': (C.c_int, [C.c_int, C.c_int, C.c_int]),
     'eagcn_bx3_used_splits': (C.c_int, [C.c_int, C.c_int, C.c_int, C.c_int]),
     'eagcn_set_bx3_wide': (C.c_int, [C.c_int]),
+    'eagcn_set_chain_folds': (C.c_int, [C.c_int]),
     'eagcn_bx3_pair_used_splits': (C.c_int, [C.c_int] * 7),
     'eagcn_bx3_plane_elems': (C.c_size_t, [C.c_int, C.c_int]),
     'eagcn_bx3_split': (C.c_int, [_fp, C.c_int, C.c_int, _fp, C.c_size_t, C.c_int, C.c_int, _fp]),
diff --git a/eagcn_amd/csrc/head.hip b/eagcn_amd/csrc/head.hip
--- a/eagcn_amd/csrc/head.hip
+++ b/eagcn_amd/csrc/head.hip
@@ -142,6 +142,7 @@
     double* hws;
     double* hsb;
     void* layer; size_t layer_bytes;
+    size_t dw_region;
 };
 static size_t carve_scratch(void* base, const eagcn_batch* b, const eagcn_model* m, ModelScratch* out) {
     Carver2 c(base);
@@ -161,10 +162,12 @@
                                                              (size_t)h->n_den2 * h->nclass) : 1);
     int ldmax = 0;
     size_t lbytes = 0;
+    s.dw_region = 0;
+    for (int l = 0; l < m->n_layers; ++l) s.dw_region = std::max(s.dw_region, layer_dw_floats(b, &m->layer[l]));
     for (int l = 0; l < m->n_layers; ++l) {
         ldmax = std::max(ldmax, eagcn_layer_out_ld(&m->layer[l]));
         lbytes = std::max(lbytes, eagcn_layer_fwd_scratch_bytes(b, &m->layer[l]));
-        lbytes = std::max(lbytes, eagcn_layer_bwd_scratch_bytes(b, &m->layer[l]));
+        lbytes = std::max(lbytes, layer_bwd_scratch_bytes(b, &m->layer[l], s.dw_region));
     }
     s.dxa = c.take<float>(T * ldmax);
     s.dxb = c.take<float>(T * ldmax);
@@ -341,7 +344,9 @@
     EAGCN_CHECK_ARG(carve_scratch(scratch, b, m, &sc) <= scratch_bytes, "%s: scratch too small", who);
     const eagcn_head_params* h = &m->head;
     HandOff ho{m->start_signal, m->wait_flag, wait_err_word(), 200000000ull};
-    if (!m->input_packed && (m->wait_flag || m->start_signal)) {
+    bool general_rel = false;
+    for (int k = 0; k < b->K; ++k) general_rel = general_rel || b->rel_vec[k] != nullptr;
+    if ((!m->input_packed || general_rel) && (m->wait_flag || m->start_signal)) {
         handoff_kernel<<<1, 64, 0, s>>>(ho);
         EAGCN_LAUNCH_CHECK();
         ho.start = nullptr; ho.flag = nullptr;
@@ -351,12 +356,14 @@
     if (!m->input_packed)
         RC(eagcn_pack_rows(b, afm, layout_width(&m->layer[0].in), &m->layer[0].in, sv.x0, stream));
     const float* x = sv.x0;
+    PackRiders riders;
+    riders.n = 0;
     {
         const eagcn_layer_params* ps[4];
         void* pk[4];
         size_t pkb[4];
         for (int l = 0; l < m->n_layers; ++l) { ps[l] = &m->layer[l]; pk[l] = sv.L[l].packed; pkb[l] = sv.L[l].packed_bytes; }
-        RC(pack_params_all(b, ps, pk, pkb, m->n_layers, stream, &zj, &ho));
+        RC(pack_params_all(b, ps, pk, pkb, m->n_layers, stream, &zj, &ho, &riders));
     }
     for (int l = 0; l < m->n_layers; ++l) {
         LayerSaved& L = sv.L[l];
@@ -367,7 +374,8 @@
         w.stats_hook = m->stats_hook; w.stats_user = m->stats_user;
         w.x_planes = l > 0 ? sv.L[l - 1].xout_planes : nullptr; w.xout_planes = L.xout_planes;
         const bool po = hidden_planes_only(b, m, sv, l);
-        RC(layer_forward_impl(b, &m->layer[l], &w, stream, true, l == m->n_layers - 1 && fused_readout(m), po));
+        RC(layer_forward_impl(b, &m->layer[l], &w, stream, true, l == m->n_layers - 1 && fused_readout(m), po,
+                              l == 0 ? &riders : nullptr));
         x = po ? nullptr : L.xout;
     }
     const eagcn_layer_params* last = &m->layer[m->n_layers - 1];
@@ -647,9 +655,9 @@
     memset(&rgd, 0, sizeof(rgd));
     rgd.dg = sc.dg; rgd.F = F; rgd.size = size; rgd.mode = m->molfp_mode; rgd.map = make_colmap(&lay);
     const int top_l = m->n_layers - 1;
-    EdgeDrain pend_in, pend_out;
-    pend_in.eacc = nullptr;
-    pend_out.eacc = nullptr;
+    DeferredGrads pend_in, pend_out;
+    pend_in.edge.eacc = nullptr; pend_in.unpack.nblocks = 0;
+    pend_out.edge.eacc = nullptr; pend_out.unpack.nblocks = 0;
     for (int l = layer_hi; l >= layer_lo; --l) {
         const int t = top_l - l;
         float* cur = (t & 1) ? sc.dxb : sc.dxa;
@@ -667,9 +675,10 @@
         const float* dpad = (weighted && top) ? sc.dpad : nullptr;
         RC(layer_backward_impl(b, &m->layer[l], &w, top ? nullptr : cur, top ? &rgd : nullptr, dpad,
                                l > 0 ? other : dx0, input_only ? nullptr : &lg[l], stream, top && sampled, top ? &zb : nullptr,
-                               pend_in.eacc ? &pend_in : nullptr, (l > layer_lo && !input_only) ? &pend_out : nullptr, input_only));
+                               (pend_in.edge.eacc || pend_in.unpack.nblocks) ? &pend_in : nullptr,
+                               (l > layer_lo && !input_only) ? &pend_out : nullptr, input_only, sc.dw_region));
         pend_in = pend_out;
-        if (l == layer_lo) pend_in.eacc = nullptr;
+        if (l == layer_lo) { pend_in.edge.eacc = nullptr; pend_in.unpack.nblocks = 0; }
     }
     if (forked) RC(stream_after(s, side));
     return EAGCN_OK;
diff --git a/eagcn_amd/csrc/kernels.h b/eagcn_amd/csrc/kernels.h
--- a/eagcn_amd/csrc/kernels.h
+++ b/eagcn_amd/csrc/kernels.h
@@ -198,16 +198,55 @@
 int head_bwd(const HeadBwd& a, hipStream_t s);
 int head_gbn_bwd(const HeadGbn& a, hipStream_t s);
 
+struct ParamPtrs {
+    const float* att_w[EAGCN_MAX_VIEWS];
+    const float* self_r[EAGCN_MAX_VIEWS];
+    const float* W[EAGCN_MAX_VIEWS];
+    const float* bias[EAGCN_MAX_VIEWS];
+    const float* gamma[EAGCN_MAX_VIEWS];
+    const float* beta[EAGCN_MAX_VIEWS];
+    float* run_mean[EAGCN_MAX_VIEWS];
+    float* run_var[EAGCN_MAX_VIEWS];
+    const float* ave_w;
+    int channels[EAGCN_MAX_VIEWS];
+    const float* rel_vec[EAGCN_MAX_VIEWS];
+    int rel_c[EAGCN_MAX_VIEWS];
+};
+struct GradPtrs {
+    float* dW[EAGCN_MAX_VIEWS];
+    float* dbias[EAGCN_MAX_VIEWS];
+    float* dgamma[EAGCN_MAX_VIEWS];
+    float* dbeta[EAGCN_MAX_VIEWS];
+    float* datt_w[EAGCN_MAX_VIEWS];
+    float* dself_r[EAGCN_MAX_VIEWS];
+    float* dave_w;
+};
+
 struct EdgeDrain {
     double* eacc; int K;
     float* datt_w[EAGCN_MAX_VIEWS]; float* dself_r[EAGCN_MAX_VIEWS]; int channels[EAGCN_MAX_VIEWS];
     const float* rsig;
 };
+struct UnpackJob {
+    GradPtrs gp; ParamPtrs pp; ViewCols vc; ColMapD in;
+    int ld_in, fp;
+    const float* dWcat; int nsplit; size_t slab;
+    double* datt; int nedge;
+    const float* rsig;
+    int wblocks;
+    const int32_t* meta;
+    int xk_G, edge_drain, bx_per, bx_wide;
+    int nblocks;
+};
+struct DeferredGrads { EdgeDrain edge; UnpackJob unpack; };
+int chain_folds();
 int layer_backward_impl(const eagcn_batch* b, const eagcn_layer_params* p, const eagcn_layer_bufs* w,
                         const float* dxout, const ReadoutGrad* rg, const float* dpad_row, float* dx,
                         const eagcn_layer_grads* g, void* stream, bool dpad_views = false,
-                        const ZeroJob* zero_after = nullptr, const EdgeDrain* drain_in = nullptr, EdgeDrain* drain_out = nullptr,
-                        bool input_only = false);
+                        const ZeroJob* zero_after = nullptr, const DeferredGrads* drain_in = nullptr, DeferredGrads* drain_out = nullptr,
+                        bool input_only = false, size_t dw_region = 0);
+size_t layer_dw_floats(const eagcn_batch* b, const eagcn_layer_params* p);
+size_t layer_bwd_scratch_bytes(const eagcn_batch* b, const eagcn_layer_params* p, size_t dw_region);
 int model_backward_input_packed(const eagcn_batch* b, const eagcn_model* m, const int64_t* size, void* saved, size_t saved_bytes,
                                 void* scratch, size_t scratch_bytes, const float* dout, const float* dgraph_rep,
                                 const eagcn_layer_grads* lg, const eagcn_head_grads* hg, float** dx0, void* stream, const char* who);
@@ -215,11 +254,18 @@
                       float* score, hipStream_t s);
 int model_input_slot(const eagcn_batch* b, const eagcn_model* m, void* saved, size_t saved_bytes, float** x0, const char* who);
 int layer_forward_impl(const eagcn_batch* b, const eagcn_layer_params* p, const eagcn_layer_bufs* w, void* stream,
-                       bool prepacked, bool skip_apply = false, bool planes_only = false);
+                       bool prepacked, bool skip_apply = false, bool planes_only = false, const struct PackRiders* riders = nullptr);
 bool layer_reads_planes_only(const eagcn_batch* b, const eagcn_layer_params* p, bool aux_stream);
 int layer_apply_impl(const eagcn_batch* b, const eagcn_layer_params* p, const eagcn_layer_bufs* w, void* stream);
+struct PackJob {
+    ParamPtrs pp; ViewCols vc; ColMapD in; int ld_in, fp;
+    float *Wcat, *WcatT, *colp, *sig, *rsig;
+    BxOut wp, wtp;
+};
+struct PackRiders { PackJob j1, j2, j3; int n; int nb1, nb2, nb3; };
 int pack_params_all(const eagcn_batch* b, const eagcn_layer_params* const* ps, void* const* packed,
-                    const size_t* packed_bytes, int n, void* stream, const ZeroJob* zj = nullptr, const HandOff* ho = nullptr);
+                    const size_t* packed_bytes, int n, void* stream, const ZeroJob* zj = nullptr, const HandOff* ho = nullptr,
+                    PackRiders* riders = nullptr);
 struct ReadoutBn {
     const float* Y; int ldy;
     const float* bn; int fp;
diff --git a/eagcn_amd/csrc/layer.hip b/eagcn_amd/csrc/layer.hip
--- a/eagcn_amd/csrc/layer.hip
+++ b/eagcn_amd/csrc/layer.hip
@@ -7,20 +7,6 @@
 
 namespace eagcn {
 
-struct ParamPtrs {
-    const float* att_w[EAGCN_MAX_VIEWS];
-    const float* self_r[EAGCN_MAX_VIEWS];
-    const float* W[EAGCN_MAX_VIEWS];
-    const float* bias[EAGCN_MAX_VIEWS];
-    const float* gamma[EAGCN_MAX_VIEWS];
-    const float* beta[EAGCN_MAX_VIEWS];
-    float* run_mean[EAGCN_MAX_VIEWS];
-    float* run_var[EAGCN_MAX_VIEWS];
-    const float* ave_w;
-    int channels[EAGCN_MAX_VIEWS];
-    const float* rel_vec[EAGCN_MAX_VIEWS];
-    int rel_c[EAGCN_MAX_VIEWS];
-};
 __device__ __forceinline__ float att_logit(const ParamPtrs& pp, int k, int c) {
     if (!pp.rel_vec[k]) return pp.att_w[k][c - 1];
     const float* v = pp.rel_vec[k] + (size_t)(c - 1) * pp.rel_c[k];
@@ -28,16 +14,6 @@
     for (int ch = 0; ch < pp.rel_c[k]; ++ch) s = fmaf(pp.att_w[k][ch], v[ch], s);
     return s;
 }
-struct GradPtrs {
-    float* dW[EAGCN_MAX_VIEWS];
-    float* dbias[EAGCN_MAX_VIEWS];
-    float* dgamma[EAGCN_MAX_VIEWS];
-    float* dbeta[EAGCN_MAX_VIEWS];
-    float* datt_w[EAGCN_MAX_VIEWS];
-    float* dself_r[EAGCN_MAX_VIEWS];
-    float* dave_w;
-};
-
 enum { CP_GAMMA = 0, CP_BETA, CP_BIAS, CP_RMEAN, CP_RVAR, CP_AVEW, CP_ROWS = 8 };
 
 __device__ __forceinline__ int col_view(const ViewCols& vc, int cp) {
@@ -59,11 +35,11 @@
 __device__ __forceinline__ void pack_params_body(const ParamPtrs& pp, const ViewCols& vc, const ColMapD& in, int ld_in,
                                                  int fp, float* __restrict__ Wcat, float* __restrict__ WcatT,
                                                  float* __restrict__ colp, float* __restrict__ sig, float* __restrict__ rsig,
-                                                 const BxOut wp = BxOut{nullptr, 0, 0, 0}, const BxOut wtp = BxOut{nullptr, 0, 0, 0}) {
+                                                 const BxOut wp, const BxOut wtp, const int bid, const int nb) {
     __shared__ float tile[32][33];
     const int tx = threadIdx.x & 31, ty = threadIdx.x >> 5;
     const int ntx = (fp + 31) >> 5, nty = (ld_in + 31) >> 5;
-    for (int t = blockIdx.x; t < ntx * nty; t += gridDim.x) {
+    for (int t = bid; t < ntx * nty; t += nb) {
         const int ip0 = (t / ntx) << 5, cp0 = (t % ntx) << 5;
         {
             const int cp = cp0 + tx;
@@ -96,7 +72,7 @@
         }
         __syncthreads();
     }
-    for (int cp = blockIdx.x * blockDim.x + threadIdx.x; cp < fp; cp += gridDim.x * blockDim.x) {
+    for (int cp = bid * blockDim.x + threadIdx.x; cp < fp; cp += nb * blockDim.x) {
         const int k = col_view(vc, cp), f = cp - vc.off[k];
         const bool ok = f < vc.width[k];
         colp[CP_GAMMA * fp + cp] = ok ? pp.gamma[k][f] : 0.0f;
@@ -106,24 +82,22 @@
         colp[CP_RVAR * fp + cp] = ok ? pp.run_var[k][f] : 1.0f;
         colp[CP_AVEW * fp + cp] = pp.ave_w ? pp.ave_w[k] : 1.0f;
     }
-    for (int e = blockIdx.x * blockDim.x + threadIdx.x; e < vc.K * 256; e += gridDim.x * blockDim.x) {
+    for (int e = bid * blockDim.x + threadIdx.x; e < vc.K * 256; e += nb * blockDim.x) {
         const int k = e >> 8, c = e & 255;
         sig[e] = (c >= 1 && c <= pp.channels[k]) ? sigmoidf_(att_logit(pp, k, c)) : 0.0f;
     }
-    if (blockIdx.x == 0 && threadIdx.x < vc.K) rsig[threadIdx.x] = sigmoidf_(pp.self_r[threadIdx.x][0]);
+    if (bid == 0 && threadIdx.x < vc.K) rsig[threadIdx.x] = sigmoidf_(pp.self_r[threadIdx.x][0]);
 }
 __global__ __launch_bounds__(256) void pack_params_kernel(ParamPtrs pp, ViewCols vc, ColMapD in, int ld_in, int fp,
                                                            float* __restrict__ Wcat, float* __restrict__ WcatT,
                                                            float* __restrict__ colp, float* __restrict__ sig,
                                                            float* __restrict__ rsig, BxOut wp, BxOut wtp) {
-    pack_params_body(pp, vc, in, ld_in, fp, Wcat, WcatT, colp, sig, rsig, wp, wtp);
-}
-struct PackJob {
-    ParamPtrs pp; ViewCols vc; ColMapD in; int ld_in, fp;
-    float *Wcat, *WcatT, *colp, *sig, *rsig;
-    BxOut wp, wtp;
-};
+    pack_params_body(pp, vc, in, ld_in, fp, Wcat, WcatT, colp, sig, rsig, wp, wtp, blockIdx.x, gridDim.x);
+}
 struct PackJobs { PackJob j0, j1, j2, j3; };
+__device__ __forceinline__ void pack_job_body(const PackJob& j, int bid, int nb) {
+    pack_params_body(j.pp, j.vc, j.in, j.ld_in, j.fp, j.Wcat, j.WcatT, j.colp, j.sig, j.rsig, j.wp, j.wtp, bid, nb);
+}
 __global__ __launch_bounds__(256) void pack_params_multi_kernel(PackJobs jobs, ZeroJob zj, HandOff ho) {
     if (blockIdx.y == 0) {
         for (int i = blockIdx.x * blockDim.x + threadIdx.x; i < max(zj.nu, zj.nd); i += gridDim.x * blockDim.x) {
@@ -131,10 +105,10 @@
             if (i < zj.nd) zj.d[i] = 0.0;
         }
     }
-    if (blockIdx.y == 0) pack_params_body(jobs.j0.pp, jobs.j0.vc, jobs.j0.in, jobs.j0.ld_in, jobs.j0.fp, jobs.j0.Wcat, jobs.j0.WcatT, jobs.j0.colp, jobs.j0.sig, jobs.j0.rsig, jobs.j0.wp, jobs.j0.wtp);
-    else if (blockIdx.y == 1) pack_params_body(jobs.j1.pp, jobs.j1.vc, jobs.j1.in, jobs.j1.ld_in, jobs.j1.fp, jobs.j1.Wcat, jobs.j1.WcatT, jobs.j1.colp, jobs.j1.sig, jobs.j1.rsig, jobs.j1.wp, jobs.j1.wtp);
-    else if (blockIdx.y == 2) pack_params_body(jobs.j2.pp, jobs.j2.vc, jobs.j2.in, jobs.j2.ld_in, jobs.j2.fp, jobs.j2.Wcat, jobs.j2.WcatT, jobs.j2.colp, jobs.j2.sig, jobs.j2.rsig, jobs.j2.wp, jobs.j2.wtp);
-    else pack_params_body(jobs.j3.pp, jobs.j3.vc, jobs.j3.in, jobs.j3.ld_in, jobs.j3.fp, jobs.j3.Wcat, jobs.j3.WcatT, jobs.j3.colp, jobs.j3.sig, jobs.j3.rsig, jobs.j3.wp, jobs.j3.wtp);
+    if (blockIdx.y == 0) pack_job_body(jobs.j0, blockIdx.x, gridDim.x);
+    else if (blockIdx.y == 1) pack_job_body(jobs.j1, blockIdx.x, gridDim.x);
+    else if (blockIdx.y == 2) pack_job_body(jobs.j2, blockIdx.x, gridDim.x);
+    else pack_job_body(jobs.j3, blockIdx.x, gridDim.x);
     if (blockIdx.x == 0 && blockIdx.y == 0 && threadIdx.x == 0) handoff_body(ho);
 }
 
@@ -231,9 +205,22 @@
     int do_drop; uint32_t thr; float inv_keep; uint64_t seed; const uint64_t* seed_dev;
     BxOut planes;
     int tile_map;
+    PackRiders riders;
+    int nriders;
 };
+static_assert(sizeof(ApplyArgs) <= 4096, "bn_apply_kernel: argument block beyond the 4 KB kernel-argument limit");
 
 __global__ __launch_bounds__(256) void bn_apply_kernel(ApplyArgs a) {
+    const int gx = (int)gridDim.x - a.nriders;
+    if ((int)blockIdx.x >= gx) {
+        int v = (int)blockIdx.x - gx;
+        if (v < a.riders.nb1) { pack_job_body(a.riders.j1, v, a.riders.nb1); return; }
+        v -= a.riders.nb1;
+        if (v < a.riders.nb2) { pack_job_body(a.riders.j2, v, a.riders.nb2); return; }
+        v -= a.riders.nb2;
+        if (v < a.riders.nb3) pack_job_body(a.riders.j3, v, a.riders.nb3);
+        return;
+    }
     const int fp = a.fp;
     const uint64_t seed = a.seed_dev ? *a.seed_dev : a.seed;
     if (blockIdx.x == 0) {
@@ -251,7 +238,7 @@
     if (a.structure == EAGCN_STRUCT_CONCATE) {
         const uint32_t g4 = a.tile_map ? ((uint32_t)(fp + 31) >> 5) : fp / 4;
         const uint32_t total = a.tile_map ? (((uint32_t)T + 7) >> 3) * g4 * 64u : (uint32_t)T * g4;
-        for (uint32_t e = blockIdx.x * blockDim.x + threadIdx.x; e < total; e += gridDim.x * blockDim.x) {
+        for (uint32_t e = blockIdx.x * blockDim.x + threadIdx.x; e < total; e += gx * blockDim.x) {
             int r, c;
             if (a.tile_map) {
                 const uint32_t it = e >> 6, rg = it / g4;
@@ -280,7 +267,7 @@
     } else {
         const uint32_t g4 = a.tile_map ? ((uint32_t)(a.ldo + 31) >> 5) : a.ldo / 4;
         const uint32_t total = a.tile_map ? (((uint32_t)T + 7) >> 3) * g4 * 64u : (uint32_t)T * g4;
-        for (uint32_t e = blockIdx.x * blockDim.x + threadIdx.x; e < total; e += gridDim.x * blockDim.x) {
+        for (uint32_t e = blockIdx.x * blockDim.x + threadIdx.x; e < total; e += gx * blockDim.x) {
             int r, f;
             if (a.tile_map) {
                 const uint32_t it = e >> 6, rg = it / g4;
@@ -338,17 +325,26 @@
     int do_drop; uint32_t thr; float inv_keep; uint64_t seed; const uint64_t* seed_dev;
     double* zero; int nzero;
     EdgeDrain drain;
+    UnpackJob job;
     const float* cc;
     int store_dh;
 };
 
+__device__ __forceinline__ void unpack_grads_body(const UnpackJob& j, const int vb);
 template <bool WEIGHTED, bool DG, bool DROP, bool APPLY>
 __global__ __launch_bounds__(256) void bn_bwd_reduce_kernel(BwdArgs a) {
     __shared__ double da_s[EAGCN_MAX_VIEWS];
+    const int gx = APPLY ? (int)gridDim.x : (int)gridDim.x - a.job.nblocks;
+    if constexpr (!APPLY) {
+        if ((int)blockIdx.x >= gx) {
+            if (blockIdx.y == 0) unpack_grads_body(a.job, (int)blockIdx.x - gx);
+            return;
+        }
+    }
     const uint64_t seed = DROP ? (a.seed_dev ? *a.seed_dev : a.seed) : 0ull;
     const int fp = a.fp, T = min(a.meta[EAGCN_META_T], a.Tcap);
     const int rows = T + (APPLY ? 0 : a.nvirt);
-    const int nwg = max(1, min((int)gridDim.x, (rows + BWD_ROWS - 1) / BWD_ROWS));
+    const int nwg = max(1, min(gx, (rows + BWD_ROWS - 1) / BWD_ROWS));
     if (!APPLY && a.drain.eacc && blockIdx.x == 0 && blockIdx.y == 0) {
         const int K = a.drain.K;
         for (int e = threadIdx.x; e < K * EDGE_SLAB; e += blockDim.x) {
@@ -504,7 +500,7 @@
         }
         __syncthreads();
         if (threadIdx.x < EAGCN_MAX_VIEWS)
-            a.slab_da[((size_t)blockIdx.y * gridDim.x + blockIdx.x) * EAGCN_MAX_VIEWS + threadIdx.x] = da_s[threadIdx.x];
+            a.slab_da[((size_t)blockIdx.y * gx + blockIdx.x) * EAGCN_MAX_VIEWS + threadIdx.x] = da_s[threadIdx.x];
     }
 }
 
@@ -571,18 +567,25 @@
     }
 }
 
-__global__ __launch_bounds__(256) void unpack_grads_kernel(GradPtrs gp, ParamPtrs pp, ViewCols vc, ColMapD in,
-                                                            int ld_in, int fp, const float* __restrict__ dWcat,
-                                                            int nsplit, size_t slab, double* __restrict__ datt,
-                                                            int nedge, const float* __restrict__ rsig, int wblocks,
-                                                            const int32_t* __restrict__ meta, int xk_G, int edge_drain, int bx_per, int bx_wide) {
+__device__ __forceinline__ void unpack_grads_body(const UnpackJob& j, const int vb) {
+    const GradPtrs& gp = j.gp;
+    const ParamPtrs& pp = j.pp;
+    const ViewCols& vc = j.vc;
+    const ColMapD& in = j.in;
+    const int ld_in = j.ld_in, fp = j.fp, wblocks = j.wblocks, xk_G = j.xk_G, edge_drain = j.edge_drain, bx_per = j.bx_per, bx_wide = j.bx_wide;
+    const float* __restrict__ dWcat = j.dWcat;
+    const size_t slab = j.slab;
+    double* __restrict__ datt = j.datt;
+    const float* __restrict__ rsig = j.rsig;
+    const int32_t* __restrict__ meta = j.meta;
+    int nedge = j.nedge, nsplit = j.nsplit;
     nedge = nedge < 0 ? -nedge : min(nedge, (meta[EAGCN_META_T] + 15) / 16);
     const int bxm = bx_wide ? BX3W_BM : BX3_BM, bxn = bx_wide ? BX3W_BN : BX3_BN;
     nsplit = nsplit < 0 ? bx3_used_splits_wave(-nsplit, meta[EAGCN_META_T], ((ld_in + bxm - 1) / bxm) * ((fp + bxn - 1) / bxn),
                                           bx_per > 0 ? ((meta[EAGCN_META_T] + bxm - 1) / bxm) * ((ld_in + bxn - 1) / bxn) : 0, max(1, (fp + 31) >> 5), bx_per)
                         : max(1, min(nsplit, meta[EAGCN_META_T] >> 7));
-    if ((int)blockIdx.x < wblocks) {
-        const int tid = blockIdx.x * blockDim.x + threadIdx.x;
+    if (vb < wblocks) {
+        const int tid = vb * blockDim.x + threadIdx.x;
         if (xk_G > 0) {
             const int e = tid;
             if (e >= ld_in * fp) return;
@@ -630,7 +633,7 @@
         if (f + sub < vc.width[k]) gp.dW[k][(size_t)fi * vc.width[k] + f + sub] = tv;
         return;
     }
-    const int er = ((int)blockIdx.x - wblocks) * 16 + (threadIdx.x >> 4), sl = threadIdx.x & 15;
+    const int er = (vb - wblocks) * 16 + (threadIdx.x >> 4), sl = threadIdx.x & 15;
     const int tot = vc.K * EDGE_SLAB;
     const int e = min(er, tot - 1);
     const int k = e / EDGE_SLAB, c = e % EDGE_SLAB;
@@ -671,6 +674,7 @@
         gp.datt_w[k][c - 1] = (float)t;
     }
 }
+__global__ __launch_bounds__(256) void unpack_grads_kernel(UnpackJob j) { unpack_grads_body(j, (int)blockIdx.x); }
 
 __global__ __launch_bounds__(256) void attention_dense_kernel(eagcn_batch bt, ParamPtrs pp, float* __restrict__ out) {
     const size_t total = (size_t)bt.K * bt.B * bt.N * bt.N;
@@ -777,11 +781,13 @@
     if (s) *s = t;
     return c.off;
 }
-static size_t carve_bwd(void* base, const eagcn_batch* b, const LayerDims& d, BwdScratch* s) {
+static size_t dw_floats(const LayerDims& d) { return d.wslab * std::max(std::max(d.nsplit, G3_XSEG), d.np ? d.bx_splits : 1); }
+static size_t carve_bwd(void* base, const eagcn_batch* b, const LayerDims& d, BwdScratch* s, size_t dw_region = 0) {
     Carver c(base);
     BwdScratch t;
     t.gws = c.take<char>(gemm3_workspace_bytes());
     t.eacc = (double*)c.take<char>(edge_acc_bytes());
+    t.dWcat = c.take<float>(std::max(dw_region, dw_floats(d)));
     t.Wcat = c.take<float>(d.wslab);
     t.WcatT = c.take<float>(d.wslab);
     t.colp = c.take<float>((size_t)CP_ROWS * d.fp);
@@ -792,7 +798,6 @@
     t.dY = c.take<float>((size_t)std::max(b->T, 1) * d.fp);
     t.dP = c.take<float>((size_t)std::max(b->T, 1) * d.fp);
     t.cc = c.take<float>((size_t)2 * d.fp);
-    t.dWcat = c.take<float>(d.wslab * std::max(std::max(d.nsplit, G3_XSEG), d.np ? d.bx_splits : 1));
     t.slab = c.take<double>((size_t)d.gxb * d.fp * 2);
     t.slab_da = c.take<double>((size_t)d.gxb * cdiv(d.fp, 1024) * EAGCN_MAX_VIEWS);
     t.datt = c.take<double>((size_t)edge_grid_x(b) * EAGCN_MAX_VIEWS * EDGE_SLAB);
@@ -847,7 +852,7 @@
 }
 
 static int apply_launch_(const eagcn_batch* b, const eagcn_layer_params* p, const eagcn_layer_bufs* w, const eagcn::LayerDims& d,
-                         const float* colp, hipStream_t s, bool planes_only = false);
+                         const float* colp, hipStream_t s, bool planes_only = false, const eagcn::PackRiders* riders = nullptr);
 #define apply_launch apply_launch_
 
 using namespace eagcn;
@@ -869,6 +874,16 @@
     LayerDims d = layer_dims(b, p);
     return carve_bwd(nullptr, b, d, nullptr);
 }
+
+size_t eagcn::layer_dw_floats(const eagcn_batch* b, const eagcn_layer_params* p) { return dw_floats(layer_dims(b, p)); }
+size_t eagcn::layer_bwd_scratch_bytes(const eagcn_batch* b, const eagcn_layer_params* p, size_t dw_region) {
+    LayerDims d = layer_dims(b, p);
+    return carve_bwd(nullptr, b, d, nullptr, dw_region);
+}
+
+static int g_chain_folds = [] { const char* v = getenv("EAGCN_CHAIN_FOLDS"); return v ? (atoi(v) & 3) : 3; }();
+int eagcn::chain_folds() { return __atomic_load_n(&g_chain_folds, __ATOMIC_RELAXED); }
+extern "C" int eagcn_set_chain_folds(int mask) { return __atomic_exchange_n(&g_chain_folds, mask & 3, __ATOMIC_RELAXED); }
 
 extern "C" int eagcn_layer_forward(const eagcn_batch* b, const eagcn_layer_params* p, const eagcn_layer_bufs* w,
                                    void* stream) {
@@ -881,11 +896,14 @@
 }
 
 int eagcn::pack_params_all(const eagcn_batch* b, const eagcn_layer_params* const* ps, void* const* packed,
-                           const size_t* packed_bytes, int n, void* stream, const ZeroJob* zj, const HandOff* ho) {
+                           const size_t* packed_bytes, int n, void* stream, const ZeroJob* zj, const HandOff* ho,
+                           PackRiders* riders) {
     hipStream_t s = (hipStream_t)stream;
     EAGCN_CHECK_ARG(n >= 1 && n <= 4, "pack_params_all: 1..4 layers");
     PackJob jobs[4];
-    size_t wmax = 0;
+    size_t wmax = 0, w0 = 0;
+    int ntiles[4] = {0, 0, 0, 0};
+    if (riders) riders->n = 0;
     for (int l = 0; l < 4; ++l) {
         const int ll = l < n ? l : n - 1;
         int rc = check_layer(b, ps[ll], "eagcn_model_forward");
@@ -902,19 +920,28 @@
         jobs[l].Wcat = pk.Wcat; jobs[l].WcatT = pk.WcatT; jobs[l].colp = pk.colp; jobs[l].sig = pk.sig; jobs[l].rsig = pk.rsig;
         jobs[l].wp = BxOut{d.np ? pk.Wp : nullptr, d.wpslab, d.np, d.ld_in};
         jobs[l].wtp = BxOut{d.np ? pk.WTp : nullptr, d.wtpslab, d.np, d.fp};
-        if (l < n) wmax = std::max(wmax, d.wslab);
+        if (l < n) { wmax = std::max(wmax, d.wslab); ntiles[l] = cdiv(d.fp, 32) * cdiv(d.ld_in, 32); }
+        if (l == 0) w0 = d.wslab;
+    }
+    int ny = n;
+    if (riders && n > 1 && (chain_folds() & 2)) {
+        riders->j1 = jobs[1]; riders->j2 = jobs[2]; riders->j3 = jobs[3];
+        riders->n = n - 1;
+        riders->nb1 = std::min(ntiles[1], 2048); riders->nb2 = std::min(ntiles[2], 2048); riders->nb3 = std::min(ntiles[3], 2048);
+        wmax = w0;
+        ny = 1;
     }
     PackJobs pj{jobs[0], jobs[1], jobs[2], jobs[3]};
     ProfScope ps_(PROF_PACK, s);
     const ZeroJob none{nullptr, 0, nullptr, 0};
     const HandOff noho{nullptr, nullptr, nullptr, 0};
-    pack_params_multi_kernel<<<dim3(ew_grid(wmax), n), 256, 0, s>>>(pj, zj ? *zj : none, ho ? *ho : noho);
+    pack_params_multi_kernel<<<dim3(ew_grid(wmax), ny), 256, 0, s>>>(pj, zj ? *zj : none, ho ? *ho : noho);
     EAGCN_LAUNCH_CHECK();
     return EAGCN_OK;
 }
 
 int eagcn::layer_forward_impl(const eagcn_batch* b, const eagcn_layer_params* p, const eagcn_layer_bufs* w,
-                              void* stream, bool prepacked, bool skip_apply, bool planes_only) {
+                              void* stream, bool prepacked, bool skip_apply, bool planes_only, const PackRiders* riders) {
     hipStream_t s = (hipStream_t)stream;
     int rc = check_layer(b, p, "eagcn_layer_forward");
     if (rc) return rc;
@@ -1018,8 +1045,9 @@
                                                                 p->bn_momentum, sc.colp, pp, d.vc, w->bn, b->meta, tiles_per_wg, b->B, nullptr);
     EAGCN_LAUNCH_CHECK();
     }
+    EAGCN_CHECK_ARG(!(skip_apply && riders && riders->n), "eagcn_layer_forward: parameter-packing riders need the layer's apply launch");
     if (skip_apply) return EAGCN_OK;
-    return apply_launch(b, p, w, d, sc.colp, s, planes_only);
+    return apply_launch(b, p, w, d, sc.colp, s, planes_only, riders);
 }
 
 bool eagcn::layer_reads_planes_only(const eagcn_batch* b, const eagcn_layer_params* p, bool aux_stream) {
@@ -1051,7 +1079,7 @@
 }
 
 static int apply_launch_(const eagcn_batch* b, const eagcn_layer_params* p, const eagcn_layer_bufs* w, const LayerDims& d,
-                         const float* colp, hipStream_t s, bool planes_only) {
+                         const float* colp, hipStream_t s, bool planes_only, const PackRiders* riders) {
     ProfScope psbn(PROF_BN, s);
     ApplyArgs aa;
     aa.bt = *b; aa.vc = d.vc; aa.structure = p->structure; aa.fp = d.fp; aa.Y = w->Y; aa.ldy = d.fp;
@@ -1066,7 +1094,9 @@
     static const int map_env = [] { const char* v = getenv("EAGCN_BN_APPLY_MAP"); return v ? atoi(v) : -1; }();
     aa.tile_map = map_env >= 0 ? map_env : (aa.planes.p ? 1 : 0);
     const size_t nthr = aa.tile_map ? (size_t)cdiv(std::max(b->T, 1), 8) * cdiv(d.ldo, 32) * 64 : (size_t)std::max(b->T, 1) * d.ldo / 4;
-    bn_apply_kernel<<<ew_grid(nthr), 256, 0, s>>>(aa);
+    if (riders && riders->n) { aa.riders = *riders; aa.nriders = riders->nb1 + riders->nb2 + riders->nb3; }
+    else { memset(&aa.riders, 0, sizeof(aa.riders)); aa.nriders = 0; }
+    bn_apply_kernel<<<ew_grid(nthr) + aa.nriders, 256, 0, s>>>(aa);
     EAGCN_LAUNCH_CHECK();
     return EAGCN_OK;
 }
@@ -1103,8 +1133,8 @@
 int eagcn::layer_backward_impl(const eagcn_batch* b, const eagcn_layer_params* p, const eagcn_layer_bufs* w,
                                const float* dxout, const ReadoutGrad* rg, const float* dpad_row, float* dx,
                                const eagcn_layer_grads* g, void* stream, bool dpad_views, const ZeroJob* zero_after,
-                               const EdgeDrain* drain_in, EdgeDrain* drain_out, bool input_only) {
-    if (drain_out) drain_out->eacc = nullptr;
+                               const DeferredGrads* drain_in, DeferredGrads* drain_out, bool input_only, size_t dw_region) {
+    if (drain_out) { drain_out->edge.eacc = nullptr; drain_out->unpack.nblocks = 0; }
     hipStream_t s = (hipStream_t)stream;
     int rc = check_layer(b, p, "eagcn_layer_backward");
     if (rc) return rc;
@@ -1118,7 +1148,7 @@
                             "eagcn_layer_backward: view %d has a null gradient buffer", k);
     const LayerDims d = layer_dims(b, p);
     BwdScratch sc;
-    const size_t need = carve_bwd(w->scratch, b, d, &sc);
+    const size_t need = carve_bwd(w->scratch, b, d, &sc, dw_region);
     if (need > w->scratch_bytes) {
         set_error("eagcn_layer_backward: scratch too small (%zu < %zu)", w->scratch_bytes, need);
         return EAGCN_ERR_SCRATCH;
@@ -1176,7 +1206,8 @@
     ba.seed_dev = p->seed_dev;
     ba.zero = zero_after ? zero_after->d : nullptr;
     ba.nzero = zero_after ? zero_after->nd : 0;
-    if (drain_in && drain_in->eacc) ba.drain = *drain_in; else memset(&ba.drain, 0, sizeof(ba.drain));
+    if (drain_in && drain_in->edge.eacc) ba.drain = drain_in->edge; else memset(&ba.drain, 0, sizeof(ba.drain));
+    if (drain_in && drain_in->unpack.nblocks > 0) ba.job = drain_in->unpack; else memset(&ba.job, 0, sizeof(ba.job));
     const int rows = b->T + ba.nvirt;
     const int gxb = std::max(1, std::min(rows, d.gxb));
     bool fused_bn_apply = false, fused_w_apply = false, w_rows = false, fused_c_apply = false;
@@ -1215,7 +1246,7 @@
         {
             const bool wt = p->structure == EAGCN_STRUCT_WEIGHTED, dr = ba.do_drop != 0;
             bool dg = ba.rg.dg != nullptr;
-            const dim3 grid(gxb, ny);
+            const dim3 grid(gxb + ba.job.nblocks, ny);
             ba.cc = sc.cc;
             ba.store_dh = bn_bwd_two_pass(wt) ? 0 : 1;
             static const bool rows_first = [] { const char* v = getenv("EAGCN_W_ROWS_FIRST"); return !(v && v[0] == '0'); }();
@@ -1227,6 +1258,7 @@
                 dg = false;
             }
             launch_bn_bwd_pass(false, wt, dg, dr, grid, ba, s);
+            ba.job.nblocks = 0;
         }
         EAGCN_LAUNCH_CHECK();
         const double* gsum = nullptr;
@@ -1393,16 +1425,25 @@
         const int edge_drain = edge_src == sc.eacc ? 1 : 0;
         static const bool defer_env = [] { const char* v = getenv("EAGCN_NO_EDGE_DEFER"); return !(v && v[0] == '1'); }();
         if (defer_env && drain_out && edge_drain && wblocks == 0 && !forked && b->T > 0) {
-            drain_out->eacc = sc.eacc; drain_out->K = p->K; drain_out->rsig = sc.rsig;
+            EdgeDrain& ed = drain_out->edge;
+            ed.eacc = sc.eacc; ed.K = p->K; ed.rsig = sc.rsig;
             for (int k = 0; k < EAGCN_MAX_VIEWS; ++k) {
-                drain_out->datt_w[k] = gp.datt_w[k]; drain_out->dself_r[k] = gp.dself_r[k]; drain_out->channels[k] = pp.channels[k];
+                ed.datt_w[k] = gp.datt_w[k]; ed.dself_r[k] = gp.dself_r[k]; ed.channels[k] = pp.channels[k];
             }
             return EAGCN_OK;
         }
+        UnpackJob uj;
+        uj.gp = gp; uj.pp = pp; uj.vc = d.vc; uj.in = in; uj.ld_in = d.ld_in; uj.fp = d.fp;
+        uj.dWcat = sc.dWcat; uj.nsplit = bx_slabs ? -nsplit : nsplit; uj.slab = d.wslab;
+        uj.datt = edge_src; uj.nedge = nedge; uj.rsig = sc.rsig; uj.wblocks = wblocks; uj.meta = b->meta;
+        uj.xk_G = xk_G; uj.edge_drain = edge_drain; uj.bx_per = bx_per; uj.bx_wide = bx_wide;
+        uj.nblocks = wblocks + cdiv(p->K * EDGE_SLAB, 16);
+        if ((chain_folds() & 1) && drain_out && edge_drain && wblocks > 0 && !forked && !w->stats_hook && b->T > 0) {
+            drain_out->unpack = uj;
+            return EAGCN_OK;
+        }
         ProfScope psu(PROF_PACK, side);
-        unpack_grads_kernel<<<wblocks + cdiv(p->K * EDGE_SLAB, 16), 256, 0, side>>>(gp, pp, d.vc, in, d.ld_in, d.fp, sc.dWcat,
-                                                                                    bx_slabs ? -nsplit : nsplit, d.wslab, edge_src, nedge, sc.rsig,
-                                                                                    wblocks, b->meta, xk_G, edge_drain, bx_per, bx_wide);
+        unpack_grads_kernel<<<uj.nblocks, 256, 0, side>>>(uj);
         EAGCN_LAUNCH_CHECK();
     }
     if (forked) { rc = stream_after(s, side); if (rc) return rc; }
diff --git a/include/eagcn_hip.h b/include/eagcn_hip.h
--- a/include/eagcn_hip.h
+++ b/include/eagcn_hip.h
@@ -323,6 +323,7 @@
 int eagcn_bx3_split(const float* x, int rows, int ld, uint16_t* planes, size_t plane_stride, int rows_cap, int np, void* stream);
 int eagcn_bx3_used_splits(int splits, int M, int N, int K);
 int eagcn_set_bx3_wide(int mode);
+int eagcn_set_chain_folds(int mask);
 int eagcn_bx3_pair_used_splits(int splits, int M, int N, int K, int M0, int N0, int K0);
 int eagcn_gemm_bx3(int tn, int M, int N, int K, const uint16_t* A, size_t a_pstride, int lda, int a_rows, const uint16_t* B,
                    size_t b_pstride, int ldb, int b_rows, float* C, int ldc, int splits, size_t slab, int np, void* stream);
```

After: 682,800. -4.0%, worse.
